# sikang/motion_primitive_library

Hardware: AMD Instinct MI355X
Metric: node-expansions/s (frontier x |U| pair evaluations per second) (higher is better)
Workload: dtype f64; 1 GPU; C4: 3D VoxelMapUtil 512^3, Control::ACC |U|=729 (9^3), 64k-node synthetic frontier; frontier=random, frontier_nodes=65536, frontier_nodes_per_gpu=65536, controls=729, dim=3, map_cells=134217728, device=AMD Radeon Graphics (gfx950:sramecc+:xnack-), compute_units=256, kernel=expand_lex_kernel

## Files before the change

### include/mplx.h

```cpp
#ifndef MPLX_H
#define MPLX_H

#include <stddef.h>
#include <stdint.h>

#ifdef __cplusplus
extern "C" {
#endif

#define MPLX_ABI_VERSION 9

typedef struct mplx_ctx mplx_ctx;

typedef enum {
  MPLX_OK = 0,
  MPLX_ERR_ARG = -1,
  MPLX_ERR_HIP = -2,
  MPLX_ERR_NO_DEVICE = -3,
  MPLX_ERR_STATE = -4,
  MPLX_ERR_NOMEM = -5
} mplx_status;

enum {
  MPLX_VEL = 0x01, MPLX_ACC = 0x03, MPLX_JRK = 0x07, MPLX_SNP = 0x0f,
  MPLX_VELxYAW = 0x11, MPLX_ACCxYAW = 0x13, MPLX_JRKxYAW = 0x17, MPLX_SNPxYAW = 0x1f
};

enum {
  MPLX_SLOT_SKIP_SAME = 0,
  MPLX_SLOT_FINITE = 1,
  MPLX_SLOT_BLOCKED = 2,
  MPLX_SLOT_SKIP_DYN = 3
};

typedef struct {
  int32_t control;
  int32_t reserved;
  double dt;
  double w;
  double wyaw;
  double v_max, a_max, j_max, yaw_max;
  double potential_weight;
  double gradient_weight;
} mplx_params;

typedef struct {
  uint8_t *status;
  double *cost;
  uint64_t *hash;
  double *state;
  int64_t state_stride;
  int32_t *iters;
} mplx_succ;

int mplx_create(int dim, int device, mplx_ctx **out);
void mplx_destroy(mplx_ctx *ctx);
const char *mplx_last_error(const mplx_ctx *ctx);
int mplx_abi_version(void);

int mplx_set_map(mplx_ctx *ctx, const int8_t *cells, const int32_t *dim, const double *origin,
                 double res);
int mplx_edit_map(mplx_ctx *ctx, const int64_t *cell_index, const int8_t *values, int64_t n);
int mplx_map_upload_bytes(mplx_ctx *ctx, uint64_t *bytes);
int mplx_read_cells(mplx_ctx *ctx, int which, const int64_t *cell_index, int64_t n, int8_t *out);

int mplx_set_potential(mplx_ctx *ctx, const int8_t *cells_or_null);
int mplx_set_region(mplx_ctx *ctx, const uint8_t *cells_or_null);
int mplx_set_params(mplx_ctx *ctx, const mplx_params *p);
int mplx_set_controls(mplx_ctx *ctx, const double *U, int32_t nU, int32_t udim);

int mplx_update_potential_map(mplx_ctx *ctx, const double *pos, const double *radius,
                              const double *range_or_null, double pow, int8_t *h_map_out_or_null);
int mplx_set_search_region_path(mplx_ctx *ctx, const double *path, int32_t n_points, int32_t dense,
                                const double *search_radius, uint8_t *h_region_out_or_null);

int mplx_expand_device(mplx_ctx *ctx, const double *d_nodes, int64_t n_nodes, int64_t node_stride,
                       const mplx_succ *d_out);
int mplx_expand(mplx_ctx *ctx, const double *h_nodes, int64_t n_nodes, int64_t node_stride,
                const mplx_succ *h_out);
int mplx_get_succ(mplx_ctx *ctx, const double *node, double *succ, double *cost, int32_t *action,
                  int32_t *n_succ);

typedef struct {
  int32_t *count;
  int32_t *action;
  double *cost;
  uint64_t *hash;
  double *state;
  int64_t state_stride;
  int32_t *iters;
  int64_t node_stride;
  double *heur;
  uint8_t *flags;
} mplx_succ_lists;

int mplx_expand_lists_device(mplx_ctx *ctx, const double *d_nodes, int64_t n_nodes, int64_t node_stride,
                             const mplx_succ_lists *d_out);
int mplx_expand_lists(mplx_ctx *ctx, const double *h_nodes, int64_t n_nodes, int64_t node_stride,
                      const mplx_succ_lists *h_out);

int mplx_lists_zero_fill(mplx_ctx *ctx, const mplx_succ_lists *d_lists, uint32_t *zero_rows);
int mplx_expand_lists_device_z(mplx_ctx *ctx, const double *d_nodes, int64_t n_nodes, int64_t node_stride,
                               const mplx_succ_lists *d_out, uint32_t *zero_rows);

typedef struct {
  const double *goal;
  int32_t control;
  int32_t goal_control;
  double w, v_max;
  double tol_pos, tol_vel, tol_acc, tol_yaw;
} mplx_goal_spec;

int mplx_set_goal(mplx_ctx *ctx, const mplx_goal_spec *goal);

typedef struct {
  double *heur;
  uint8_t *flags;
  int32_t *canon;
} mplx_post;

int mplx_post_lists_device(mplx_ctx *ctx, const mplx_succ_lists *d_lists, int64_t n_nodes,
                           const mplx_goal_spec *goal, const mplx_post *d_out);

typedef struct {
  int32_t *count;
  int64_t *offs;
  int32_t *action;
  double *cost;
  uint64_t *hash;
  double *state;
  int64_t state_stride;
  int64_t capacity;
} mplx_packed_lists;

int mplx_pack_lists_device(mplx_ctx *ctx, const mplx_succ_lists *d_lists, int64_t n_nodes,
                           const mplx_packed_lists *d_out, int64_t *h_total_or_null);

int mplx_post_packed_device(mplx_ctx *ctx, const mplx_packed_lists *d_packed, int64_t n_nodes,
                            const mplx_goal_spec *goal, const mplx_post *d_out);

#define MPLX_COMM_ID_BYTES 128
int mplx_comm_unique_id(uint8_t *id_out );
int mplx_comm_init(mplx_ctx *ctx, const uint8_t *id, int32_t rank, int32_t world);
int mplx_comm_destroy(mplx_ctx *ctx);
int mplx_comm_broadcast_map(mplx_ctx *ctx, int32_t root);
int mplx_comm_allgather_lists(mplx_ctx *ctx, const mplx_packed_lists *d_local, int64_t n_local,
                              const mplx_packed_lists *d_all, int64_t *h_node_offs, int64_t *h_entry_offs);

#define MPLX_COMM_META 8
enum { MPLX_ROWBIT_ACTION = 1, MPLX_ROWBIT_COST = 2, MPLX_ROWBIT_HASH = 4, MPLX_ROWBIT_STATE = 8 };
enum { MPLX_COMM_COPY = 0, MPLX_COMM_SEND = 1, MPLX_COMM_RECV = 2 };
enum { MPLX_ROW_COUNT = 0, MPLX_ROW_ACTION = 1, MPLX_ROW_COST = 2, MPLX_ROW_HASH = 3, MPLX_ROW_STATE0 = 4  };
typedef struct {
  int32_t kind;
  int32_t peer;
  int32_t row;
  int32_t elem;
  int64_t src_off;
  int64_t dst_off;
  int64_t bytes;
} mplx_comm_op;
int64_t mplx_comm_schedule(int32_t world, int32_t rank, const int64_t *meta, int32_t n_fields,
                           mplx_comm_op *ops, int64_t cap, int64_t *node_offs, int64_t *entry_offs);

typedef struct {
  uint8_t *free_flag;
  double *cost;
  int32_t *cells;
  int32_t *cell_count;
  int32_t cell_cap;
  uint8_t *outside;
} mplx_edges_out;
int mplx_check_edges(mplx_ctx *ctx, const double *h_parents, const int32_t *h_actions, int64_t n_edges,
                     int64_t stride, const mplx_edges_out *h_out);

int mplx_device_alloc(mplx_ctx *ctx, size_t bytes, void **dptr);
int mplx_device_free(mplx_ctx *ctx, void *dptr);
int mplx_memcpy_h2d(mplx_ctx *ctx, void *dst, const void *src, size_t bytes);
int mplx_memcpy_d2h(mplx_ctx *ctx, void *dst, const void *src, size_t bytes);
int mplx_memset(mplx_ctx *ctx, void *dst, int value, size_t bytes);
int mplx_synchronize(mplx_ctx *ctx);
int mplx_timer_begin(mplx_ctx *ctx);
int mplx_timer_end(mplx_ctx *ctx, float *ms);


typedef struct mplx_planner mplx_planner;

typedef int (*mplx_succ_fn)(void *user, const double *node, double *succ, double *cost,
                            int32_t *action, int32_t *n_succ);
typedef int (*mplx_batch_fn)(void *user, const double *nodes, int64_t n, uint8_t *status,
                             double *cost, double *state);

typedef struct {
  int32_t control;
  int32_t max_expand;
  int32_t batch;
  int32_t goal_control;
  double dt, w, v_max;
  double epsilon;
  double tol_pos, tol_vel, tol_acc, tol_yaw;
} mplx_planner_config;

typedef struct {
  int32_t ok;
  int32_t expansions;
  int32_t closed, opened, nodes;
  int32_t device_launches;
  int64_t pairs;
  double cost;
  double total_time;
  double J[4];
  int32_t segments;
  int32_t state_mismatches;
} mplx_plan_summary;

int mplx_planner_create(int dim, mplx_planner **out);
void mplx_planner_destroy(mplx_planner *p);
int mplx_planner_attach_ctx(mplx_planner *p, mplx_ctx *ctx);
int mplx_planner_set_provider(mplx_planner *p, mplx_succ_fn single, mplx_batch_fn batched, void *user);
int mplx_planner_set_map(mplx_planner *p, const int8_t *cells, const int32_t *dim,
                         const double *origin, double res);
int mplx_planner_edit_map(mplx_planner *p, const int64_t *cell_index, const int8_t *values, int64_t n);
int mplx_planner_set_controls(mplx_planner *p, const double *U, int32_t nU, int32_t udim);
int mplx_planner_configure(mplx_planner *p, const mplx_planner_config *cfg);
int mplx_planner_plan(mplx_planner *p, const double *start, const double *goal, mplx_plan_summary *out);
int mplx_planner_trajectory(mplx_planner *p, double *nodes, int32_t *actions, int32_t cap_segments);
int mplx_planner_trajectory_end(mplx_planner *p, double *node);
int mplx_planner_closed_set(mplx_planner *p, double *pos, int32_t cap, int32_t *n);
int mplx_planner_open_set(mplx_planner *p, double *states, int32_t cap, int32_t *n);
const char *mplx_planner_last_error(const mplx_planner *p);
typedef struct {
  double total_ms;
  double provider_ms;
  double fill_ms;
  double pick_ms;
  double relax_ms;
  double recover_ms;
  int64_t relaxed;
  int64_t improved;
  int64_t pushes;
  int64_t materialised;
  int64_t heur_from_device;
} mplx_plan_timing;
int mplx_planner_timing(const mplx_planner *p, mplx_plan_timing *out);
int mplx_planner_set_prior_trajectory(mplx_planner *p, const mplx_planner *from);
int mplx_planner_set_prior_trajectory_potential(mplx_planner *p, const mplx_planner *from, const int8_t *potential,
                                                double potential_weight, double gradient_weight);

int mplx_planner_set_lpastar(mplx_planner *p, int on);
int mplx_planner_reset(mplx_planner *p);
int mplx_planner_linked_nodes(mplx_planner *p, double *points, int64_t cap_points, int64_t *n_points, int64_t *n_cells,
                              int64_t *n_entries);
int mplx_planner_update_blocked_nodes(mplx_planner *p, const int32_t *cells, int64_t n);
int mplx_planner_update_cleared_nodes(mplx_planner *p, const int32_t *cells, int64_t n);
int mplx_planner_sub_state_space(mplx_planner *p, int32_t time_step);
typedef int (*mplx_edges_fn)(void *user, const double *parents, const int32_t *actions, int64_t n_edges, uint8_t *free_flag,
                             double *cost, int32_t *cells, int32_t *cell_count, int32_t cell_cap);
int mplx_planner_set_edge_provider(mplx_planner *p, mplx_edges_fn fn, void *user);
int mplx_planner_use_device_heuristic(mplx_planner *p, int on);

enum { MPLX_ROUTE_AUTO = 0, MPLX_ROUTE_DENSE = 1, MPLX_ROUTE_TILE = 2, MPLX_ROUTE_GRID = 3 };
int mplx_set_lists_route(mplx_ctx *ctx, int route);
int mplx_last_lists_route(const mplx_ctx *ctx);
int mplx_last_lists_zero_rows(const mplx_ctx *ctx);
enum { MPLX_KERNEL_NONE = 0, MPLX_KERNEL_GRID = 1, MPLX_KERNEL_LEX = 2,
       MPLX_KERNEL_PAIR = 3 };
int mplx_last_grid_kernel(const mplx_ctx *ctx);
enum { MPLX_IDENTITY_TABLE = 0, MPLX_IDENTITY_CLAIMED = 1, MPLX_IDENTITY_EXACT = 2, MPLX_IDENTITY_CLAIMED_THEN_EXACT = 3 };
int mplx_last_identity_form(const mplx_ctx *ctx);
int mplx_service(mplx_ctx *ctx, int mode, int64_t stats[4]);
int mplx_device_info(mplx_ctx *ctx, char *name, size_t cap, int32_t *compute_units);

#ifdef __cplusplus
}
#endif
#endif
```

### motion_primitive_library_amd/_abi.py

```python
import ctypes as C
import os

HERE = os.path.dirname(os.path.abspath(__file__))
LIB_PATH = os.environ.get("MPLX_LIB") or os.path.join(HERE, "csrc", "libmplx.so")

OK = 0
ERR_ARG, ERR_HIP, ERR_NO_DEVICE, ERR_STATE = -1, -2, -3, -4

SYMBOLS = [
    "mplx_create", "mplx_destroy", "mplx_last_error", "mplx_abi_version",
    "mplx_set_map", "mplx_edit_map", "mplx_map_upload_bytes", "mplx_read_cells", "mplx_set_potential", "mplx_set_region", "mplx_set_params", "mplx_set_controls",
    "mplx_update_potential_map", "mplx_set_search_region_path",
    "mplx_expand_device", "mplx_expand", "mplx_expand_lists_device", "mplx_expand_lists", "mplx_lists_zero_fill", "mplx_expand_lists_device_z", "mplx_get_succ",
    "mplx_set_goal", "mplx_post_lists_device", "mplx_post_packed_device",
    "mplx_pack_lists_device", "mplx_comm_unique_id", "mplx_comm_init", "mplx_comm_destroy", "mplx_comm_broadcast_map",
    "mplx_comm_allgather_lists", "mplx_comm_schedule",
    "mplx_check_edges",
    "mplx_device_alloc", "mplx_device_free", "mplx_memcpy_h2d", "mplx_memcpy_d2h", "mplx_memset",
    "mplx_synchronize", "mplx_timer_begin", "mplx_timer_end",
    "mplx_planner_create", "mplx_planner_destroy", "mplx_planner_attach_ctx", "mplx_planner_set_provider",
    "mplx_planner_set_map", "mplx_planner_edit_map", "mplx_planner_set_controls", "mplx_planner_configure", "mplx_planner_plan",
    "mplx_planner_trajectory", "mplx_planner_trajectory_end", "mplx_planner_closed_set", "mplx_planner_open_set", "mplx_planner_last_error", "mplx_planner_timing", "mplx_planner_set_prior_trajectory", "mplx_planner_set_prior_trajectory_potential", "mplx_planner_use_device_heuristic", "mplx_planner_set_lpastar", "mplx_planner_reset", "mplx_planner_linked_nodes", "mplx_planner_update_blocked_nodes", "mplx_planner_update_cleared_nodes", "mplx_planner_sub_state_space", "mplx_planner_set_edge_provider",
    "mplx_selftest_math", "mplx_selftest_forward_state", "mplx_set_lists_route", "mplx_last_lists_route", "mplx_last_lists_zero_rows", "mplx_last_grid_kernel", "mplx_last_identity_form", "mplx_debug_store_model", "mplx_yaw_pin_stats", "mplx_service", "mplx_device_info",
]

MAP_UTIL_SYMBOLS = ["mplx_map_dilate", "mplx_map_free", "mplx_map_cloud"]
CELL_OCCUPIED, CELL_FREE, CELL_UNKNOWN = 0, 1, 2
ROLLOUT_SYMBOLS = ["mplx_rollout_device", "mplx_rollout"]
ROLLOUT_BAD_ACTION, ROLLOUT_HEADING_BAND = 4, 0x80
RAY_SYMBOLS = ["mplx_ray_trace_device", "mplx_ray_trace", "mplx_goal_sight_device"]
RAY_LEFT_MAP, RAY_HIT, RAY_BAD, RAY_TRUNCATED = 1, 2, 4, 8
FLAG_GOAL_BLOCKED = 8
TRAJ_SYMBOLS = ["mplx_traj_info_device", "mplx_traj_info", "mplx_traj_sample_device", "mplx_traj_sample",
                "mplx_traj_traverse_device", "mplx_traj_traverse"]
TRAJ_EMPTY, TRAJ_BAD_ACTION, TRAJ_BAD = 1, 2, 4
TRAJ_COMMAND, TRAJ_WAYPOINT = 0, 1
TABLE_SYMBOLS = ["mplx_table_create", "mplx_table_destroy", "mplx_table_clear", "mplx_table_view_of", "mplx_table_stats",
                 "mplx_table_seed", "mplx_table_relax_device", "mplx_table_find_device", "mplx_table_find", "mplx_table_path",
                 "mplx_table_set_time_keys", "mplx_time_key"]
TABLE_NODES_FULL, TABLE_PROBE_FULL, TABLE_FRONTIER_FULL = 1, 2, 4
OPEN_SYMBOLS = ["mplx_open_create", "mplx_open_destroy", "mplx_open_clear", "mplx_open_view_of", "mplx_open_push_device",
                "mplx_open_select_device"]
OPEN_IS_OPEN, OPEN_IS_GOAL, OPEN_SEEN = 1, 2, 4
OPEN_SELECTED, OPEN_FOUND, OPEN_EMPTY = 0, 1, 2
MULTI_SYMBOLS = ["mplx_table_create_multi", "mplx_table_query_of", "mplx_table_seed_multi", "mplx_table_find_multi_device",
                 "mplx_table_find_multi", "mplx_open_set_goals", "mplx_open_select_multi_device"]
REPLAN_SYMBOLS = ["mplx_table_rebase_device", "mplx_table_rebase_multi_device", "mplx_open_push_closed_device"]
PRIOR_SYMBOLS = ["mplx_open_set_priors_device", "mplx_open_clear_priors", "mplx_open_prior_view_of", "mplx_planner_prior_table"]
SOLVE_SYMBOLS = ["mplx_poly_create", "mplx_poly_destroy", "mplx_solve_device", "mplx_solve", "mplx_poly_info_device",
                 "mplx_poly_info", "mplx_poly_sample_device", "mplx_poly_sample", "mplx_poly_traverse_device",
                 "mplx_poly_traverse"]
SOLVE_EMPTY, SOLVE_BAD_TIME, SOLVE_SINGULAR = 1, 2, 8
USE_POS, USE_VEL, USE_ACC = 1, 2, 4
LIMITS_SYMBOLS = ["mplx_poly_load_device", "mplx_poly_load", "mplx_poly_limits_device", "mplx_poly_limits",
                  "mplx_shortcut_device", "mplx_shortcut"]
SHORTCUT_BAD_CHAIN = 16
LIMITS_REFERENCE, LIMITS_ALL_ROOTS = 0, 1
EXCEED_VEL, EXCEED_ACC, EXCEED_JRK = 1, 2, 4
SCALE_SYMBOLS = ["mplx_poly_set_lambda_device", "mplx_poly_set_lambda", "mplx_poly_scale_device", "mplx_poly_scale",
                 "mplx_poly_scale_down_device", "mplx_poly_scale_down", "mplx_poly_tau_device", "mplx_poly_tau",
                 "mplx_poly_clear_lambda"]
SCALE_REFERENCE, SCALE_ROBUST = 0, 1
LAMBDA_BAD_POINTS, LAMBDA_NOT_POSITIVE = 32, 64
LAMBDA_MAX_SEGS, LAMBDA_NEWTON = 8, 3
CONFLICT_SYMBOLS = ["mplx_poly_conflicts_device", "mplx_poly_conflicts", "mplx_traj_conflicts_device", "mplx_traj_conflicts"]
CONFLICT_PARK, CONFLICT_GONE = 0, 1
CONFLICT_BAD_INPUT = 128
RESERVE_SYMBOLS = ["mplx_reserve_create", "mplx_reserve_destroy", "mplx_reserve_fill_poly_device", "mplx_reserve_fill_poly",
                   "mplx_reserve_fill_traj_device", "mplx_reserve_fill_traj", "mplx_reserve_shape", "mplx_reserve_positions",
                   "mplx_reserve_set_queries", "mplx_reserve_check_device", "mplx_reserve_park_device"]
RESERVE_MAX_BYTES = 1 << 30
WAIT_SYMBOLS = ["mplx_lists_add_wait_device"]
REPLAN_TIMED_SYMBOLS = ["mplx_table_rebase_timed_device"]
FIELD_SYMBOLS = ["mplx_field_create", "mplx_field_destroy", "mplx_field_build", "mplx_field_shape", "mplx_field_view_of",
                 "mplx_field_download", "mplx_field_is_stale", "mplx_field_passes", "mplx_open_set_field", "mplx_open_clear_field"]
FIELD_MAX_BYTES = 1 << 30
HEUR_SYMBOLS = ["mplx_heur_eval", "mplx_heur_eval_device", "mplx_open_set_heur", "mplx_planner_set_heur_dynamics"]
HEUR_DEFAULT, HEUR_REFERENCE, HEUR_ROBUST = 0, 1, 2
HEUR_BISECT = 56


def heur_mode(mode):
    names = {None: HEUR_DEFAULT, False: HEUR_DEFAULT, "default": HEUR_DEFAULT, "reference": HEUR_REFERENCE, "robust": HEUR_ROBUST}
    if isinstance(mode, str) or mode is None:
        if mode not in names:
            raise ValueError("heuristic mode %r: None, 'default', 'reference' or 'robust'" % (mode,))
        return names[mode]
    return int(mode)

ROUTE_AUTO, ROUTE_DENSE, ROUTE_TILE, ROUTE_GRID = 0, 1, 2, 3


class Params(C.Structure):
    _fields_ = [
        ("control", C.c_int32), ("reserved", C.c_int32),
        ("dt", C.c_double), ("w", C.c_double), ("wyaw", C.c_double),
        ("v_max", C.c_double), ("a_max", C.c_double), ("j_max", C.c_double), ("yaw_max", C.c_double),
        ("potential_weight", C.c_double), ("gradient_weight", C.c_double),
    ]


class Succ(C.Structure):
    _fields_ = [
        ("status", C.c_void_p), ("cost", C.c_void_p), ("hash", C.c_void_p),
        ("state", C.c_void_p), ("state_stride", C.c_int64), ("iters", C.c_void_p),
    ]


class SuccLists(C.Structure):
    _fields_ = [
        ("count", C.c_void_p), ("action", C.c_void_p), ("cost", C.c_void_p), ("hash", C.c_void_p),
        ("state", C.c_void_p), ("state_stride", C.c_int64), ("iters", C.c_void_p), ("node_stride", C.c_int64),
        ("heur", C.c_void_p), ("flags", C.c_void_p),
    ]


class RolloutOut(C.Structure):
    _fields_ = [
        ("status", C.c_void_p), ("steps", C.c_void_p), ("cost", C.c_void_p), ("prefix_cost", C.c_void_p),
        ("end_state", C.c_void_p), ("end_stride", C.c_int64),
        ("end_hash", C.c_void_p), ("end_heur", C.c_void_p), ("end_flags", C.c_void_p),
    ]


class RayOut(C.Structure):
    _fields_ = [("status", C.c_void_p), ("n_cells", C.c_void_p), ("first_hit", C.c_void_p), ("cells", C.c_void_p),
                ("cell_cap", C.c_int32)]


class TrajSet(C.Structure):
    _fields_ = [("starts", C.c_void_p), ("n_starts", C.c_int64), ("start_stride", C.c_int64), ("actions", C.c_void_p),
                ("n_traj", C.c_int64), ("horizon", C.c_int32), ("action_stride", C.c_int64)]


class TrajInfoOut(C.Structure):
    _fields_ = [("status", C.c_void_p), ("n_segs", C.c_void_p), ("total_time", C.c_void_p), ("effort", C.c_void_p),
                ("effort_stride", C.c_int64), ("seg_state", C.c_void_p), ("seg_stride", C.c_int64)]


class TrajTimes(C.Structure):
    _fields_ = [("form", C.c_int32), ("n_uniform", C.c_int32), ("times", C.c_void_p), ("n_times", C.c_int64),
                ("time_stride", C.c_int64)]


class TrajSampleOut(C.Structure):
    _fields_ = [("out", C.c_void_p), ("row_stride", C.c_int64), ("sample_stride", C.c_int64), ("status", C.c_void_p)]


class TrajTraverseOut(C.Structure):
    _fields_ = [("status", C.c_void_p), ("cost", C.c_void_p), ("n_samples", C.c_void_p), ("n_cells", C.c_void_p),
                ("stop_sample", C.c_void_p)]


class SolveIn(C.Structure):
    _fields_ = [("waypoints", C.c_void_p), ("n_prob", C.c_int64), ("w_max", C.c_int32), ("wp_stride", C.c_int64),
                ("n_wp", C.c_void_p), ("dts", C.c_void_p), ("dt_stride", C.c_int64), ("v", C.c_double),
                ("v_arr", C.c_void_p), ("control", C.c_int32), ("yaw_control", C.c_int32), ("wp_flags", C.c_void_p),
                ("flag_stride", C.c_int64)]


class SolveOut(C.Structure):
    _fields_ = [("status", C.c_void_p), ("n_segs", C.c_void_p), ("total_time", C.c_void_p), ("coeff", C.c_void_p),
                ("coeff_stride", C.c_int64), ("dts_out", C.c_void_p), ("dts_out_stride", C.c_int64),
                ("yaw_coeff", C.c_void_p), ("yaw_stride", C.c_int64), ("taus", C.c_void_p), ("taus_stride", C.c_int64)]


class PolyLoadIn(C.Structure):
    _fields_ = [("n_prob", C.c_int64), ("w_max", C.c_int32), ("control", C.c_int32), ("n_segs", C.c_void_p),
                ("dts", C.c_void_p), ("dt_stride", C.c_int64), ("coeff", C.c_void_p), ("coeff_stride", C.c_int64),
                ("src", C.c_void_p), ("src_index", C.c_void_p), ("index_stride", C.c_int64)]


class PolyLoadOut(C.Structure):
    _fields_ = [("status", C.c_void_p), ("n_segs", C.c_void_p), ("total_time", C.c_void_p), ("taus", C.c_void_p),
                ("taus_stride", C.c_int64)]


class ShortcutIn(C.Structure):
    _fields_ = [("states", C.c_void_p), ("n_query", C.c_int64), ("w_max", C.c_int32), ("control", C.c_int32),
                ("stride", C.c_int64), ("n_wp", C.c_void_p), ("max_hop", C.c_int32)]


class ShortcutOut(C.Structure):
    _fields_ = [("status", C.c_void_p), ("n_keep", C.c_void_p), ("keep", C.c_void_p), ("keep_stride", C.c_int64),
                ("cost", C.c_void_p), ("chain_cost", C.c_void_p), ("edge_cost", C.c_void_p), ("pair_out", C.POINTER(SolveOut))]


class LimitsIn(C.Structure):
    _fields_ = [("mv", C.c_double), ("ma", C.c_double), ("mj", C.c_double), ("mode", C.c_int32)]


class LimitsOut(C.Structure):
    _fields_ = [("max_vel", C.c_void_p), ("max_acc", C.c_void_p), ("max_jrk", C.c_void_p), ("max_stride", C.c_int64),
                ("exceed", C.c_void_p), ("valid", C.c_void_p), ("first_bad", C.c_void_p)]


class LambdaOut(C.Structure):
    _fields_ = [("status", C.c_void_p), ("n_lseg", C.c_void_p), ("total", C.c_void_p), ("Ts", C.c_void_p),
                ("ts_stride", C.c_int64), ("segs", C.c_void_p), ("seg_stride", C.c_int64)]


class LambdaIn(C.Structure):
    _fields_ = [("pts", C.c_void_p), ("stride", C.c_int64), ("n_pts", C.c_void_p), ("mode", C.c_int32)]


class ScaleIn(C.Structure):
    _fields_ = [("ri", C.c_double), ("rf", C.c_double), ("ri_arr", C.c_void_p), ("rf_arr", C.c_void_p), ("mode", C.c_int32)]


class ScaleDownIn(C.Structure):
    _fields_ = [("mv", C.c_double), ("ma", C.c_double), ("ri", C.c_double), ("rf", C.c_double), ("mode", C.c_int32)]


class ScaleDownOut(C.Structure):
    _fields_ = [("scaled", C.c_void_p), ("max_l", C.c_void_p), ("t_lo", C.c_void_p), ("t_hi", C.c_void_p), ("lam", LambdaOut)]


class TauOut(C.Structure):
    _fields_ = [("tau", C.c_void_p), ("lam", C.c_void_p), ("lam_dot", C.c_void_p), ("found", C.c_void_p), ("stride", C.c_int64)]


class ConflictIn(C.Structure):
    _fields_ = [("step", C.c_double), ("n_steps", C.c_int32), ("mode", C.c_int32), ("t0", C.c_void_p), ("radius", C.c_void_p),
                ("radius_all", C.c_double), ("group", C.c_void_p), ("rank", C.c_void_p), ("chunk_steps", C.c_int32)]


class ConflictOut(C.Structure):
    _fields_ = [("first_step", C.c_void_p), ("first_partner", C.c_void_p), ("min_d2", C.c_void_p), ("status", C.c_void_p),
                ("pair_first", C.c_void_p), ("pair_stride", C.c_int64)]


class TableView(C.Structure):
    _fields_ = [("hash", C.c_void_p), ("g", C.c_void_p), ("pred", C.c_void_p), ("pred_action", C.c_void_p),
                ("state", C.c_void_p), ("state_stride", C.c_int64)]


class TableFrontier(C.Structure):
    _fields_ = [("id", C.c_void_p), ("g", C.c_void_p), ("state", C.c_void_p), ("state_stride", C.c_int64),
                ("capacity", C.c_int64), ("count", C.c_void_p)]


class OpenView(C.Structure):
    _fields_ = [("f", C.c_void_p), ("flags", C.c_void_p)]


class OpenResult(C.Structure):
    _fields_ = [("status", C.c_int32), ("goal_id", C.c_int32), ("count", C.c_int64), ("n_open", C.c_int64),
                ("f_min", C.c_double), ("goal_f", C.c_double), ("goal_g", C.c_double)]


class PriorSource(C.Structure):
    _fields_ = [("control", C.c_int32), ("nU", C.c_int32), ("udim", C.c_int32), ("U", C.c_void_p), ("dt", C.c_double)]


class PriorInfo(C.Structure):
    _fields_ = [("status", C.c_void_p), ("n_steps", C.c_void_p)]


class PriorView(C.Structure):
    _fields_ = [("n_steps", C.c_void_p), ("pos", C.c_void_p), ("togo", C.c_void_p), ("goal_row", C.c_void_p),
                ("goal_hash", C.c_void_p), ("step_capacity", C.c_int64)]


class FieldView(C.Structure):
    _fields_ = [("dist", C.c_void_p), ("F", C.c_int32), ("n_cells", C.c_int64)]


class RebaseResult(C.Structure):
    _fields_ = [("n_kept", C.c_int64), ("n_bad_edges", C.c_int64), ("n_roots", C.c_int64)]


class PackedLists(C.Structure):
    _fields_ = [
        ("count", C.c_void_p), ("offs", C.c_void_p), ("action", C.c_void_p), ("cost", C.c_void_p), ("hash", C.c_void_p),
        ("state", C.c_void_p), ("state_stride", C.c_int64), ("capacity", C.c_int64),
    ]


COMM_ID_BYTES = 128
COMM_META = 8
ROWBIT_ACTION, ROWBIT_COST, ROWBIT_HASH, ROWBIT_STATE = 1, 2, 4, 8
COMM_COPY, COMM_SEND, COMM_RECV = 0, 1, 2
ROW_COUNT, ROW_ACTION, ROW_COST, ROW_HASH, ROW_STATE0 = 0, 1, 2, 3, 4


class CommOp(C.Structure):
    _fields_ = [("kind", C.c_int32), ("peer", C.c_int32), ("row", C.c_int32), ("elem", C.c_int32),
                ("src_off", C.c_int64), ("dst_off", C.c_int64), ("bytes", C.c_int64)]


class GoalSpec(C.Structure):
    _fields_ = [("goal", C.c_void_p), ("control", C.c_int32), ("goal_control", C.c_int32), ("w", C.c_double),
                ("v_max", C.c_double), ("tol_pos", C.c_double), ("tol_vel", C.c_double), ("tol_acc", C.c_double),
                ("tol_yaw", C.c_double)]


class EdgesOut(C.Structure):
    _fields_ = [("free_flag", C.c_void_p), ("cost", C.c_void_p), ("cells", C.c_void_p), ("cell_count", C.c_void_p),
                ("cell_cap", C.c_int32), ("outside", C.c_void_p)]


class Post(C.Structure):
    _fields_ = [("heur", C.c_void_p), ("flags", C.c_void_p), ("canon", C.c_void_p)]


class PlannerConfig(C.Structure):
    _fields_ = [
        ("control", C.c_int32), ("max_expand", C.c_int32), ("batch", C.c_int32), ("goal_control", C.c_int32),
        ("dt", C.c_double), ("w", C.c_double), ("v_max", C.c_double), ("epsilon", C.c_double),
        ("tol_pos", C.c_double), ("tol_vel", C.c_double), ("tol_acc", C.c_double), ("tol_yaw", C.c_double),
    ]


class PlanSummary(C.Structure):
    _fields_ = [
        ("ok", C.c_int32), ("expansions", C.c_int32), ("closed", C.c_int32), ("opened", C.c_int32),
        ("nodes", C.c_int32), ("device_launches", C.c_int32), ("pairs", C.c_int64),
        ("cost", C.c_double), ("total_time", C.c_double), ("J", C.c_double * 4),
        ("segments", C.c_int32), ("state_mismatches", C.c_int32),
    ]


class PlanTiming(C.Structure):
    _fields_ = [(k, C.c_double) for k in ("total_ms", "provider_ms", "fill_ms", "pick_ms", "relax_ms", "recover_ms")] + \
               [(k, C.c_int64) for k in ("relaxed", "improved", "pushes", "materialised", "heur_from_device")]


class MplxError(RuntimeError):
    def __init__(self, code, text):
        super().__init__("mplx error %d: %s" % (code, text))
        self.code = code


_lib = None


def lib():
    global _lib
    if _lib is not None:
        return _lib
    if not os.path.exists(LIB_PATH):
        raise ImportError(
            "motion_primitive_library_amd: %s is missing. Build it with "
            "`python -m motion_primitive_library_amd.build` (needs hipcc); there is no CPU fallback."
            % LIB_PATH)
    try:
        L = C.CDLL(LIB_PATH)
    except OSError as e:
        raise ImportError("motion_primitive_library_amd: cannot load %s: %s" % (LIB_PATH, e))
    vp, i32, i64, dbl = C.c_void_p, C.c_int32, C.c_int64, C.c_double
    sig = {
        "mplx_create": (C.c_int, [C.c_int, C.c_int, C.POINTER(vp)]),
        "mplx_destroy": (None, [vp]),
        "mplx_last_error": (C.c_char_p, [vp]),
        "mplx_abi_version": (C.c_int, []),
        "mplx_set_map": (C.c_int, [vp, vp, vp, vp, dbl]),
        "mplx_set_potential": (C.c_int, [vp, vp]),
        "mplx_set_region": (C.c_int, [vp, vp]),
        "mplx_set_params": (C.c_int, [vp, C.POINTER(Params)]),
        "mplx_set_controls": (C.c_int, [vp, vp, i32, i32]),
        "mplx_edit_map": (C.c_int, [vp, vp, vp, i64]),
        "mplx_map_upload_bytes": (C.c_int, [vp, C.POINTER(C.c_uint64)]),
        "mplx_read_cells": (C.c_int, [vp, C.c_int, vp, i64, vp]),
        "mplx_set_goal": (C.c_int, [vp, C.POINTER(GoalSpec)]),
        "mplx_update_potential_map": (C.c_int, [vp, vp, vp, vp, dbl, vp]),
        "mplx_set_search_region_path": (C.c_int, [vp, vp, i32, i32, vp, vp]),
        "mplx_expand_device": (C.c_int, [vp, vp, i64, i64, C.POINTER(Succ)]),
        "mplx_expand": (C.c_int, [vp, vp, i64, i64, C.POINTER(Succ)]),
        "mplx_expand_lists_device": (C.c_int, [vp, vp, i64, i64, C.POINTER(SuccLists)]),
        "mplx_expand_lists": (C.c_int, [vp, vp, i64, i64, C.POINTER(SuccLists)]),
        "mplx_lists_zero_fill": (C.c_int, [vp, C.POINTER(SuccLists), C.POINTER(C.c_uint32)]),
        "mplx_expand_lists_device_z": (C.c_int, [vp, vp, i64, i64, C.POINTER(SuccLists), C.POINTER(C.c_uint32)]),
        "mplx_get_succ": (C.c_int, [vp, vp, vp, vp, vp, C.POINTER(i32)]),
        "mplx_post_lists_device": (C.c_int, [vp, C.POINTER(SuccLists), i64, C.POINTER(GoalSpec), C.POINTER(Post)]),
        "mplx_check_edges": (C.c_int, [vp, vp, vp, i64, i64, C.POINTER(EdgesOut)]),
        "mplx_pack_lists_device": (C.c_int, [vp, C.POINTER(SuccLists), i64, C.POINTER(PackedLists), C.POINTER(i64)]),
        "mplx_post_packed_device": (C.c_int, [vp, C.POINTER(PackedLists), i64, C.POINTER(GoalSpec), C.POINTER(Post)]),
        "mplx_comm_unique_id": (C.c_int, [vp]),
        "mplx_comm_init": (C.c_int, [vp, vp, i32, i32]),
        "mplx_comm_destroy": (C.c_int, [vp]),
        "mplx_comm_broadcast_map": (C.c_int, [vp, i32]),
        "mplx_comm_allgather_lists": (C.c_int, [vp, C.POINTER(PackedLists), i64, C.POINTER(PackedLists), vp, vp]),
        "mplx_comm_schedule": (i64, [i32, i32, vp, i32, C.POINTER(CommOp), i64, vp, vp]),
        "mplx_device_alloc": (C.c_int, [vp, C.c_size_t, C.POINTER(vp)]),
        "mplx_device_free": (C.c_int, [vp, vp]),
        "mplx_memcpy_h2d": (C.c_int, [vp, vp, vp, C.c_size_t]),
        "mplx_memcpy_d2h": (C.c_int, [vp, vp, vp, C.c_size_t]),
        "mplx_memset": (C.c_int, [vp, vp, C.c_int, C.c_size_t]),
        "mplx_synchronize": (C.c_int, [vp]),
        "mplx_timer_begin": (C.c_int, [vp]),
        "mplx_timer_end": (C.c_int, [vp, C.POINTER(C.c_float)]),
        "mplx_planner_create": (C.c_int, [C.c_int, C.POINTER(vp)]),
        "mplx_planner_destroy": (None, [vp]),
        "mplx_planner_attach_ctx": (C.c_int, [vp, vp]),
        "mplx_planner_set_provider": (C.c_int, [vp, vp, vp, vp]),
        "mplx_planner_set_map": (C.c_int, [vp, vp, vp, vp, dbl]),
        "mplx_planner_edit_map": (C.c_int, [vp, vp, vp, i64]),
        "mplx_planner_set_controls": (C.c_int, [vp, vp, i32, i32]),
        "mplx_planner_configure": (C.c_int, [vp, C.POINTER(PlannerConfig)]),
        "mplx_planner_plan": (C.c_int, [vp, vp, vp, C.POINTER(PlanSummary)]),
        "mplx_planner_trajectory": (C.c_int, [vp, vp, vp, i32]),
        "mplx_planner_trajectory_end": (C.c_int, [vp, vp]),
        "mplx_planner_closed_set": (C.c_int, [vp, vp, i32, C.POINTER(i32)]),
        "mplx_planner_open_set": (C.c_int, [vp, vp, i32, C.POINTER(i32)]),
        "mplx_planner_last_error": (C.c_char_p, [vp]),
        "mplx_planner_timing": (C.c_int, [vp, C.POINTER(PlanTiming)]),
        "mplx_planner_use_device_heuristic": (C.c_int, [vp, C.c_int]),
        "mplx_planner_set_prior_trajectory": (C.c_int, [vp, vp]),
        "mplx_planner_set_prior_trajectory_potential": (C.c_int, [vp, vp, vp, dbl, dbl]),
        "mplx_planner_set_lpastar": (C.c_int, [vp, C.c_int]),
        "mplx_planner_reset": (C.c_int, [vp]),
        "mplx_planner_linked_nodes": (C.c_int, [vp, vp, i64, C.POINTER(i64), C.POINTER(i64), C.POINTER(i64)]),
        "mplx_planner_update_blocked_nodes": (C.c_int, [vp, vp, i64]),
        "mplx_planner_update_cleared_nodes": (C.c_int, [vp, vp, i64]),
        "mplx_planner_sub_state_space": (C.c_int, [vp, i32]),
        "mplx_planner_set_edge_provider": (C.c_int, [vp, vp, vp]),
        "mplx_selftest_math": (C.c_int, [vp, C.c_int, vp, vp, vp, i64]),
        "mplx_selftest_forward_state": (C.c_int, [i32, i32, vp, vp, C.c_double, vp]),
        "mplx_set_lists_route": (C.c_int, [vp, C.c_int]),
        "mplx_last_lists_route": (C.c_int, [vp]),
        "mplx_last_lists_zero_rows": (C.c_int, [vp]),
        "mplx_last_grid_kernel": (C.c_int, [vp]),
        "mplx_last_identity_form": (C.c_int, [vp]),
        "mplx_debug_store_model": (C.c_int, [vp, C.POINTER(SuccLists), i64]),
        "mplx_yaw_pin_stats": (C.c_int, [vp, C.POINTER(i64), C.POINTER(i64)]),
        "mplx_service": (C.c_int, [vp, C.c_int, C.POINTER(i64)]),
        "mplx_device_info": (C.c_int, [vp, C.c_char_p, C.c_size_t, C.POINTER(i32)]),
        "mplx_map_dilate": (C.c_int, [vp, vp, i32, vp]),
        "mplx_map_free": (C.c_int, [vp, C.c_int, vp]),
        "mplx_map_cloud": (C.c_int, [vp, C.c_int, vp, i64, C.POINTER(i64)]),
        "mplx_rollout_device": (C.c_int, [vp, vp, i64, i64, vp, i64, i32, i64, C.POINTER(RolloutOut)]),
        "mplx_rollout": (C.c_int, [vp, vp, i64, i64, vp, i64, i32, i64, C.POINTER(RolloutOut)]),
        "mplx_ray_trace_device": (C.c_int, [vp, vp, vp, i64, i64, i64, i32, C.POINTER(RayOut)]),
        "mplx_ray_trace": (C.c_int, [vp, vp, vp, i64, i64, i64, i32, C.POINTER(RayOut)]),
        "mplx_goal_sight_device": (C.c_int, [vp, C.POINTER(SuccLists), i64, C.POINTER(GoalSpec), vp]),
        "mplx_traj_info_device": (C.c_int, [vp, C.POINTER(TrajSet), C.POINTER(TrajInfoOut)]),
        "mplx_traj_info": (C.c_int, [vp, C.POINTER(TrajSet), C.POINTER(TrajInfoOut)]),
        "mplx_traj_sample_device": (C.c_int, [vp, C.POINTER(TrajSet), C.POINTER(TrajTimes), C.POINTER(TrajSampleOut)]),
        "mplx_traj_sample": (C.c_int, [vp, C.POINTER(TrajSet), C.POINTER(TrajTimes), C.POINTER(TrajSampleOut)]),
        "mplx_traj_traverse_device": (C.c_int, [vp, C.POINTER(TrajSet), i32, C.POINTER(TrajTraverseOut)]),
        "mplx_traj_traverse": (C.c_int, [vp, C.POINTER(TrajSet), i32, C.POINTER(TrajTraverseOut)]),
        "mplx_poly_create": (C.c_int, [vp, i64, i32, C.POINTER(vp)]),
        "mplx_poly_destroy": (None, [vp]),
        "mplx_solve_device": (C.c_int, [vp, C.POINTER(SolveIn), C.POINTER(SolveOut)]),
        "mplx_solve": (C.c_int, [vp, C.POINTER(SolveIn), C.POINTER(SolveOut)]),
        "mplx_poly_info_device": (C.c_int, [vp, C.POINTER(TrajInfoOut)]),
        "mplx_poly_info": (C.c_int, [vp, C.POINTER(TrajInfoOut)]),
        "mplx_poly_sample_device": (C.c_int, [vp, C.POINTER(TrajTimes), C.POINTER(TrajSampleOut)]),
        "mplx_poly_sample": (C.c_int, [vp, C.POINTER(TrajTimes), C.POINTER(TrajSampleOut)]),
        "mplx_poly_traverse_device": (C.c_int, [vp, i32, C.POINTER(TrajTraverseOut)]),
        "mplx_poly_traverse": (C.c_int, [vp, i32, C.POINTER(TrajTraverseOut)]),
        "mplx_poly_load_device": (C.c_int, [vp, C.POINTER(PolyLoadIn), C.POINTER(PolyLoadOut)]),
        "mplx_poly_load": (C.c_int, [vp, C.POINTER(PolyLoadIn), C.POINTER(PolyLoadOut)]),
        "mplx_poly_limits_device": (C.c_int, [vp, C.POINTER(LimitsIn), C.POINTER(LimitsOut)]),
        "mplx_poly_limits": (C.c_int, [vp, C.POINTER(LimitsIn), C.POINTER(LimitsOut)]),
        "mplx_shortcut_device": (C.c_int, [vp, vp, C.POINTER(ShortcutIn), C.POINTER(ShortcutOut)]),
        "mplx_shortcut": (C.c_int, [vp, vp, C.POINTER(ShortcutIn), C.POINTER(ShortcutOut)]),
        "mplx_poly_set_lambda_device": (C.c_int, [vp, C.POINTER(LambdaIn), C.POINTER(LambdaOut)]),
        "mplx_poly_set_lambda": (C.c_int, [vp, C.POINTER(LambdaIn), C.POINTER(LambdaOut)]),
        "mplx_poly_scale_device": (C.c_int, [vp, C.POINTER(ScaleIn), C.POINTER(LambdaOut)]),
        "mplx_poly_scale": (C.c_int, [vp, C.POINTER(ScaleIn), C.POINTER(LambdaOut)]),
        "mplx_poly_scale_down_device": (C.c_int, [vp, C.POINTER(ScaleDownIn), C.POINTER(ScaleDownOut)]),
        "mplx_poly_scale_down": (C.c_int, [vp, C.POINTER(ScaleDownIn), C.POINTER(ScaleDownOut)]),
        "mplx_poly_tau_device": (C.c_int, [vp, C.POINTER(TrajTimes), C.POINTER(TauOut)]),
        "mplx_poly_tau": (C.c_int, [vp, C.POINTER(TrajTimes), C.POINTER(TauOut)]),
        "mplx_poly_clear_lambda": (C.c_int, [vp]),
        "mplx_poly_conflicts_device": (C.c_int, [vp, C.POINTER(ConflictIn), C.POINTER(ConflictOut)]),
        "mplx_poly_conflicts": (C.c_int, [vp, C.POINTER(ConflictIn), C.POINTER(ConflictOut)]),
        "mplx_traj_conflicts_device": (C.c_int, [vp, C.POINTER(TrajSet), C.POINTER(ConflictIn), C.POINTER(ConflictOut)]),
        "mplx_traj_conflicts": (C.c_int, [vp, C.POINTER(TrajSet), C.POINTER(ConflictIn), C.POINTER(ConflictOut)]),
        "mplx_table_create": (C.c_int, [vp, i64, i32, C.POINTER(vp)]),
        "mplx_table_destroy": (None, [vp]),
        "mplx_table_clear": (C.c_int, [vp]),
        "mplx_table_view_of": (C.c_int, [vp, C.POINTER(TableView)]),
        "mplx_table_stats": (C.c_int, [vp, C.POINTER(i64), C.POINTER(C.c_uint32)]),
        "mplx_table_seed": (C.c_int, [vp, vp, i64, i64, vp, C.POINTER(TableFrontier), C.POINTER(i64)]),
        "mplx_table_relax_device": (C.c_int, [vp, C.POINTER(SuccLists), i64, vp, vp, dbl, C.POINTER(TableFrontier), vp,
                                              C.POINTER(i64)]),
        "mplx_table_find_device": (C.c_int, [vp, vp, i64, vp]),
        "mplx_table_find": (C.c_int, [vp, vp, i64, vp]),
        "mplx_table_path": (C.c_int, [vp, i32, vp, vp, i64, C.POINTER(i64)]),
        "mplx_open_create": (C.c_int, [vp, C.POINTER(vp)]),
        "mplx_open_destroy": (None, [vp]),
        "mplx_open_clear": (C.c_int, [vp]),
        "mplx_open_view_of": (C.c_int, [vp, C.POINTER(OpenView)]),
        "mplx_open_push_device": (C.c_int, [vp, C.POINTER(TableFrontier), i64, dbl, i32]),
        "mplx_open_select_device": (C.c_int, [vp, dbl, C.POINTER(TableFrontier), vp, C.POINTER(OpenResult)]),
        "mplx_table_create_multi": (C.c_int, [vp, i64, i32, i32, C.POINTER(vp)]),
        "mplx_table_query_of": (C.c_int, [vp, C.POINTER(vp), C.POINTER(i32)]),
        "mplx_table_seed_multi": (C.c_int, [vp, vp, i64, i64, vp, vp, C.POINTER(TableFrontier), C.POINTER(i64)]),
        "mplx_table_find_multi_device": (C.c_int, [vp, vp, vp, i64, vp]),
        "mplx_table_find_multi": (C.c_int, [vp, vp, vp, i64, vp]),
        "mplx_open_set_goals": (C.c_int, [vp, C.POINTER(GoalSpec), i32]),
        "mplx_open_select_multi_device": (C.c_int, [vp, dbl, C.POINTER(TableFrontier), vp, C.POINTER(OpenResult)]),
        "mplx_table_rebase_device": (C.c_int, [vp, i32, i32, C.POINTER(TableFrontier), vp, C.POINTER(RebaseResult)]),
        "mplx_table_rebase_multi_device": (C.c_int, [vp, vp, i32, C.POINTER(TableFrontier), vp, C.POINTER(RebaseResult)]),
        "mplx_open_push_closed_device": (C.c_int, [vp, C.POINTER(TableFrontier), i64, dbl, i32]),
        "mplx_open_set_priors_device": (C.c_int, [vp, C.POINTER(PriorSource), C.POINTER(TrajSet), C.POINTER(PriorInfo)]),
        "mplx_open_clear_priors": (C.c_int, [vp]),
        "mplx_open_prior_view_of": (C.c_int, [vp, C.POINTER(PriorView)]),
        "mplx_planner_prior_table": (C.c_int, [vp, vp, vp, i32, C.POINTER(i32), vp, C.POINTER(i32)]),
        "mplx_reserve_create": (C.c_int, [vp, C.POINTER(vp)]),
        "mplx_reserve_destroy": (None, [vp]),
        "mplx_reserve_fill_poly_device": (C.c_int, [vp, vp, C.POINTER(ConflictIn)]),
        "mplx_reserve_fill_poly": (C.c_int, [vp, vp, C.POINTER(ConflictIn)]),
        "mplx_reserve_fill_traj_device": (C.c_int, [vp, vp, C.POINTER(TrajSet), C.POINTER(ConflictIn)]),
        "mplx_reserve_fill_traj": (C.c_int, [vp, vp, C.POINTER(TrajSet), C.POINTER(ConflictIn)]),
        "mplx_reserve_shape": (C.c_int, [vp, C.POINTER(i64), C.POINTER(i32), C.POINTER(dbl)]),
        "mplx_reserve_positions": (C.c_int, [vp, vp, vp, vp, vp, vp, vp]),
        "mplx_reserve_set_queries": (C.c_int, [vp, i32, vp, vp, vp]),
        "mplx_reserve_check_device": (C.c_int, [vp, vp, C.POINTER(SuccLists), i64, vp, vp, i64, vp, vp]),
        "mplx_reserve_park_device": (C.c_int, [vp, vp, C.POINTER(TableFrontier), i64, vp, vp]),
        "mplx_lists_add_wait_device": (C.c_int, [vp, C.POINTER(SuccLists), i64, vp, i64, vp, vp]),
        "mplx_table_rebase_timed_device": (C.c_int, [vp, vp, i32, i32, vp, C.POINTER(TableFrontier), vp, vp, vp,
                                                    C.POINTER(RebaseResult)]),
        "mplx_field_create": (C.c_int, [vp, C.POINTER(vp)]),
        "mplx_field_destroy": (None, [vp]),
        "mplx_field_build": (C.c_int, [vp, i32, vp, vp]),
        "mplx_field_shape": (C.c_int, [vp, C.POINTER(i32), C.POINTER(i64)]),
        "mplx_field_view_of": (C.c_int, [vp, C.POINTER(FieldView)]),
        "mplx_field_download": (C.c_int, [vp, vp]),
        "mplx_field_is_stale": (C.c_int, [vp]),
        "mplx_field_passes": (C.c_int, [vp, C.POINTER(i64)]),
        "mplx_open_set_field": (C.c_int, [vp, vp, vp]),
        "mplx_open_clear_field": (C.c_int, [vp]),
        "mplx_heur_eval": (C.c_int, [vp, C.POINTER(GoalSpec), i32, vp, i64, i64, vp]),
        "mplx_heur_eval_device": (C.c_int, [vp, C.POINTER(GoalSpec), i32, vp, i64, i64, vp]),
        "mplx_open_set_heur": (C.c_int, [vp, i32]),
        "mplx_planner_set_heur_dynamics": (C.c_int, [vp, i32]),
        "mplx_table_set_time_keys": (C.c_int, [vp, i32]),
        "mplx_time_key": (C.c_uint64, [C.c_uint64, dbl]),
    }
    for name in SYMBOLS + MAP_UTIL_SYMBOLS + ROLLOUT_SYMBOLS + RAY_SYMBOLS + TRAJ_SYMBOLS + TABLE_SYMBOLS + OPEN_SYMBOLS + MULTI_SYMBOLS + REPLAN_SYMBOLS + PRIOR_SYMBOLS + SOLVE_SYMBOLS + LIMITS_SYMBOLS + SCALE_SYMBOLS + CONFLICT_SYMBOLS + RESERVE_SYMBOLS + WAIT_SYMBOLS + REPLAN_TIMED_SYMBOLS + FIELD_SYMBOLS + HEUR_SYMBOLS:
        fn = getattr(L, name)
        fn.restype, fn.argtypes = sig[name]
    _lib = L
    return L


def check(ctx, rc):
    if rc != OK:
        msg = lib().mplx_last_error(ctx)
        raise MplxError(rc, msg.decode() if msg else "?")
```

### motion_primitive_library_amd/build.py

```python
import os
import shutil
import subprocess
import sys

HERE = os.path.dirname(os.path.abspath(__file__))
CSRC = os.path.join(HERE, "csrc")
LIB = os.path.join(CSRC, "libmplx.so")
SOURCES = ["expand_kernel.hip", "expand_tile_kernel.hip", "expand_grid_kernel.hip", "expand_lex_kernel.hip", "expand_pair_kernel.hip", "map_prep_kernel.hip", "map_prep_api.cpp", "map_util_kernel.hip", "map_util_api.cpp", "rollout_kernel.hip", "rollout_api.cpp", "ray_kernel.hip", "ray_api.cpp", "traj_kernel.hip", "traj_api.cpp", "solve_kernel.hip", "solve_api.cpp", "limits_kernel.hip", "limits_api.cpp", "scale_kernel.hip", "scale_api.cpp", "conflict_kernel.hip", "conflict_api.cpp", "reserve_kernel.hip", "reserve_api.cpp", "wait_kernel.hip", "wait_api.cpp", "table_kernel.hip", "table_api.cpp", "open_kernel.hip", "open_api.cpp", "field_kernel.hip", "field_api.cpp", "heur_kernel.hip", "heur_api.cpp", "replan_kernel.hip", "replan_api.cpp", "post_kernel.hip", "identity_kernel.hip", "post_api.cpp", "edge_kernel.hip", "edge_api.cpp", "mplx_api.cpp", "lists_route.cpp", "yaw_pin.cpp", "lists_host.cpp", "planner_capi.cpp", "pack_kernel.hip", "store_model_kernel.hip", "lists_copy_api.cpp", "pack_api.cpp", "comm_api.cpp"]
HEADERS = ["mplx_internal.h", "mplx_ctx.h", "mplx_device_common.h", "mplx_pair_device.h", "mplx_grid_common.h", "mplx_poly.h", "mplx_traj_device.h", "mplx_limits_math.h", "mplx_scale_math.h", "mplx_heur_math.h", "host_planner.hpp", "host_lpastar.hpp", os.path.join("..", "..", "include", "mplx.h"), os.path.join("..", "..", "include", "mplx_debug.h"), os.path.join("..", "..", "include", "mplx_map_util.h"), os.path.join("..", "..", "include", "mplx_rollout.h"), os.path.join("..", "..", "include", "mplx_ray.h"), os.path.join("..", "..", "include", "mplx_traj.h"), os.path.join("..", "..", "include", "mplx_table.h"), os.path.join("..", "..", "include", "mplx_open.h"), os.path.join("..", "..", "include", "mplx_multi.h"), os.path.join("..", "..", "include", "mplx_replan.h"), os.path.join("..", "..", "include", "mplx_replan_timed.h"), os.path.join("..", "..", "include", "mplx_prior.h"), os.path.join("..", "..", "include", "mplx_solve.h"), os.path.join("..", "..", "include", "mplx_limits.h"), os.path.join("..", "..", "include", "mplx_scale.h"), os.path.join("..", "..", "include", "mplx_conflict.h"), os.path.join("..", "..", "include", "mplx_reserve.h"), os.path.join("..", "..", "include", "mplx_wait.h"), os.path.join("..", "..", "include", "mplx_field.h"), os.path.join("..", "..", "include", "mplx_heur.h")]
ARCH = "gfx950"


def hipcc_path():
    for cand in (os.environ.get("HIPCC"), shutil.which("hipcc"), "/opt/rocm/bin/hipcc"):
        if cand and os.path.exists(cand):
            return cand
    raise RuntimeError("hipcc not found (set HIPCC or install ROCm under /opt/rocm)")


def _obj_dir():
    d = os.path.join(CSRC, "build")
    os.makedirs(d, exist_ok=True)
    return d


def is_stale():
    if not os.path.exists(LIB):
        return True
    t = os.path.getmtime(LIB)
    deps = [os.path.join(CSRC, s) for s in SOURCES + HEADERS]
    return any(os.path.getmtime(d) > t for d in deps)


FLAGS = ["--offload-arch=" + ARCH, "-O3", "-std=c++17", "-ffp-contract=off", "-fPIC", "-Wall"]
EXTRA_FLAGS = {}


def build_variant(out_path, defines, verbose=False):
    cmd = [hipcc_path()] + FLAGS + ["-D" + d for d in defines] + ["-shared", "-o", out_path] + SOURCES
    if verbose:
        print(" ".join(cmd), file=sys.stderr)
    proc = subprocess.run(cmd, cwd=CSRC, capture_output=True, text=True)
    if proc.returncode != 0:
        raise RuntimeError("hipcc failed:\n%s\n%s" % (proc.stdout, proc.stderr))
    return out_path


def build(force=False, verbose=False, jobs=None):
    if not force and not is_stale():
        return LIB
    from concurrent.futures import ThreadPoolExecutor

    hipcc = hipcc_path()
    odir = _obj_dir()
    hdr_t = max(os.path.getmtime(os.path.join(CSRC, h)) for h in HEADERS)
    todo, objs = [], []
    for src in SOURCES:
        obj = os.path.join(odir, src + ".o")
        objs.append(obj)
        st = max(os.path.getmtime(os.path.join(CSRC, src)), hdr_t)
        if force or not os.path.exists(obj) or os.path.getmtime(obj) < st:
            todo.append((src, obj))

    def cc(job):
        src, obj = job
        cmd = [hipcc] + FLAGS + EXTRA_FLAGS.get(src, []) + ["-x", "hip", "-c", src, "-o", obj]
        if verbose:
            print(" ".join(cmd), file=sys.stderr)
        return src, subprocess.run(cmd, cwd=CSRC, capture_output=True, text=True)

    with ThreadPoolExecutor(max_workers=jobs or min(8, os.cpu_count() or 1)) as ex:
        for src, proc in ex.map(cc, todo):
            if proc.returncode != 0:
                raise RuntimeError("hipcc failed on %s:\n%s\n%s" % (src, proc.stdout, proc.stderr))
            if verbose and proc.stderr.strip():
                print(proc.stderr, file=sys.stderr)
    cmd = [hipcc, "--offload-arch=" + ARCH, "-fPIC", "-shared", "-o", LIB] + objs
    if verbose:
        print(" ".join(cmd), file=sys.stderr)
    proc = subprocess.run(cmd, cwd=CSRC, capture_output=True, text=True)
    if proc.returncode != 0:
        raise RuntimeError("hipcc link failed:\n%s\n%s" % (proc.stdout, proc.stderr))
    return LIB


if __name__ == "__main__":
    if "--define" in sys.argv:
        defs = [d for i, a in enumerate(sys.argv[:-1]) if a == "--define" for d in sys.argv[i + 1].split(",")]
        out = sys.argv[sys.argv.index("--out") + 1]
        print(build_variant(os.path.abspath(out), defs, verbose=True))
    else:
        print(build(force="--force" in sys.argv, verbose=True))
```

### motion_primitive_library_amd/csrc/lists_copy_api.cpp

```cpp
#include "mplx_ctx.h"

#include <atomic>
#include <cstring>
#include <thread>

namespace mplx_detail {

namespace {

struct Row {
  const void *dev;
  char *host;
  int es;
  int64_t host_node_stride;
};

constexpr size_t kChunkBytes = 32u << 20;

int ensure_pinned(mplx_ctx *c, size_t bytes) {
  if (bytes <= c->pk_pin_cap) return MPLX_OK;
  for (int i = 0; i < 2; i++) {
    if (c->pk_pin[i]) HIP_TRY(c, hipHostFree(c->pk_pin[i]));
    c->pk_pin[i] = nullptr;
  }
  c->pk_pin_cap = 0;
  for (int i = 0; i < 2; i++) HIP_TRY(c, hipHostMalloc(&c->pk_pin[i], bytes, hipHostMallocDefault));
  c->pk_pin_cap = bytes;
  return MPLX_OK;
}

struct Chunk {
  int64_t node0, node1, off0, entries;
};

void scatter(const Row *rows, int n_rows, const int64_t *row_off, const char *pin, const int32_t *count,
             const int64_t *offs, const Chunk &ch, int64_t a, int64_t b) {
  for (int r = 0; r < n_rows; r++) {
    const int es = rows[r].es;
    const char *src = pin + row_off[r];
    for (int64_t k = a; k < b; k++) {
      const int cnt = count[k];
      if (cnt > 0)
        std::memcpy(rows[r].host + (size_t)k * rows[r].host_node_stride * es, src + (size_t)(offs[k] - ch.off0) * es,
                    (size_t)cnt * es);
    }
  }
}

}

void release_copy_buffers(mplx_ctx *c) {
  for (int i = 0; i < 2; i++) {
    if (c->pk_pin[i]) (void)hipHostFree(c->pk_pin[i]);
    c->pk_pin[i] = nullptr;
    if (c->pk_ev[i]) (void)hipEventDestroy(c->pk_ev[i]);
    c->pk_ev[i] = nullptr;
    release(c->pk_dev[i]);
  }
  c->pk_pin_cap = 0;
  release(c->pk_offs);
  if (c->pk_hb) (void)hipHostFree(c->pk_hb);
  c->pk_hb = nullptr;
  c->pk_hb_cap = 0;
}

int copy_lists_to_host(mplx_ctx *c, const mplx_succ_lists &d, const mplx_succ_lists *h, int64_t n_nodes) {
  const int F = 4 * c->dim + 2;
  const int64_t S = list_stride(c, &d);
  HIP_TRY(c, hipMemcpyAsync(h->count, d.count, (size_t)n_nodes * 4, hipMemcpyDeviceToHost, c->stream));
  HIP_TRY(c, hipStreamSynchronize(c->stream));
  Row rows[mplx::kPackRows];
  int n_rows = 0;
  if (h->cost) rows[n_rows++] = {d.cost, (char *)h->cost, 8, S};
  if (h->hash) rows[n_rows++] = {d.hash, (char *)h->hash, 8, S};
  if (h->state)
    for (int f = 0; f < F; f++)
      rows[n_rows++] = {d.state + (size_t)f * d.state_stride, (char *)(h->state + (size_t)f * h->state_stride), 8, S};
  if (h->action) rows[n_rows++] = {d.action, (char *)h->action, 4, S};
  if (h->iters) rows[n_rows++] = {d.iters, (char *)h->iters, 4, S};
  if (n_rows == 0) return MPLX_OK;
  int bpe = 0;
  for (int r = 0; r < n_rows; r++) bpe += rows[r].es;

  std::vector<int64_t> &offs = c->pk_hoffs;
  offs.resize((size_t)n_nodes + 1);
  int64_t total = 0;
  int max_cnt = 0;
  for (int64_t k = 0; k < n_nodes; k++) {
    offs[(size_t)k] = total;
    const int cnt = h->count[k];
    total += cnt;
    max_cnt = cnt > max_cnt ? cnt : max_cnt;
  }
  offs[(size_t)n_nodes] = total;
  if (total == 0) return MPLX_OK;
  size_t cap = kChunkBytes;
  if ((size_t)max_cnt * bpe > cap) cap = (size_t)max_cnt * bpe;
  if ((size_t)total * bpe < cap) cap = (size_t)total * bpe;
  cap = align256(cap);
  const int64_t cap_entries = (int64_t)(cap / bpe);
  if (int rc = ensure_pinned(c, cap)) return rc;
  for (int i = 0; i < 2; i++) {
    if (int rc = ensure(c, c->pk_dev[i], cap)) return rc;
    if (!c->pk_ev[i]) HIP_TRY(c, hipEventCreateWithFlags(&c->pk_ev[i], hipEventDisableTiming));
  }
  if (int rc = ensure(c, c->pk_offs, (size_t)n_nodes * 8)) return rc;
  HIP_TRY(c, hipMemcpyAsync(c->pk_offs.p, offs.data(), (size_t)n_nodes * 8, hipMemcpyHostToDevice, c->stream));

  std::vector<Chunk> chunks;
  for (int64_t a = 0; a < n_nodes;) {
    int64_t b = a + 1;
    while (b < n_nodes && offs[(size_t)b + 1] - offs[(size_t)a] <= cap_entries) b++;
    chunks.push_back({a, b, offs[(size_t)a], offs[(size_t)b] - offs[(size_t)a]});
    a = b;
  }
  const int n_chunks = (int)chunks.size();
  std::vector<int64_t> row_off((size_t)n_chunks * n_rows);
  for (int i = 0; i < n_chunks; i++) {
    int64_t o = 0;
    for (int r = 0; r < n_rows; r++) {
      row_off[(size_t)i * n_rows + r] = o;
      o += chunks[(size_t)i].entries * rows[r].es;
    }
  }

  int n_thr = (int)(((size_t)total * bpe) >> 23);
  const int hw = (int)std::thread::hardware_concurrency();
  if (n_thr > 15) n_thr = 15;
  if (hw > 0 && n_thr > hw - 1) n_thr = hw - 1;
  if (n_thr < 0) n_thr = 0;
  int parts = n_thr + 1;
  std::atomic<int> ready{0};
  std::atomic<int> done{0};
  std::atomic<bool> cancel{false};
  const int32_t *count = h->count;
  auto share = [&](int i, int part) {
    const Chunk &ch = chunks[(size_t)i];
    const int64_t n = ch.node1 - ch.node0;
    const int64_t a = ch.node0 + n * part / parts, b = ch.node0 + n * (part + 1) / parts;
    scatter(rows, n_rows, &row_off[(size_t)i * n_rows], (const char *)c->pk_pin[i & 1], count, offs.data(), ch, a, b);
  };
  std::vector<std::thread> helpers;
  try {
    for (int t = 0; t < n_thr; t++)
      helpers.emplace_back([&, t] {
        for (int i = 0; i < n_chunks; i++) {
          while (ready.load(std::memory_order_acquire) <= i) std::this_thread::yield();
          if (cancel.load(std::memory_order_acquire)) return;
          share(i, t + 1);
          done.fetch_add(1, std::memory_order_release);
        }
      });
  } catch (...) {
    cancel.store(true, std::memory_order_release);
    ready.store(n_chunks + 1, std::memory_order_release);
    for (auto &th : helpers) th.join();
    helpers.clear();
    ready.store(0, std::memory_order_release);
    n_thr = 0;
    parts = 1;
  }
  auto join_all = [&] {
    ready.store(n_chunks + 1, std::memory_order_release);
    for (auto &th : helpers) th.join();
  };

  int rc = MPLX_OK;
  auto issue = [&](int i) -> hipError_t {
    const Chunk &ch = chunks[(size_t)i];
    mplx::PackArgs a{};
    for (int r = 0; r < n_rows; r++) {
      a.src[r] = rows[r].dev;
      a.dst_off[r] = row_off[(size_t)i * n_rows + r];
      a.es[r] = rows[r].es;
    }
    a.n_rows = n_rows;
    a.node_stride = S;
    a.count = d.count;
    a.offs = (const int64_t *)c->pk_offs.p;
    a.node0 = ch.node0;
    a.off0 = ch.off0;
    a.dst = (char *)c->pk_dev[i & 1].p;
    hipError_t e = mplx::launch_pack_rows(a, ch.node1 - ch.node0, c->stream);
    if (e != hipSuccess) return e;
    if (ch.entries > 0) {
      e = hipMemcpyAsync(c->pk_pin[i & 1], c->pk_dev[i & 1].p, (size_t)ch.entries * bpe, hipMemcpyDeviceToHost, c->stream);
      if (e != hipSuccess) return e;
    }
    return hipEventRecord(c->pk_ev[i & 1], c->stream);
  };
  for (int i = 0; i <= n_chunks && rc == MPLX_OK; i++) {
    hipError_t e = hipSuccess;
    if (i < n_chunks) e = issue(i);
    if (e == hipSuccess && i >= 1) e = hipEventSynchronize(c->pk_ev[(i - 1) & 1]);
    if (e != hipSuccess) {
      rc = fail(c, MPLX_ERR_HIP, "copy of the successor lists failed: %s", hipGetErrorString(e));
      break;
    }
    if (i >= 1) {
      ready.store(i, std::memory_order_release);
      share(i - 1, 0);
      while (done.load(std::memory_order_acquire) < i * n_thr) std::this_thread::yield();
    }
  }
  if (rc != MPLX_OK) {
    join_all();
    (void)hipStreamSynchronize(c->stream);
    return rc;
  }
  join_all();
  return MPLX_OK;
}

int expand_lists_packed(mplx_ctx *c, const double *h_nodes, int64_t n_nodes, int64_t node_stride, bool want_state,
                        PackedLists *out, bool want_heur) {
  if (!c || !out || !h_nodes || n_nodes <= 0 || node_stride < n_nodes) return fail(c, MPLX_ERR_ARG, "expand_lists_packed: bad arguments");
  if (int rc = ctx_ready(c)) return rc;
  const int F = 4 * c->dim + 2;
  const int64_t S = (c->nU + 31) & ~31;
  const int64_t n_slots = n_nodes * S;
  {
    mplx_succ_lists want{}, v{};
    int32_t dummy_i = 0;
    double dummy_d = 0;
    uint64_t dummy_h = 0;
    want.count = &dummy_i; want.action = &dummy_i; want.cost = &dummy_d; want.hash = &dummy_h;
    if (want_state) want.state = &dummy_d;
    if (want_heur) want.heur = &dummy_d;
    want.node_stride = S;
    bool handled = false;
    if (int rc = svc_request(c, h_nodes, n_nodes, node_stride, &want, &handled, &v)) return rc;
    if (handled) {
      c->pk_hoffs.resize((size_t)n_nodes + 1);
      for (int64_t k = 0; k <= n_nodes; k++) c->pk_hoffs[(size_t)k] = k * S;
      *out = PackedLists{};
      out->total = want_state ? v.state_stride : n_slots;
      out->count = v.count;
      out->offs = c->pk_hoffs.data();
      out->cost = v.cost;
      out->hash = v.hash;
      out->action = v.action;
      out->state = want_state ? v.state : nullptr;
      out->heur = want_heur ? v.heur : nullptr;
      return MPLX_OK;
    }
    const int counted = c->svc.streak;
    if (int rc = bind_device(c)) return rc;
    c->svc.streak = counted;
  }
  if (c->tune.zero_copy && (size_t)n_slots * (size_t)((want_state ? F * 8 : 0) + 24 + (want_heur ? 8 : 0)) <= ((size_t)32 << 20)) {
    const size_t o_cnt = align256((size_t)F * n_nodes * 8);
    const size_t o_off = o_cnt + align256((size_t)n_nodes * 4);
    const size_t o_act = o_off + align256((size_t)(n_nodes + 1) * 8);
    const size_t o_cost = o_act + align256((size_t)n_slots * 4);
    const size_t o_hash = o_cost + align256((size_t)n_slots * 8);
    const size_t o_heur = o_hash + align256((size_t)n_slots * 8);
    const size_t o_state = o_heur + (want_heur ? align256((size_t)n_slots * 8) : 0);
    const size_t bytes = o_state + (want_state ? align256((size_t)F * n_slots * 8) : 0);
    if (bytes > c->pk_hb_cap) {
      if (c->pk_hb) HIP_TRY(c, hipHostFree(c->pk_hb));
      c->pk_hb = nullptr;
      c->pk_hb_cap = 0;
      HIP_TRY(c, hipHostMalloc(&c->pk_hb, bytes + bytes / 2, hipHostMallocCoherent));
      c->pk_hb_cap = bytes + bytes / 2;
    }
    char *hb = (char *)c->pk_hb;
    for (int f = 0; f < F; f++)
      std::memcpy(hb + (size_t)f * n_nodes * 8, h_nodes + (size_t)f * node_stride, (size_t)n_nodes * 8);
    mplx_succ_lists d{};
    d.count = (int32_t *)(hb + o_cnt);
    d.action = (int32_t *)(hb + o_act);
    d.cost = (double *)(hb + o_cost);
    d.hash = (uint64_t *)(hb + o_hash);
    if (want_state) { d.state = (double *)(hb + o_state); d.state_stride = n_slots; }
    if (want_heur) d.heur = (double *)(hb + o_heur);
    d.node_stride = S;
    c->want_done = true;
    const int rc_launch = lists_device(c, (const double *)hb, n_nodes, n_nodes, &d);
    c->want_done = false;
    if (rc_launch) return rc_launch;
    if (int rc = wait_small_launch(c)) return rc;
    if (int rc = resolve_pending(c, true)) return rc;
    int64_t *offs = (int64_t *)(hb + o_off);
    for (int64_t k = 0; k <= n_nodes; k++) offs[k] = k * S;
    *out = PackedLists{};
    out->total = n_slots;
    out->count = d.count;
    out->offs = offs;
    out->cost = d.cost;
    out->hash = d.hash;
    out->action = d.action;
    out->state = d.state;
    out->heur = d.heur;
    return MPLX_OK;
  }
  const size_t o_cnt = align256((size_t)F * n_nodes * 8);
  const size_t o_off = o_cnt + align256((size_t)n_nodes * 4);
  const size_t hb_bytes = o_off + (size_t)(n_nodes + 1) * 8;
  if (hb_bytes > c->pk_hb_cap) {
    if (c->pk_hb) HIP_TRY(c, hipHostFree(c->pk_hb));
    c->pk_hb = nullptr;
    c->pk_hb_cap = 0;
    HIP_TRY(c, hipHostMalloc(&c->pk_hb, hb_bytes * 2, hipHostMallocCoherent));
    c->pk_hb_cap = hb_bytes * 2;
  }
  char *hb = (char *)c->pk_hb;
  for (int f = 0; f < F; f++)
    std::memcpy(hb + (size_t)f * n_nodes * 8, h_nodes + (size_t)f * node_stride, (size_t)n_nodes * 8);
  const size_t slots = (size_t)n_slots;
  StageLayout l;
  const size_t o_nodes = l.add((size_t)F * n_nodes * 8), o_count = l.add((size_t)n_nodes * 4), o_action = l.add(slots * 4),
               o_cost = l.add(slots * 8), o_hash = l.add(slots * 8), o_state = l.add(want_state ? F * slots * 8 : 0);
  if (int rc = stage_commit(c, &l)) return rc;
  if (int rc = ensure(c, c->pk_offs, (size_t)n_nodes * 8)) return rc;
  HIP_TRY(c, stage_in(c, l.base + o_nodes, hb, (size_t)F * n_nodes * 8));
  mplx_succ_lists d{};
  d.count = (int32_t *)(l.base + o_count);
  d.action = (int32_t *)(l.base + o_action);
  d.cost = (double *)(l.base + o_cost);
  d.hash = (uint64_t *)(l.base + o_hash);
  if (want_state) { d.state = (double *)(l.base + o_state); d.state_stride = n_slots; }
  d.node_stride = S;
  if (int rc = lists_device(c, (const double *)(l.base + o_nodes), n_nodes, n_nodes, &d)) return rc;
  if (int rc = resolve_pending(c)) return rc;
  int32_t *cnt = (int32_t *)(hb + o_cnt);
  int64_t *offs = (int64_t *)(hb + o_off);
  HIP_TRY(c, hipMemcpyAsync(cnt, d.count, (size_t)n_nodes * 4, hipMemcpyDeviceToHost, c->stream));
  HIP_TRY(c, hipStreamSynchronize(c->stream));
  int64_t total = 0;
  for (int64_t k = 0; k < n_nodes; k++) { offs[k] = total; total += cnt[k]; }
  offs[n_nodes] = total;
  *out = PackedLists{};
  out->total = total;
  out->count = cnt;
  out->offs = offs;
  if (total == 0) return MPLX_OK;
  const int bpe = 8 + 8 + (want_state ? 8 * F : 0) + 4;
  const size_t bytes = align256((size_t)total * bpe);
  if (int rc = ensure_pinned(c, bytes)) return rc;
  if (int rc = ensure(c, c->pk_dev[0], bytes)) return rc;
  HIP_TRY(c, hipMemcpyAsync(c->pk_offs.p, offs, (size_t)n_nodes * 8, hipMemcpyHostToDevice, c->stream));
  mplx::PackArgs a{};
  int r = 0;
  int64_t o = 0;
  auto row = [&](const void *src, int es) { a.src[r] = src; a.dst_off[r] = o; a.es[r] = es; o += total * es; r++; };
  row(d.cost, 8);
  row(d.hash, 8);
  if (want_state)
    for (int f = 0; f < F; f++) row(d.state + (size_t)f * n_slots, 8);
  row(d.action, 4);
  a.n_rows = r;
  a.node_stride = S;
  a.count = d.count;
  a.offs = (const int64_t *)c->pk_offs.p;
  a.node0 = 0;
  a.off0 = 0;
  a.dst = (char *)c->pk_dev[0].p;
  HIP_TRY(c, mplx::launch_pack_rows(a, n_nodes, c->stream));
  HIP_TRY(c, hipMemcpyAsync(c->pk_pin[0], c->pk_dev[0].p, (size_t)total * bpe, hipMemcpyDeviceToHost, c->stream));
  HIP_TRY(c, hipStreamSynchronize(c->stream));
  const char *pin = (const char *)c->pk_pin[0];
  out->cost = (const double *)(pin + a.dst_off[0]);
  out->hash = (const uint64_t *)(pin + a.dst_off[1]);
  out->state = want_state ? (const double *)(pin + a.dst_off[2]) : nullptr;
  out->action = (const int32_t *)(pin + a.dst_off[want_state ? 2 + F : 2]);
  return MPLX_OK;
}

}
```

### motion_primitive_library_amd/csrc/lists_host.cpp

```cpp
#include "mplx_ctx.h"

#include <atomic>
#include <chrono>
#include <cstring>

using namespace mplx_detail;

namespace {

double mono_us() {
  return std::chrono::duration<double, std::micro>(std::chrono::steady_clock::now().time_since_epoch()).count();
}

struct ArenaLayout {
  size_t o_count = 0, o_action = 0, o_cost = 0, o_hash = 0, o_iters = 0, o_heur = 0, o_flags = 0, o_state = 0, total = 0;
  int64_t n_alloc = 0, n_slots = 0;
};
enum : unsigned { kRowAction = 1, kRowCost = 2, kRowHash = 4, kRowIters = 8, kRowState = 16, kRowHeur = 32, kRowFlags = 64 };

unsigned rows_of(const mplx_succ_lists *o) {
  return (o->action ? kRowAction : 0u) | (o->cost ? kRowCost : 0u) | (o->hash ? kRowHash : 0u) |
         (o->iters ? kRowIters : 0u) | (o->state ? kRowState : 0u) | (o->heur ? kRowHeur : 0u) | (o->flags ? kRowFlags : 0u);
}

ArenaLayout arena_layout(int F, int64_t n_alloc, int64_t S, unsigned rows) {
  ArenaLayout L;
  L.n_alloc = n_alloc;
  L.n_slots = n_alloc * S;
  L.o_count = align256((size_t)F * n_alloc * 8);
  L.o_action = L.o_count + align256((size_t)n_alloc * 4);
  L.o_cost = L.o_action + ((rows & kRowAction) ? align256((size_t)L.n_slots * 4) : 0);
  L.o_hash = L.o_cost + ((rows & kRowCost) ? align256((size_t)L.n_slots * 8) : 0);
  L.o_iters = L.o_hash + ((rows & kRowHash) ? align256((size_t)L.n_slots * 8) : 0);
  L.o_heur = L.o_iters + ((rows & kRowIters) ? align256((size_t)L.n_slots * 4) : 0);
  L.o_flags = L.o_heur + ((rows & kRowHeur) ? align256((size_t)L.n_slots * 8) : 0);
  L.o_state = L.o_flags + ((rows & kRowFlags) ? align256((size_t)L.n_slots) : 0);
  L.total = L.o_state + ((rows & kRowState) ? align256((size_t)F * L.n_slots * 8) : 0);
  return L;
}

void arena_put_nodes(char *hb, const ArenaLayout &L, int F, const double *h_nodes, int64_t n_nodes, int64_t node_stride) {
  for (int f = 0; f < F; f++)
    std::memcpy(hb + (size_t)f * L.n_alloc * 8, h_nodes + (size_t)f * node_stride, (size_t)n_nodes * 8);
}

mplx_succ_lists arena_lists(char *b, const ArenaLayout &L, int64_t S, unsigned rows) {
  mplx_succ_lists d{};
  d.count = (int32_t *)(b + L.o_count);
  if (rows & kRowAction) d.action = (int32_t *)(b + L.o_action);
  if (rows & kRowCost) d.cost = (double *)(b + L.o_cost);
  if (rows & kRowHash) d.hash = (uint64_t *)(b + L.o_hash);
  if (rows & kRowIters) d.iters = (int32_t *)(b + L.o_iters);
  if (rows & kRowHeur) d.heur = (double *)(b + L.o_heur);
  if (rows & kRowFlags) d.flags = (uint8_t *)(b + L.o_flags);
  if (rows & kRowState) { d.state = (double *)(b + L.o_state); d.state_stride = L.n_slots; }
  d.node_stride = S;
  return d;
}

void arena_get_lists(const char *hb, const ArenaLayout &L, int F, int64_t S, int64_t n_nodes, const mplx_succ_lists *h_out) {
  const int32_t *cnt = (const int32_t *)(hb + L.o_count);
  std::memcpy(h_out->count, cnt, (size_t)n_nodes * 4);
  for (int64_t k = 0; k < n_nodes; k++) {
    const size_t m = (size_t)cnt[k], at = (size_t)k * (size_t)S;
    if (!m) continue;
    if (h_out->action) std::memcpy(h_out->action + at, hb + L.o_action + at * 4, m * 4);
    if (h_out->cost) std::memcpy(h_out->cost + at, hb + L.o_cost + at * 8, m * 8);
    if (h_out->hash) std::memcpy(h_out->hash + at, hb + L.o_hash + at * 8, m * 8);
    if (h_out->iters) std::memcpy(h_out->iters + at, hb + L.o_iters + at * 4, m * 4);
    if (h_out->heur) std::memcpy(h_out->heur + at, hb + L.o_heur + at * 8, m * 8);
    if (h_out->flags) std::memcpy(h_out->flags + at, hb + L.o_flags + at, m);
    if (h_out->state)
      for (int f = 0; f < F; f++)
        std::memcpy(h_out->state + (size_t)f * h_out->state_stride + at,
                    hb + L.o_state + ((size_t)f * L.n_slots + at) * 8, m * 8);
  }
}

int svc_launch(mplx_ctx *c, const TilePlan &tp, uint32_t seq_served) {
  mplx_ctx::Service &sv = c->svc;
  const int F = 4 * c->dim + 2;
  HIP_TRY(c, hipSetDevice(c->device));
  if (!sv.stream) HIP_TRY(c, hipStreamCreateWithFlags(&sv.stream, hipStreamNonBlocking));
  if (!sv.mb) {
    HIP_TRY(c, hipHostMalloc((void **)&sv.mb, sizeof(mplx::SvcMailbox), hipHostMallocCoherent));
    std::memset(sv.mb, 0, sizeof(mplx::SvcMailbox));
  }
  if (int rc = ensure_tables(c)) return rc;
  HIP_TRY(c, hipStreamSynchronize(c->stream));
  const ArenaLayout L = arena_layout(F, sv.cap, sv.S, sv.rows);
  if (L.total > sv.block_cap) {
    if (sv.block) HIP_TRY(c, hipHostFree(sv.block));
    sv.block = nullptr;
    sv.block_cap = 0;
    HIP_TRY(c, hipHostMalloc((void **)&sv.block, L.total, hipHostMallocCoherent));
    sv.block_cap = L.total;
  }
  int64_t g = (sv.cap + tp.npb - 1) / tp.npb;
  if (g > tp.grid) g = tp.grid;
  if (g > 1024) g = 1024;
  sv.workgroups = (int)g;
  if (int rc = ensure(c, sv.dev, (size_t)(1 + g) * 8)) return rc;
  HIP_TRY(c, hipMemsetAsync(sv.dev.p, 0, (size_t)(1 + g) * 8, sv.stream));
  const mplx_succ_lists d = arena_lists(sv.block, L, sv.S, sv.rows);
  mplx::TileArgs a = tile_args(c, tp, (const double *)sv.block, sv.cap, sv.cap, &d);
  a.grid_limit = (int32_t)g;
  a.svc_mb = sv.mb;
  a.svc_dev = (uint64_t *)sv.dev.p;
  a.svc_seq0 = seq_served;
  a.svc_idle = (uint64_t)c->tune.service_idle_us * 100ull;
  const int resident = mplx::tile_service_resident_workgroups(c->dim, c->prm.control, a);
  if (resident > 0 && resident < (int)g) {
    sv.disabled = true;
    return MPLX_OK;
  }
  *(volatile uint32_t *)&sv.mb->quit = 0;
  *(volatile uint32_t *)&sv.mb->alive = 1;
  std::atomic_thread_fence(std::memory_order_seq_cst);
  HIP_TRY(c, mplx::launch_expand_tile(c->dim, c->prm.control, a, sv.stream));
  sv.running = true;
  sv.launches++;
  return MPLX_OK;
}
}

int mplx_detail::svc_stop(mplx_ctx *c) {
  mplx_ctx::Service &sv = c->svc;
  if (!sv.running) return MPLX_OK;
  sv.running = false;
  *(volatile uint32_t *)&sv.mb->quit = 1;
  std::atomic_thread_fence(std::memory_order_seq_cst);
  const hipError_t e = hipStreamSynchronize(sv.stream);
  *(volatile uint32_t *)&sv.mb->quit = 0;
  if (e != hipSuccess) {
    sv.disabled = true;
    return fail(c, MPLX_ERR_HIP, "the resident expansion kernel did not leave: %s", hipGetErrorString(e));
  }
  return MPLX_OK;
}

int mplx_detail::wait_small_launch(mplx_ctx *c) {
  if (!c->done_armed) {
    HIP_TRY(c, hipStreamSynchronize(c->stream));
    return MPLX_OK;
  }
  c->done_armed = false;
  volatile uint64_t *f = c->done_host;
  const uint64_t want = c->done_seq;
  double t0 = 0;
  c->done_waits++;
  for (uint32_t spins = 1; *f != want; spins++) {
    __builtin_ia32_pause();
    if ((spins & 0xfffu) != 0) continue;
    const double now = mono_us();
    if (t0 == 0) t0 = now;
    if (now - t0 > 2e5) {
      c->done_timeouts++;
      c->tune.done_flag = 0;
      HIP_TRY(c, hipStreamSynchronize(c->stream));
      (void)hipMemsetAsync(c->done_count.p, 0, 64, c->stream);
      return MPLX_OK;
    }
  }
  std::atomic_thread_fence(std::memory_order_acquire);
  return MPLX_OK;
}

int mplx_detail::svc_request(mplx_ctx *c, const double *h_nodes, int64_t n_nodes, int64_t node_stride, const mplx_succ_lists *h_out,
                bool *handled, mplx_succ_lists *view) {
  *handled = false;
  mplx_ctx::Service &sv = c->svc;
  if (!c->tune.service || sv.disabled) return MPLX_OK;
  const TilePlan tp = (c->lists_route == MPLX_ROUTE_AUTO || c->lists_route == MPLX_ROUTE_TILE) ? plan_tile(c) : TilePlan();
  constexpr int64_t kMaxWorkgroups = 64;
  if (!tp.ok || n_nodes > c->tune.service_max_nodes || (n_nodes + tp.npb - 1) / tp.npb > kMaxWorkgroups) {
    sv.streak = 0;
    return MPLX_OK;
  }
  const int F = 4 * c->dim + 2;
  const int64_t S = list_stride(c, h_out);
  const unsigned rows = rows_of(h_out);
  if (!sv.running || S != sv.S || (rows & ~sv.rows) != 0 || n_nodes > sv.cap) {
    if (!sv.running && ++sv.streak < 2) return MPLX_OK;
    if (int rc = svc_stop(c)) return rc;
    int64_t cap = 64;
    while (cap < n_nodes) cap <<= 1;
    const size_t arena_max = c->tune.arena_kb > 0 ? (size_t)c->tune.arena_kb << 10 : (size_t)8 << 20;
    const unsigned want_rows = (S == sv.S) ? (rows | sv.rows) : rows;
    while (cap > n_nodes && (arena_layout(F, cap, S, want_rows).total > arena_max || (cap + tp.npb - 1) / tp.npb > kMaxWorkgroups)) cap >>= 1;
    if (cap < n_nodes) cap = n_nodes;
    if (arena_layout(F, cap, S, want_rows).total > arena_max) return MPLX_OK;
    sv.cap = cap;
    sv.rows = (S == sv.S) ? (rows | sv.rows) : rows;
    sv.S = S;
    if (sv.seq > 0xfffffff0u) {
      sv.seq = 0;
      if (sv.mb) *(volatile uint64_t *)&sv.mb->doorbell = 0;
    }
    if (int rc = svc_launch(c, tp, sv.seq)) return rc;
    if (!sv.running) return MPLX_OK;
  }
  const ArenaLayout L = arena_layout(F, sv.cap, sv.S, sv.rows);
  arena_put_nodes(sv.block, L, F, h_nodes, n_nodes, node_stride);
  const uint32_t seq = ++sv.seq;
  std::atomic_thread_fence(std::memory_order_release);
  *(volatile uint64_t *)&sv.mb->doorbell = ((uint64_t)seq << 32) | (uint64_t)(uint32_t)n_nodes;
  volatile uint64_t *done = &sv.mb->done;
  volatile uint32_t *alive = &sv.mb->alive;
  double t0 = 0;
  int relaunches = 0;
  for (uint32_t spins = 1; *done != (uint64_t)seq; spins++) {
    __builtin_ia32_pause();
    if ((spins & 0x3ffu) != 0) continue;
    const double now = mono_us();
    if (t0 == 0) t0 = now;
    if (*alive == 0 && *done != (uint64_t)seq && relaunches < 2) {
      sv.running = false;
      relaunches++;
      if (int rc = svc_launch(c, tp, seq - 1)) return rc;
      if (!sv.running) return MPLX_OK;
    } else if (now - t0 > 2e6) {
      sv.failures++;
      (void)svc_stop(c);
      sv.disabled = true;
      return MPLX_OK;
    }
  }
  std::atomic_thread_fence(std::memory_order_acquire);
  if (view) *view = arena_lists(sv.block, L, sv.S, sv.rows);
  else arena_get_lists(sv.block, L, F, sv.S, n_nodes, h_out);
  sv.requests++;
  c->last_route = MPLX_ROUTE_TILE;
  *handled = true;
  return MPLX_OK;
}

extern "C" {

int mplx_expand_lists(mplx_ctx *c, const double *h_nodes, int64_t n_nodes, int64_t node_stride,
                      const mplx_succ_lists *h_out) {
  if (!c) return MPLX_ERR_ARG;
  if (!h_out || !h_out->count || n_nodes < 0 || node_stride < n_nodes || (!h_nodes && n_nodes > 0))
    return fail(c, MPLX_ERR_ARG, "mplx_expand_lists: bad arguments");
  if (int rc = ctx_ready(c)) return rc;
  if (n_nodes == 0) return MPLX_OK;
  const int F = 4 * c->dim + 2;
  if (h_out->node_stride != 0 && h_out->node_stride < c->nU)
    return fail(c, MPLX_ERR_ARG, "mplx_expand_lists: node_stride %lld < nU %d", (long long)h_out->node_stride, c->nU);
  const int64_t S = list_stride(c, h_out), n_slots = n_nodes * S;
  if (h_out->state && h_out->state_stride < n_slots)
    return fail(c, MPLX_ERR_ARG, "mplx_expand_lists: state_stride < n_nodes*node_stride");
  {
    bool handled = false;
    if (int rc = svc_request(c, h_nodes, n_nodes, node_stride, h_out, &handled, nullptr)) return rc;
    if (handled) return MPLX_OK;
    const int counted = c->svc.streak;
    if (int rc = bind_device(c)) return rc;
    c->svc.streak = counted;
  }
  {
    const unsigned rows = rows_of(h_out);
    const ArenaLayout L = arena_layout(F, n_nodes, S, rows);
    const size_t total = L.total, o_count = L.o_count;
    const size_t arena_max = c->tune.arena_kb > 0 ? (size_t)c->tune.arena_kb << 10 : (size_t)8 << 20;
    if (total <= arena_max) {
      if (int rc = ensure(c, c->s_arena, total)) return rc;
      if (total > c->h_arena_cap) {
        if (c->h_arena) HIP_TRY(c, hipHostFree(c->h_arena));
        c->h_arena = nullptr;
        c->h_arena_cap = 0;
        HIP_TRY(c, hipHostMalloc(&c->h_arena, arena_max, hipHostMallocCoherent));
        c->h_arena_cap = arena_max;
      }
      char *hb = (char *)c->h_arena, *db = (char *)c->s_arena.p;
      arena_put_nodes(hb, L, F, h_nodes, n_nodes, node_stride);
      const bool zero_copy = c->tune.zero_copy != 0;
      if (zero_copy) db = hb;
      else HIP_TRY(c, hipMemcpyAsync(db, hb, (size_t)F * n_nodes * 8, hipMemcpyHostToDevice, c->stream));
      const mplx_succ_lists d = arena_lists(db, L, h_out->node_stride, rows);
      c->want_done = zero_copy;
      const int rc_launch = lists_device(c, (const double *)db, n_nodes, n_nodes, &d);
      c->want_done = false;
      if (rc_launch) return rc_launch;
      if (!zero_copy)
        HIP_TRY(c, hipMemcpyAsync(hb + o_count, db + o_count, total - o_count, hipMemcpyDeviceToHost, c->stream));
      if (int rc = wait_small_launch(c)) return rc;
      if (!c->yaw_pending.empty()) {
        if (int rc = resolve_pending(c, true)) return rc;
        if (!zero_copy) {
          HIP_TRY(c, hipMemcpyAsync(hb + o_count, db + o_count, total - o_count, hipMemcpyDeviceToHost, c->stream));
          HIP_TRY(c, hipStreamSynchronize(c->stream));
        }
      }
      arena_get_lists(hb, L, F, S, n_nodes, h_out);
      return MPLX_OK;
    }
  }
  if (h_out->heur || h_out->flags)
    return fail(c, MPLX_ERR_ARG, "mplx_expand_lists: the heur / flags rows come back through host pointers for batches of up to "
                                 "8 MiB of lists only (a search's); larger ones: mplx_expand_lists_device and a copy of the rows");
  const size_t slots = (size_t)n_slots;
  StageLayout l;
  const size_t o_nodes = l.add((size_t)F * n_nodes * 8), o_count = l.add((size_t)n_nodes * 4), o_action = l.add(h_out->action ? slots * 4 : 0),
               o_cost = l.add(h_out->cost ? slots * 8 : 0), o_hash = l.add(h_out->hash ? slots * 8 : 0),
               o_iters = l.add(h_out->iters ? slots * 4 : 0), o_state = l.add(h_out->state ? F * slots * 8 : 0);
  if (int rc = stage_commit(c, &l)) return rc;
  HIP_TRY(c, stage_in_rows(c, l.base + o_nodes, h_nodes, (size_t)node_stride * 8, (size_t)n_nodes * 8, F));
  mplx_succ_lists d{};
  d.count = (int32_t *)(l.base + o_count);
  if (h_out->action) d.action = (int32_t *)(l.base + o_action);
  if (h_out->cost) d.cost = (double *)(l.base + o_cost);
  if (h_out->hash) d.hash = (uint64_t *)(l.base + o_hash);
  if (h_out->iters) d.iters = (int32_t *)(l.base + o_iters);
  if (h_out->state) { d.state = (double *)(l.base + o_state); d.state_stride = n_slots; }
  d.node_stride = h_out->node_stride;
  if (int rc = lists_device(c, (const double *)(l.base + o_nodes), n_nodes, n_nodes, &d)) return rc;
  MPLX_GUARD_BEGIN
  if (int rc = resolve_pending(c)) return rc;
  return copy_lists_to_host(c, d, h_out, n_nodes);
  MPLX_GUARD_END(c)
}

int mplx_get_succ(mplx_ctx *c, const double *node, double *succ, double *cost, int32_t *action,
                  int32_t *n_succ) {
  if (!c) return MPLX_ERR_ARG;
  if (!node || !succ || !cost || !action || !n_succ) return fail(c, MPLX_ERR_ARG, "mplx_get_succ: NULL argument");
  if (int rc = ctx_ready(c)) return rc;
  MPLX_GUARD_BEGIN
  const int F = 4 * c->dim + 2;
  const int nU = c->nU;
  c->h_state.resize((size_t)F * nU);
  int32_t count = 0;
  mplx_succ_lists o{};
  o.count = &count;
  o.action = action;
  o.cost = cost;
  o.state = c->h_state.data();
  o.state_stride = nU;
  if (int rc = mplx_expand_lists(c, node, 1, 1, &o)) return rc;
  for (int m = 0; m < count; m++)
    for (int f = 0; f < F; f++) succ[(size_t)m * F + f] = c->h_state[(size_t)f * nU + m];
  *n_succ = count;
  return MPLX_OK;
  MPLX_GUARD_END(c)
}

int mplx_service(mplx_ctx *c, int mode, int64_t stats[4]) {
  if (!c) return MPLX_ERR_ARG;
  if (mode < -1 || mode > 1) return fail(c, MPLX_ERR_ARG, "mplx_service: mode must be -1, 0 or 1");
  if (mode >= 0) {
    c->tune.service = mode;
    c->svc.streak = 0;
    if (mode == 0) {
      if (int rc = svc_stop(c)) return rc;
    }
  }
  if (stats) {
    stats[0] = c->svc.requests;
    stats[1] = c->svc.launches;
    stats[2] = c->svc.failures;
    stats[3] = c->svc.running ? 1 : 0;
  }
  return MPLX_OK;
}

}
```

### motion_primitive_library_amd/csrc/lists_route.cpp

```cpp
#include "mplx_ctx.h"

#include <cmath>
#include <cstdio>
#include <cstdlib>

namespace mplx_detail {


template <class Args>
static void set_env(const mplx_ctx *c, Args *a) {
  a->region = c->has_region ? (const uint32_t *)c->region_bits.p : nullptr;
  a->dim0 = c->mdim[0]; a->dim1 = c->mdim[1]; a->dim2 = c->mdim[2];
  a->org0 = c->origin[0]; a->org1 = c->origin[1]; a->org2 = c->origin[2];
  a->res = c->res;
  a->dt = c->prm.dt; a->w = c->prm.w;
  a->v_max = c->prm.v_max; a->a_max = c->prm.a_max; a->j_max = c->prm.j_max;
}

template <class Args>
static void set_tables(const mplx_ctx *c, Args *a) {
  a->ttab = (const double *)c->tables.p;
  a->tcnt = (const unsigned char *)c->tables.p + kTcntOffset;
  a->Rres = c->recips[0]; a->R001 = c->recips[1]; a->R01 = c->recips[2];
}
// ... 49 lines not shown
static void arm_done(mplx_ctx *c, mplx::DoneSignal *done) {
  c->done_armed = false;
  if (c->want_done && c->tune.done_flag && c->done_host) {
    done->flag = c->done_host;
    done->count = (uint32_t *)c->done_count.p;
    done->seq = ++c->done_seq;
  }
}

static int sample_bound(const mplx_ctx *c, double limit) {
  const mplx_params &p = c->prm;
  double vbound;
  if ((p.control & 0x0f) == MPLX_VEL) vbound = c->u_absmax;
  else if (p.v_max > 0) vbound = p.v_max;
  else return 0;
  const double nf = std::ceil(vbound * p.dt / c->res) + 1.0;
  if (!(nf <= limit)) return 0;
  const int n_max = (int)nf;
  return n_max < 5 ? 5 : n_max;
}

TilePlan plan_tile(const mplx_ctx *c) {
  TilePlan t;
  const mplx_params &p = c->prm;
  if (p.control & 0x10) return t;
  if (c->has_pot) return t;
  if (c->nU > 1024 || c->nU < 1) return t;
  const int n_max = sample_bound(c, 63.0);
  if (!n_max) return t;
  const int cnt_max = n_max + 1;
  int npb = 1024 / c->nU;
  if (npb < 1) npb = 1;
  if (npb > 32) npb = 32;
  for (; npb >= 1; npb--) {
    const int tp = npb * c->nU;
    int uoff = 0;
    const size_t lds = mplx::tile_lds_bytes(tp, npb, tp * cnt_max, n_max, 4 * c->dim + 2, c->nU * c->udim, &uoff);
    if (lds <= 80 * 1024 || npb == 1) {
      if (lds > kLdsBudget - 64) return t;
      t.ok = true;
      t.npb = npb;
      t.tile_pairs = tp;
      t.wl_cap = tp * cnt_max;
      t.n_max = n_max;
      t.u_offset = uoff;
      t.grid = c->n_cus * (lds <= 53 * 1024 ? 3 : lds <= 80 * 1024 ? 2 : 1);
      return t;
    }
  }
  return t;
}

namespace {
struct GridPlan {
  bool ok = false;
  int ndp = 1, n_max = 0, rmax = 0, boxcap = 0, grid = 0, order = 0;
  int ulex = 0;
  bool gather = false, use_sat = true;
  bool lex = false;
};
struct PairPlan {
  bool ok = false;
  int rmax = 0, grid = 0;
};
enum OccKernel { kOccGrid = 0, kOccLex = 0x100, kOccPair = 0x200 };
}

static int resident_per_cu(const mplx_ctx *c, OccKernel kernel, int inst, int rows_per_pass, size_t lds) {
  if (lds > kLdsBudget) return 0;
  const int control = c->prm.control, key = control | kernel | (inst << 12);
  int nb = -1;
  for (const auto &e : c->grid_occ)
    if (e.control == key && e.pot == c->has_pot && e.lds == lds) nb = e.nb;
  if (nb < 0) {
    nb = kernel == kOccLex    ? mplx::lex_resident_blocks(c->dim, control, inst, lds)
         : kernel == kOccPair ? mplx::pair_resident_blocks(c->dim, control, inst, lds)
                              : mplx::grid_resident_blocks(c->dim, control, c->has_pot, lds);
    if (c->grid_occ.size() >= 8) c->grid_occ.clear();
    c->grid_occ.push_back({key, c->has_pot, lds, nb});
    if (getenv("MPLX_GRID_VERBOSE"))
      fprintf(stderr, "mplx: %s kernel control 0x%x pot %d rows/pass %d: LDS %zu B per workgroup, %d workgroups resident per CU\n",
              kernel == kOccLex ? "lex" : kernel == kOccPair ? "pair" : "grid", control, (int)c->has_pot, rows_per_pass, lds, nb);
  }
  const int by_lds = (int)(kLdsBudget / lds);
  return (nb > 0 && nb < by_lds) ? nb : by_lds;
}

static GridPlan plan_grid(const mplx_ctx *c) {
  GridPlan g;
  const mplx_params &p = c->prm;
  const bool yaw = (p.control & 0x10) != 0;
  if (yaw && (c->udim != c->dim + 1 || c->u_nd[3] < 1)) return g;
  if (!c->u_factored || c->nU < 1) return g;
  const bool lex_only = c->u_wide || c->nU > 1024;
  if (lex_only && (c->nU > 8192 || !c->u_lex || c->tune.no_lex || !c->tune.grid_lex || yaw || c->has_pot ||
                   !mplx::lex_covers(c->dim, p.control)))
    return g;
  const int n_max = sample_bound(c, 61.0);
  if (!n_max) return g;
  int ndp = 1;
  for (int i = 0; i < c->dim; i++) ndp = c->u_nd[i] > ndp ? c->u_nd[i] : ndp;
  const int order = control_order(p.control);
  const int ym = (yaw ? (p.wyaw > 0 ? 2 : 1) : 0) | ((c->has_pot && p.gradient_weight != 0) ? 4 : 0), ndy = yaw ? c->u_nd[3] : 0;
  int rmax = 4, boxcap = (c->dim == 3) ? (n_max + 3) * (n_max + 3) : 4 * (n_max + 3);
  if (boxcap < 64) boxcap = 64;
  if (boxcap > 1024) boxcap = 1024;
  if (c->has_pot) boxcap = 64;
  g.gather = false;
  if (c->tune.grid_gather >= 0) g.gather = c->tune.grid_gather != 0;
  g.use_sat = (!g.gather || c->has_pot) && order <= 2;
  if (c->tune.grid_sat >= 0) g.use_sat = c->tune.grid_sat != 0;
  if (g.gather) boxcap = 64;
  if (c->tune.grid_rmax > 0) rmax = c->tune.grid_rmax;
  if (c->tune.grid_boxcap > 0) boxcap = c->tune.grid_boxcap;
  if (rmax < 1) rmax = 1;
  const int ulex = (c->u_lex && !c->tune.no_lex && (yaw || c->udim == c->dim)) ? 1 : 0;
  g.lex = ulex && !yaw && !c->has_pot && !g.gather && c->tune.grid_lex && mplx::lex_covers(c->dim, p.control);
  if (lex_only && !g.lex) return GridPlan();
  auto lds_of = [&](int rm) -> size_t {
    return g.lex ? mplx::lex_lds_bytes(c->dim, order, ndp, c->nU, n_max, rm, boxcap)
                 : mplx::grid_lds_bytes(c->dim, order, c->nU, ndp, n_max, rm, boxcap, ym, ndy, ulex);
  };
  while (rmax > 1 && lds_of(rmax) > 80 * 1024) rmax--;
  const int wpb = g.lex ? mplx::lex_waves_per_block() : mplx::grid_waves_per_block();
  if (mplx::lex_waves_per_block() != mplx::grid_waves_per_block()) return GridPlan();
  auto resident = [&](int rm, size_t *lds_out) -> int {
    *lds_out = lds_of(rm);
    return g.lex ? resident_per_cu(c, kOccLex, ndp, rm, *lds_out) : resident_per_cu(c, kOccGrid, 0, rm, *lds_out);
  };
  const int cap = c->tune.grid_waves_per_cu > 0 ? c->tune.grid_waves_per_cu : (g.lex ? 24 : 16);
  size_t lds = 0;
  int per_cu = resident(rmax, &lds);
  if (per_cu < 1) return g;
  if (g.lex && c->dim == 3 && c->tune.grid_boxcap <= 0 && per_cu * wpb < cap) {
    const int keep = boxcap;
    boxcap = (boxcap * 25 / 32) & ~31;
    size_t lds_b = 0;
    const int per_cu_b = boxcap >= 256 ? resident(rmax, &lds_b) : 0;
    if (per_cu_b > per_cu) { per_cu = per_cu_b; lds = lds_b; }
    else boxcap = keep;
  }
  if (c->tune.grid_rmax <= 0 && rmax == 4 && per_cu * wpb < cap) {
    size_t lds3 = 0;
    const int per_cu3 = resident(3, &lds3);
    if (per_cu3 > per_cu) { rmax = 3; per_cu = per_cu3; lds = lds3; }
  }
  if (per_cu * wpb > cap) per_cu = cap / wpb;
  if (per_cu < 1) per_cu = 1;
  g.ok = true;
  g.ndp = ndp;
  g.n_max = n_max;
  g.rmax = rmax;
  g.boxcap = boxcap;
  g.order = order;
  g.ulex = ulex;
  g.grid = c->n_cus * per_cu;
  if (c->tune.grid_blocks > 0) g.grid = c->tune.grid_blocks;
  return g;
}

static PairPlan plan_pair(const mplx_ctx *c, const GridPlan &gp, const mplx::GridArgs &a) {
  PairPlan pp;
  if (!(a.live != nullptr && c->has_pot && a.ulex && !gp.lex && !c->tune.no_pair && a.yaw.tab == nullptr &&
        mplx::pair_covers(c->dim, c->prm.control) && c->dim * gp.ndp <= 16 && a.ndy <= mplx::pair_max_yaw_rates()))
    return pp;
  int per_cu = 0;
  for (int rm = c->tune.pair_rmax > 0 ? c->tune.pair_rmax : 3; rm >= 1 && per_cu < 1; rm--) {
    const size_t lds = mplx::pair_lds_bytes(c->dim, gp.order, c->nU, gp.ndp, gp.n_max, rm, c->prm.wyaw > 0, a.ndy);
    per_cu = resident_per_cu(c, kOccPair, a.ndy, rm, lds);
    pp.rmax = rm;
  }
  if (per_cu < 1) return pp;
  const int cap = c->tune.pair_wg_per_cu > 0 ? c->tune.pair_wg_per_cu : 3;
  if (per_cu > cap) per_cu = cap;
  pp.grid = c->n_cus * per_cu;
  pp.ok = true;
  return pp;
}

static int grid_work(mplx_ctx *c, mplx::GridArgs *a) {
  a->work = nullptr;
  a->work_zero = nullptr;
  a->work_chunk = 1;
  const int64_t wpb = mplx::grid_waves_per_block();
  const int64_t n_wg = (a->n_nodes + wpb - 1) / wpb;
  const int64_t W = (n_wg < (int64_t)a->grid_limit ? n_wg : (int64_t)a->grid_limit) * wpb;
  if (c->tune.grid_static || a->n_nodes <= W) return MPLX_OK;
  const size_t set_bytes = (size_t)mplx::kWorkCounters * 128;
  if (!c->work_counter.p) {
    if (int rc = ensure(c, c->work_counter, 2 * set_bytes)) return rc;
    HIP_TRY(c, hipMemsetAsync(c->work_counter.p, 0, 2 * set_bytes, c->stream));
    c->work_parity = 0;
  }
  a->work = (unsigned int *)((char *)c->work_counter.p + (c->work_parity ? set_bytes : 0));
  a->work_zero = (unsigned int *)((char *)c->work_counter.p + (c->work_parity ? 0 : set_bytes));
  int64_t per_wave = a->n_nodes / W, ck = per_wave / 16;
  if (ck < 1) ck = 1;
  if (ck > 8) ck = 8;
  if (c->tune.grid_chunk > 0) ck = c->tune.grid_chunk;
  a->work_chunk = (int32_t)ck;
  a->work_blocked = c->tune.grid_blocked ? 1 : 0;
  return MPLX_OK;
}

int launch_grid(mplx_ctx *c, mplx::GridArgs *a) {
  if (int rc = grid_work(c, a)) return rc;
  const hipError_t e = a->lex ? mplx::launch_expand_lex(c->dim, c->prm.control, *a, c->stream)
                              : mplx::launch_expand_grid(c->dim, c->prm.control, *a, c->stream);
  c->last_grid_lex = a->lex != 0;
  c->last_grid_pair = false;
  if (e != hipSuccess) {
    if (a->work) {
      (void)hipStreamSynchronize(c->stream);
      release(c->work_counter);
    }
    return fail(c, MPLX_ERR_HIP, "expand_grid_kernel launch failed: %s", hipGetErrorString(e));
  }
  if (a->work) c->work_parity ^= 1;
  return MPLX_OK;
}

static int launch_pair(mplx_ctx *c, const PairPlan &pp, const mplx::GridArgs &a) {
  mplx::GridArgs b = a;
  b.rmax = pp.rmax;
  b.grid_limit = pp.grid;
  b.work = nullptr;
  b.work_zero = nullptr;
  const hipError_t e = mplx::launch_expand_pair(c->dim, c->prm.control, b, c->stream);
  if (e != hipSuccess) return fail(c, MPLX_ERR_HIP, "expand_pair_kernel launch failed: %s", hipGetErrorString(e));
  c->last_grid_lex = false;
  c->last_grid_pair = true;
  return MPLX_OK;
}

static int prescreen(mplx_ctx *c, const GridPlan &gp, mplx::GridArgs *a) {
  const bool yaw = (c->prm.control & 0x10) != 0;
  const int64_t n_nodes = a->n_nodes;
  const int64_t ps_min = c->tune.prescreen_min > 0 ? c->tune.prescreen_min : (int64_t)4 * gp.grid * mplx::grid_waves_per_block();
  if (!(yaw && gp.order >= 2 && c->prm.yaw_max > 0 && c->tune.prescreen_min >= 0 && n_nodes >= ps_min && n_nodes < 0x7fffffffLL))
    return MPLX_OK;
  if (int rc = ensure(c, c->live_list, (size_t)n_nodes * 4)) return rc;
  if (!c->live_ctr.p) {
    if (int rc = ensure(c, c->live_ctr, 256)) return rc;
    HIP_TRY(c, hipMemsetAsync(c->live_ctr.p, 0, 256, c->stream));
    c->live_parity = 0;
  }
  int32_t *live = (int32_t *)c->live_list.p;
  uint32_t *live_n = (uint32_t *)c->live_ctr.p + (c->live_parity ? 32 : 0);
  uint32_t *live_zero = (uint32_t *)c->live_ctr.p + (c->live_parity ? 0 : 32);
  const hipError_t pe = mplx::launch_grid_prescreen(c->dim, c->prm.control, *a, live, live_n, live_zero, c->stream);
  if (pe != hipSuccess) {
    (void)hipStreamSynchronize(c->stream);
    release(c->live_ctr);
    return fail(c, MPLX_ERR_HIP, "grid_prescreen_kernel launch failed: %s", hipGetErrorString(pe));
  }
  c->live_parity ^= 1;
  a->live = live;
  a->live_n = live_n;
  return MPLX_OK;
}

static int rebuild_sat(mplx_ctx *c) {
  c->sat_stale = false;
  const int d2p = c->dim == 3 ? c->mdim[2] + 1 : 2;
  const int64_t sat_n = (int64_t)(c->mdim[0] + 1) * (c->mdim[1] + 1) * d2p;
  if (c->tune.no_sat || sat_n * 4 > (16LL << 30)) return MPLX_OK;
  if (int rc = ensure(c, c->sat, (size_t)sat_n * 4)) return rc;
  HIP_TRY(c, mplx::launch_build_sat(c->dim, (const uint32_t *)c->blk.p, c->mdim, (uint32_t *)c->sat.p, c->stream));
  c->sat_ok = true;
  return MPLX_OK;
}

int ensure_blocked_bits(mplx_ctx *c) {
  if (c->blk_ok) return MPLX_OK;
  c->sat_stale = false;
  const int64_t words = (c->n_cells + 31) >> 5;
  if (int rc = ensure(c, c->blk, (size_t)words * 4)) return rc;
  HIP_TRY(c, mplx::launch_build_blocked_bits((const int8_t *)(c->has_pot ? c->pot.p : c->map.p),
                                             c->has_region ? (const uint32_t *)c->region_bits.p : nullptr, c->n_cells,
                                             c->has_pot ? 1 : 0, (uint32_t *)c->blk.p, c->stream));
  c->sat_ok = false;
  if (int rc = rebuild_sat(c)) return rc;
  c->blk_ok = true;
  return MPLX_OK;
}

int ensure_tables(mplx_ctx *c) {
  if (c->tables_ok && c->tab_dt == c->prm.dt && c->tab_res == c->res) return MPLX_OK;
  const size_t bytes = kTcntOffset + 64 + 64;
  if (int rc = ensure(c, c->tables, bytes)) return rc;
  double *ttab = (double *)c->tables.p;
  unsigned char *tcnt = (unsigned char *)c->tables.p + kTcntOffset;
  double *rec = (double *)((unsigned char *)c->tables.p + kTcntOffset + 64);
  HIP_TRY(c, hipMemsetAsync(c->tables.p, 0, bytes, c->stream));
  HIP_TRY(c, mplx::launch_make_tables(c->prm.dt, c->res, ttab, tcnt, rec, c->stream));
  HIP_TRY(c, hipMemcpyAsync(c->recips, rec, 3 * sizeof(double), hipMemcpyDeviceToHost, c->stream));
  HIP_TRY(c, hipStreamSynchronize(c->stream));
  c->tab_dt = c->prm.dt;
  c->tab_res = c->res;
  c->tables_ok = true;
  return MPLX_OK;
}

static uint32_t const_zero_rows(int dim, int control) {
  const int order = control_order(control);
  uint32_t m = 0;
  for (int b = order + 1; b <= 3; b++)
    for (int i = 0; i < dim; i++) m |= 1u << (b * dim + i);
  if (!(control & 0x10)) m |= 1u << (4 * dim);
  return m;
}

static mplx::GridArgs grid_args(mplx_ctx *c, const GridPlan &gp, const double *d_nodes, int64_t n_nodes, int64_t node_stride,
                                const mplx_succ_lists *o, uint32_t skip) {
  mplx::GridArgs a{};
  set_env(c, &a);
  set_tables(c, &a);
  set_lists(c, o, &a);
  a.blk = (const uint32_t *)c->blk.p;
  a.blk_words = (c->n_cells + 31) >> 5;
  a.pot = c->has_pot ? (const int8_t *)c->pot.p : nullptr;
  a.pot_w = c->prm.potential_weight;
  a.grad_w = c->has_pot ? c->prm.gradient_weight : 0.0;
  const bool yaw = (c->prm.control & 0x10) != 0;
  a.sat = (c->sat_ok && gp.order <= 3 && !(yaw && c->prm.wyaw > 0) && !c->tune.no_sat && gp.use_sat)
              ? (const uint32_t *)c->sat.p : nullptr;
  a.gather = gp.gather ? 1 : 0;
  a.yaw_max = c->prm.yaw_max; a.wyaw = c->prm.wyaw; a.ndy = yaw ? c->u_nd[3] : 0;
  a.uvals = (const double *)c->uvals.p + (c->u_wide ? 4 * 16 : 0);
  a.uval_stride = c->u_wide ? 32 : 16;
  a.uidx = (const uint32_t *)c->uidx.p;
  a.nd0 = c->u_nd[0]; a.nd1 = c->u_nd[1]; a.nd2 = c->u_nd[2];
  a.ndp = gp.ndp;
  a.ulex = gp.ulex;
  a.nU = c->nU;
  a.nodes = d_nodes; a.n_nodes = n_nodes; a.node_stride = node_stride;
  a.n_max = gp.n_max; a.rmax = gp.rmax; a.boxcap = gp.boxcap; a.grid_limit = gp.grid;
  a.lex = gp.lex ? 1 : 0;
  a.dbg = c->tune.dbg;
  a.l_pad = line_pad(c, a.l_nstride);
  a.l_zrows = skip;
  a.post = post_of(c, o);
  return a;
}

static int lists_grid(mplx_ctx *c, const GridPlan &gp, const double *d_nodes, int64_t n_nodes, int64_t node_stride,
                      const mplx_succ_lists *o, uint32_t skip) {
  if (int rc = ensure_tables(c)) return rc;
  if (int rc = ensure_blocked_bits(c)) return rc;
  if (c->sat_stale && n_nodes >= 4096)
    if (int rc = rebuild_sat(c)) return rc;
  mplx::GridArgs a = grid_args(c, gp, d_nodes, n_nodes, node_stride, o, skip);
  if (int rc = yaw_slot(c, &a.yaw)) return rc;
  if (int rc = prescreen(c, gp, &a)) return rc;
  arm_done(c, &a.done);
  const PairPlan pp = plan_pair(c, gp, a);
  if (int rc = pp.ok ? launch_pair(c, pp, a) : launch_grid(c, &a)) return rc;
  c->done_armed = a.done.flag != nullptr;
  if (a.yaw.amb) {
    mplx_ctx::YawPending p;
    p.kind = 0;
    p.g = a;
    p.g.live = nullptr;
    p.g.live_n = nullptr;
    p.g.done = {};
    c->yaw_pending.push_back(p);
  }
  c->last_route = MPLX_ROUTE_GRID;
  return MPLX_OK;
}

static int lists_tile(mplx_ctx *c, const TilePlan &tp, const double *d_nodes, int64_t n_nodes, int64_t node_stride,
                      const mplx_succ_lists *o) {
  if (int rc = ensure_tables(c)) return rc;
  mplx::TileArgs a = tile_args(c, tp, d_nodes, n_nodes, node_stride, o);
  arm_done(c, &a.done);
  HIP_TRY(c, mplx::launch_expand_tile(c->dim, c->prm.control, a, c->stream));
  c->done_armed = a.done.flag != nullptr;
  c->last_route = MPLX_ROUTE_TILE;
  return MPLX_OK;
}

static int lists_dense(mplx_ctx *c, const double *d_nodes, int64_t n_nodes, int64_t node_stride, const mplx_succ_lists *o) {
  const int F = 4 * c->dim + 2;
  c->done_armed = false;
  const int64_t max_chunk_slots = (int64_t)(256u << 20) / (F * 8 + 21);
  int64_t chunk_nodes = max_chunk_slots / c->nU;
  if (chunk_nodes < 1) chunk_nodes = 1;
  if (chunk_nodes > n_nodes) chunk_nodes = n_nodes;
  const int64_t cs = chunk_nodes * c->nU;
  if (int rc = ensure(c, c->d_status, (size_t)cs)) return rc;
  if (int rc = ensure(c, c->d_cost, (size_t)cs * 8)) return rc;
  if (int rc = ensure(c, c->d_hash, (size_t)cs * 8)) return rc;
  if (int rc = ensure(c, c->d_state, (size_t)cs * 8 * F)) return rc;
  if (int rc = ensure(c, c->d_iters, (size_t)cs * 4)) return rc;
  for (int64_t k0 = 0; k0 < n_nodes; k0 += chunk_nodes) {
    const int64_t nk = (n_nodes - k0) < chunk_nodes ? (n_nodes - k0) : chunk_nodes;
    mplx_succ d{};
    d.status = (uint8_t *)c->d_status.p;
    d.cost = (double *)c->d_cost.p;
    d.hash = (uint64_t *)c->d_hash.p;
    d.state = o->state ? (double *)c->d_state.p : nullptr;
    d.state_stride = cs;
    d.iters = o->iters ? (int32_t *)c->d_iters.p : nullptr;
    mplx::ExpandArgs a = expand_args(c, d_nodes + k0, nk, node_stride, &d);
    if (int rc = yaw_slot(c, &a.yaw)) return rc;
    HIP_TRY(c, mplx::launch_expand(c->dim, c->prm.control, a, c->stream));
    if (a.yaw.amb) {
      mplx_ctx::YawPending p;
      p.kind = 1;
      p.e = a;
      c->yaw_pending.push_back(p);
      if (int rc = resolve_pending(c)) return rc;
    }
    mplx::CompactArgs ca{};
    ca.status = d.status; ca.cost = d.cost; ca.hash = d.hash; ca.state = d.state; ca.iters = d.iters;
    ca.chunk_slots = cs; ca.nU = c->nU; ca.n_fields = F;
    ca.node_offset = k0; ca.n_nodes_chunk = nk;
    set_lists(c, o, &ca);
    HIP_TRY(c, mplx::launch_compact_lists(ca, c->stream));
  }
  if (o->heur || o->flags) {
    if (!o->hash || !o->state)
      return fail(c, MPLX_ERR_STATE, "heur / flags rows on the DENSE lists route need the hash and state rows as well");
    mplx::PostArgs pa{};
    pa.count = o->count;
    pa.hash = o->hash;
    pa.state = o->state;
    pa.sstride = o->state_stride;
    pa.n_nodes = n_nodes;
    pa.nstride = list_stride(c, o);
    for (int i = 0; i < F; i++) pa.goal[i] = c->goal_fuse.goal[i];
    pa.goal_hash = c->goal_fuse.goal_hash;
    pa.w = c->goal_fuse.w; pa.v_max = c->goal_fuse.v_max;
    pa.tol_pos = c->goal_fuse.tol_pos; pa.tol_vel = c->goal_fuse.tol_vel; pa.tol_acc = c->goal_fuse.tol_acc; pa.tol_yaw = c->goal_fuse.tol_yaw;
    pa.heur = o->heur;
    pa.flags = o->flags;
    HIP_TRY(c, mplx::launch_post_lists(c->dim, pa, c->stream));
  }
  c->last_route = MPLX_ROUTE_DENSE;
  return MPLX_OK;
}

int lists_device(mplx_ctx *c, const double *d_nodes, int64_t n_nodes, int64_t node_stride,
                 const mplx_succ_lists *o, uint32_t *zero_rows) {
  const int F = 4 * c->dim + 2;
  const int route = c->lists_route;
  const uint32_t const_rows = const_zero_rows(c->dim, c->prm.control);
  const uint32_t in_rows = zero_rows ? (*zero_rows & ((1u << F) - 1u)) : 0u;
  const uint32_t skip = o->state ? (in_rows & const_rows) : 0u;
  c->last_zero_rows = 0;
  if (zero_rows) *zero_rows = o->state ? 0u : (in_rows & const_rows);
  if ((o->heur || o->flags) && !c->has_goal)
    return fail(c, MPLX_ERR_STATE, "the heur / flags rows of the lists need a goal: call mplx_set_goal first");
  const GridPlan gp = (route == MPLX_ROUTE_AUTO || route == MPLX_ROUTE_GRID) ? plan_grid(c) : GridPlan();
  if (route == MPLX_ROUTE_GRID && !gp.ok)
    return fail(c, MPLX_ERR_STATE, "lists route GRID does not cover this configuration");
  bool grid = gp.ok;
  if (route == MPLX_ROUTE_AUTO && grid && n_nodes <= 512 && c->nU >= 512 && plan_tile(c).ok) grid = false;
  if (grid && n_nodes >= 0x7fffffffLL - 4096) grid = false;
  if (grid) {
    if (int rc = lists_grid(c, gp, d_nodes, n_nodes, node_stride, o, skip)) return rc;
    c->last_zero_rows = skip;
    if (zero_rows && o->state) *zero_rows = skip;
    return MPLX_OK;
  }
  const TilePlan tp = (route == MPLX_ROUTE_AUTO || route == MPLX_ROUTE_TILE) ? plan_tile(c) : TilePlan();
  if (route == MPLX_ROUTE_TILE && !tp.ok)
    return fail(c, MPLX_ERR_STATE, "lists route TILE does not cover this configuration");
  if (tp.ok) return lists_tile(c, tp, d_nodes, n_nodes, node_stride, o);
  return lists_dense(c, d_nodes, n_nodes, node_stride, o);
}

static int lists_entry(mplx_ctx *c, const char *fn, const double *d_nodes, int64_t n_nodes, int64_t node_stride,
                       const mplx_succ_lists *d_out, uint32_t *zero_rows) {
  if (!c) return MPLX_ERR_ARG;
  if (!d_out || !d_out->count || n_nodes < 0 || node_stride < n_nodes || (!d_nodes && n_nodes > 0))
    return fail(c, MPLX_ERR_ARG, "%s: bad arguments", fn);
  if (int rc = ctx_ready(c)) return rc;
  if (n_nodes == 0) return MPLX_OK;
  if (d_out->node_stride != 0 && d_out->node_stride < c->nU)
    return fail(c, MPLX_ERR_ARG, "%s: node_stride %lld < nU %d", fn, (long long)d_out->node_stride, c->nU);
  if (d_out->state && d_out->state_stride < n_nodes * list_stride(c, d_out))
    return fail(c, MPLX_ERR_ARG, "%s: state_stride < n_nodes*node_stride", fn);
  if (int rc = bind_device(c)) return rc;
  return lists_device(c, d_nodes, n_nodes, node_stride, d_out, zero_rows);
}

}

using namespace mplx_detail;

extern "C" {

int mplx_expand_lists_device(mplx_ctx *c, const double *d_nodes, int64_t n_nodes, int64_t node_stride,
                             const mplx_succ_lists *d_out) {
  return lists_entry(c, "mplx_expand_lists_device", d_nodes, n_nodes, node_stride, d_out, nullptr);
}

int mplx_expand_lists_device_z(mplx_ctx *c, const double *d_nodes, int64_t n_nodes, int64_t node_stride,
                               const mplx_succ_lists *d_out, uint32_t *zero_rows) {
  if (!zero_rows || *zero_rows == 0) return mplx_expand_lists_device(c, d_nodes, n_nodes, node_stride, d_out);
  return lists_entry(c, "mplx_expand_lists_device_z", d_nodes, n_nodes, node_stride, d_out, zero_rows);
}

int mplx_lists_zero_fill(mplx_ctx *c, const mplx_succ_lists *d_lists, uint32_t *zero_rows) {
  if (!c) return MPLX_ERR_ARG;
  if (!d_lists || !zero_rows) return fail(c, MPLX_ERR_ARG, "mplx_lists_zero_fill: NULL argument");
  *zero_rows = 0;
  if (!d_lists->state) return MPLX_OK;
  if (d_lists->state_stride <= 0) return fail(c, MPLX_ERR_ARG, "mplx_lists_zero_fill: state_stride <= 0");
  if (int rc = bind_device(c)) return rc;
  if (int rc = resolve_pending(c)) return rc;
  const int F = 4 * c->dim + 2;
  HIP_TRY(c, hipMemsetAsync(d_lists->state, 0, (size_t)F * (size_t)d_lists->state_stride * 8, c->stream));
  *zero_rows = (1u << F) - 1u;
  return MPLX_OK;
}

}
```

### motion_primitive_library_amd/csrc/mplx_api.cpp

```cpp
#include "mplx_ctx.h"
#include "host_planner.hpp"

#include <cmath>
#include <cstdio>
#include <cstdlib>
#include <cstring>
#include <new>
#include <string>
#include <vector>

using namespace mplx_detail;

namespace mplx_detail {
std::string &create_error() {
  thread_local std::string e;
  return e;
}

int ctx_ready(mplx_ctx *c) {
  if (!c->has_map) return fail(c, MPLX_ERR_STATE, "mplx_set_map has not been called");
  if (!c->has_params) return fail(c, MPLX_ERR_STATE, "mplx_set_params has not been called");
  if (!c->has_U) return fail(c, MPLX_ERR_STATE, "mplx_set_controls has not been called");
  const int need = c->dim + ((c->prm.control & 0x10) ? 1 : 0);
  if (c->udim < need)
// ... 228 lines not shown
  if (!cells) {
    c->svc.streak = 0;
    if (int rc = mplx_detail::svc_stop(c)) return rc;
    c->blk_ok = c->blk_ok && !c->has_region;
    c->blk_epoch++;
    c->has_region = false;
    return MPLX_OK;
  }
  if (!c->has_map) return fail(c, MPLX_ERR_STATE, "mplx_set_region: set the map first");
  if (int rc = bind_device(c)) return rc;
  const size_t words = (size_t)((c->n_cells + 31) >> 5);
  if (int rc = ensure(c, c->region_bytes, (size_t)c->n_cells)) return rc;
  if (int rc = ensure(c, c->region_bits, words * 4)) return rc;
  HIP_TRY(c, hipMemcpyAsync(c->region_bytes.p, cells, (size_t)c->n_cells, hipMemcpyHostToDevice, c->stream));
  c->map_upload_bytes += (uint64_t)c->n_cells;
  HIP_TRY(c, mplx::launch_pack_region((const uint8_t *)c->region_bytes.p, (uint32_t *)c->region_bits.p,
                                      c->n_cells, c->stream));
  HIP_TRY(c, hipStreamSynchronize(c->stream));
  c->has_region = true;
  c->blk_ok = false;
  c->blk_epoch++;
  return MPLX_OK;
}

int mplx_set_params(mplx_ctx *c, const mplx_params *p) {
  if (!c) return MPLX_ERR_ARG;
  if (!p) return fail(c, MPLX_ERR_ARG, "mplx_set_params: NULL");
  if (!control_ok(p->control)) return fail(c, MPLX_ERR_ARG, "mplx_set_params: unknown control flag 0x%x", p->control);
  if (!(p->dt > 0)) return fail(c, MPLX_ERR_ARG, "mplx_set_params: dt must be > 0");
  if (int rc = resolve_pending(c)) return rc;
  if (int rc = mplx_detail::svc_stop(c)) return rc;
  c->prm = *p;
  c->has_params = true;
  return MPLX_OK;
}

int mplx_set_goal(mplx_ctx *c, const mplx_goal_spec *g) {
  if (!c) return MPLX_ERR_ARG;
  if (int rc = resolve_pending(c)) return rc;
  mplx::PostFuse f{};
  bool has = false;
  if (g) {
    if (int rc = mplx_detail::goal_fuse_of(c, "mplx_set_goal", g, &f)) return rc;
    has = true;
  }
  if (has != c->has_goal || std::memcmp(&f, &c->goal_fuse, sizeof(f)) != 0) {
    if (int rc = mplx_detail::svc_stop(c)) return rc;
    c->goal_fuse = f;
    c->has_goal = has;
  }
  c->goal_ctl[0] = g ? g->control : 0;
  c->goal_ctl[1] = g ? g->goal_control : 0;
  return MPLX_OK;
}

int mplx_set_controls(mplx_ctx *c, const double *U, int32_t nU, int32_t udim) {
  if (!c) return MPLX_ERR_ARG;
  if (!U || nU <= 0 || udim < c->dim || udim > c->dim + 1)
    return fail(c, MPLX_ERR_ARG, "mplx_set_controls: need U != NULL, nU > 0, udim in {%d,%d}", c->dim, c->dim + 1);
  MPLX_GUARD_BEGIN
  if (int rc = bind_device(c)) return rc;
  if (int rc = resolve_pending(c)) return rc;
  const size_t bytes = (size_t)nU * udim * sizeof(double);
  if (int rc = ensure(c, c->U, bytes)) return rc;
  HIP_TRY(c, hipMemcpyAsync(c->U.p, U, bytes, hipMemcpyHostToDevice, c->stream));
  HIP_TRY(c, hipStreamSynchronize(c->stream));
  c->nU = nU;
  c->udim = udim;
  c->h_U.assign(U, U + (size_t)nU * udim);
  c->u_absmax = 0;
  for (int32_t i = 0; i < nU; i++)
    for (int k = 0; k < c->dim; k++) {
      const double a = std::fabs(U[(size_t)i * udim + k]);
      if (a > c->u_absmax) c->u_absmax = a;
    }
  c->u_factored = true;
  c->u_wide = false;
  double vals32[4][32] = {};
  std::vector<uint32_t> packed((size_t)nU, 0u);
  c->u_nd[3] = 0;
  for (int k = 0; k < udim && c->u_factored; k++) {
    const int slot = k < c->dim ? k : 3;
    int n = 0;
    for (int32_t i = 0; i < nU; i++) {
      const double x = U[(size_t)i * udim + k];
      int j = 0;
      for (; j < n; j++)
        if (std::memcmp(&vals32[slot][j], &x, sizeof x) == 0) break;
      if (j == n) {
        if (n == 32) { c->u_factored = false; break; }
        vals32[slot][n++] = x;
      }
      packed[(size_t)i] |= (uint32_t)j << (8 * slot);
    }
    c->u_nd[slot] = n;
    if (n > 16) c->u_wide = true;
  }
  double vals[4][16] = {};
  for (int a4 = 0; a4 < 4; a4++) std::memcpy(vals[a4], vals32[a4], sizeof vals[a4]);
  c->u_lex = false;
  if (c->u_factored) {
    for (int k = c->dim; k < 3; k++) c->u_nd[k] = 0;
    int64_t prod = 1;
    for (int k = 0; k < c->dim; k++) prod *= c->u_nd[k];
    const int ny = udim > c->dim ? c->u_nd[3] : 1;
    prod *= ny;
    if (prod == nU) {
      c->u_lex = true;
      for (int32_t i = 0; i < nU && c->u_lex; i++) {
        int32_t r = i;
        uint32_t want = 0;
        if (udim > c->dim) { want |= (uint32_t)(r % ny) << 24; r /= ny; }
        for (int k = c->dim - 1; k >= 0; k--) { want |= (uint32_t)(r % c->u_nd[k]) << (8 * k); r /= c->u_nd[k]; }
        c->u_lex = want == packed[(size_t)i];
      }
    }
    if (c->u_wide && (!c->u_lex || udim != c->dim)) c->u_factored = false;
  }
  if (c->u_factored) {
    std::memcpy(c->h_uyaw, vals[3], sizeof c->h_uyaw);
    if (int rc = ensure(c, c->uvals, sizeof vals + sizeof vals32)) return rc;
    if (int rc = ensure(c, c->uidx, (size_t)nU * 4)) return rc;
    HIP_TRY(c, hipMemcpyAsync(c->uvals.p, vals, sizeof vals, hipMemcpyHostToDevice, c->stream));
    HIP_TRY(c, hipMemcpyAsync((char *)c->uvals.p + sizeof vals, vals32, sizeof vals32, hipMemcpyHostToDevice, c->stream));
    HIP_TRY(c, hipMemcpyAsync(c->uidx.p, packed.data(), (size_t)nU * 4, hipMemcpyHostToDevice, c->stream));
    HIP_TRY(c, hipStreamSynchronize(c->stream));
  }
  c->has_U = true;
  return MPLX_OK;
  MPLX_GUARD_END(c)
}

int mplx_expand_device(mplx_ctx *c, const double *d_nodes, int64_t n_nodes, int64_t node_stride,
                       const mplx_succ *d_out) {
  if (!c) return MPLX_ERR_ARG;
  if (!d_out || n_nodes < 0 || node_stride < n_nodes || (!d_nodes && n_nodes > 0))
    return fail(c, MPLX_ERR_ARG, "mplx_expand_device: bad arguments");
  if (int rc = ctx_ready(c)) return rc;
  if (n_nodes == 0) return MPLX_OK;
  const int64_t n_slots = n_nodes * c->nU;
  if (d_out->state && d_out->state_stride < n_slots)
    return fail(c, MPLX_ERR_ARG, "mplx_expand_device: state_stride %lld < n_slots %lld",
                (long long)d_out->state_stride, (long long)n_slots);
  if (int rc = bind_device(c)) return rc;
  mplx::ExpandArgs a = expand_args(c, d_nodes, n_nodes, node_stride, d_out);
  a.stream_out = 1;
  if (int rc = yaw_slot(c, &a.yaw)) return rc;
  HIP_TRY(c, mplx::launch_expand(c->dim, c->prm.control, a, c->stream));
  if (a.yaw.amb) {
    mplx_ctx::YawPending p;
    p.kind = 1;
    p.e = a;
    c->yaw_pending.push_back(p);
  }
  return MPLX_OK;
}

int mplx_expand(mplx_ctx *c, const double *h_nodes, int64_t n_nodes, int64_t node_stride,
                const mplx_succ *h_out) {
  if (!c) return MPLX_ERR_ARG;
  if (!h_out || n_nodes < 0 || node_stride < n_nodes || (!h_nodes && n_nodes > 0))
    return fail(c, MPLX_ERR_ARG, "mplx_expand: bad arguments");
  if (int rc = ctx_ready(c)) return rc;
  if (n_nodes == 0) return MPLX_OK;
  if (int rc = bind_device(c)) return rc;
  const int F = 4 * c->dim + 2;
  const int64_t n_slots = n_nodes * c->nU;
  if (h_out->state && h_out->state_stride < n_slots)
    return fail(c, MPLX_ERR_ARG, "mplx_expand: state_stride < n_slots");
  const size_t slots = (size_t)n_slots;
  StageLayout l;
  const size_t o_nodes = l.add((size_t)F * n_nodes * 8), o_status = l.add(h_out->status ? slots : 0),
               o_cost = l.add(h_out->cost ? slots * 8 : 0), o_hash = l.add(h_out->hash ? slots * 8 : 0),
               o_iters = l.add(h_out->iters ? slots * 4 : 0), o_state = l.add(h_out->state ? F * slots * 8 : 0);
  if (int rc = stage_commit(c, &l)) return rc;
  HIP_TRY(c, stage_in_rows(c, l.base + o_nodes, h_nodes, (size_t)node_stride * 8, (size_t)n_nodes * 8, F));
  mplx_succ d{};
  if (h_out->status) d.status = (uint8_t *)(l.base + o_status);
  if (h_out->cost) d.cost = (double *)(l.base + o_cost);
  if (h_out->hash) d.hash = (uint64_t *)(l.base + o_hash);
  if (h_out->iters) d.iters = (int32_t *)(l.base + o_iters);
  if (h_out->state) { d.state = (double *)(l.base + o_state); d.state_stride = n_slots; }
  mplx::ExpandArgs a = expand_args(c, (const double *)(l.base + o_nodes), n_nodes, n_nodes, &d);
  a.stream_out = 1;
  if (int rc = yaw_slot(c, &a.yaw)) return rc;
  HIP_TRY(c, mplx::launch_expand(c->dim, c->prm.control, a, c->stream));
  if (a.yaw.amb) {
    mplx_ctx::YawPending p;
    p.kind = 1;
    p.e = a;
    c->yaw_pending.push_back(p);
    if (int rc = mplx_detail::resolve_pending(c)) return rc;
  }
  HIP_TRY(c, stage_out(c, h_out->status, d.status, slots));
  HIP_TRY(c, stage_out(c, h_out->cost, d.cost, slots * 8));
  HIP_TRY(c, stage_out(c, h_out->hash, d.hash, slots * 8));
  HIP_TRY(c, stage_out(c, h_out->iters, d.iters, slots * 4));
  HIP_TRY(c, stage_out_rows(c, h_out->state, (size_t)h_out->state_stride * 8, d.state, slots * 8, F));
  HIP_TRY(c, hipStreamSynchronize(c->stream));
  return MPLX_OK;
}

int mplx_device_alloc(mplx_ctx *c, size_t bytes, void **dptr) {
  if (!c) return MPLX_ERR_ARG;
  if (!dptr) return fail(c, MPLX_ERR_ARG, "mplx_device_alloc: NULL");
  *dptr = nullptr;
  if (int rc = bind_device(c)) return rc;
  HIP_TRY(c, hipMalloc(dptr, bytes ? bytes : 1));
  return MPLX_OK;
}

int mplx_device_free(mplx_ctx *c, void *dptr) {
  if (!c) return MPLX_ERR_ARG;
  if (!dptr) return MPLX_OK;
  if (int rc = bind_device(c)) return rc;
  if (int rc = resolve_pending(c)) return rc;
  HIP_TRY(c, hipStreamSynchronize(c->stream));
  HIP_TRY(c, hipFree(dptr));
  return MPLX_OK;
}

int mplx_memcpy_h2d(mplx_ctx *c, void *dst, const void *src, size_t bytes) {
  if (!c) return MPLX_ERR_ARG;
  if (int rc = bind_device(c)) return rc;
  if (int rc = resolve_pending(c)) return rc;
  HIP_TRY(c, hipMemcpyAsync(dst, src, bytes, hipMemcpyHostToDevice, c->stream));
  HIP_TRY(c, hipStreamSynchronize(c->stream));
  return MPLX_OK;
}

int mplx_memcpy_d2h(mplx_ctx *c, void *dst, const void *src, size_t bytes) {
  if (!c) return MPLX_ERR_ARG;
  if (int rc = bind_device(c)) return rc;
  if (int rc = resolve_pending(c)) return rc;
  HIP_TRY(c, hipMemcpyAsync(dst, src, bytes, hipMemcpyDeviceToHost, c->stream));
  HIP_TRY(c, hipStreamSynchronize(c->stream));
  return MPLX_OK;
}

int mplx_memset(mplx_ctx *c, void *dst, int value, size_t bytes) {
  if (!c) return MPLX_ERR_ARG;
  if (int rc = bind_device(c)) return rc;
  if (int rc = resolve_pending(c)) return rc;
  HIP_TRY(c, hipMemsetAsync(dst, value, bytes, c->stream));
  return MPLX_OK;
}

int mplx_synchronize(mplx_ctx *c) {
  if (!c) return MPLX_ERR_ARG;
  if (int rc = bind_device(c)) return rc;
  HIP_TRY(c, hipStreamSynchronize(c->stream));
  return resolve_pending(c);
}

int mplx_timer_begin(mplx_ctx *c) {
  if (!c) return MPLX_ERR_ARG;
  if (int rc = bind_device(c)) return rc;
  HIP_TRY(c, hipEventRecord(c->ev0, c->stream));
  return MPLX_OK;
}

int mplx_timer_end(mplx_ctx *c, float *ms) {
  if (!c) return MPLX_ERR_ARG;
  if (!ms) return fail(c, MPLX_ERR_ARG, "mplx_timer_end: NULL");
  if (int rc = bind_device(c)) return rc;
  HIP_TRY(c, hipEventRecord(c->ev1, c->stream));
  HIP_TRY(c, hipEventSynchronize(c->ev1));
  HIP_TRY(c, hipEventElapsedTime(ms, c->ev0, c->ev1));
  return resolve_pending(c);
}

int mplx_selftest_math(mplx_ctx *c, int op, const double *a, const double *b, double *out, int64_t n) {
  if (!c) return MPLX_ERR_ARG;
  if (!a || !out || n < 0 || (op == 0 && !b) || op < 0 || op > 5)
    return fail(c, MPLX_ERR_ARG, "mplx_selftest_math: bad arguments");
  if (n == 0) return MPLX_OK;
  if (int rc = bind_device(c)) return rc;
  void *da = nullptr, *db = nullptr, *dout = nullptr;
  const size_t bytes = (size_t)n * sizeof(double);
  HIP_TRY(c, hipMalloc(&da, bytes));
  HIP_TRY(c, hipMalloc(&db, bytes));
  HIP_TRY(c, hipMalloc(&dout, bytes));
  HIP_TRY(c, hipMemcpyAsync(da, a, bytes, hipMemcpyHostToDevice, c->stream));
  HIP_TRY(c, hipMemcpyAsync(db, b ? b : a, bytes, hipMemcpyHostToDevice, c->stream));
  HIP_TRY(c, mplx::launch_math_probe(op, (const double *)da, (const double *)db, (double *)dout, n, c->stream));
  HIP_TRY(c, hipMemcpyAsync(out, dout, bytes, hipMemcpyDeviceToHost, c->stream));
  HIP_TRY(c, hipStreamSynchronize(c->stream));
  (void)hipFree(da);
  (void)hipFree(db);
  (void)hipFree(dout);
  return MPLX_OK;
}

int mplx_set_lists_route(mplx_ctx *c, int route) {
  if (!c) return MPLX_ERR_ARG;
  if (route < MPLX_ROUTE_AUTO || route > MPLX_ROUTE_GRID) return fail(c, MPLX_ERR_ARG, "mplx_set_lists_route: unknown route %d", route);
  c->lists_route = route;
  c->svc.streak = 0;
  return MPLX_OK;
}

int mplx_last_lists_route(const mplx_ctx *c) { return c ? c->last_route : MPLX_ERR_ARG; }
int mplx_last_lists_zero_rows(const mplx_ctx *c) { return c ? (int)c->last_zero_rows : MPLX_ERR_ARG; }
int mplx_last_grid_kernel(const mplx_ctx *c) {
  if (!c) return MPLX_ERR_ARG;
  if (c->last_route != MPLX_ROUTE_GRID) return MPLX_KERNEL_NONE;
  return c->last_grid_pair ? MPLX_KERNEL_PAIR : (c->last_grid_lex ? MPLX_KERNEL_LEX : MPLX_KERNEL_GRID);
}

int mplx_last_identity_form(const mplx_ctx *c) { return c ? c->last_identity_form : MPLX_ERR_ARG; }

int mplx_yaw_pin_stats(const mplx_ctx *c, int64_t *flagged_nodes, int64_t *fix_passes) {
  if (!c) return MPLX_ERR_ARG;
  if (flagged_nodes) *flagged_nodes = c->yaw_flagged;
  if (fix_passes) *fix_passes = c->yaw_fix_passes;
  return MPLX_OK;
}

int mplx_device_info(mplx_ctx *c, char *name, size_t cap, int32_t *compute_units) {
  if (!c) return MPLX_ERR_ARG;
  hipDeviceProp_t prop;
  HIP_TRY(c, hipGetDeviceProperties(&prop, c->device));
  if (name && cap) snprintf(name, cap, "%s (%s)", prop.name, prop.gcnArchName);
  if (compute_units) *compute_units = prop.multiProcessorCount;
  return MPLX_OK;
}

}
```

### motion_primitive_library_amd/csrc/mplx_ctx.h

```cpp
#ifndef MPLX_CTX_H
#define MPLX_CTX_H

#include "../../include/mplx.h"
#include "../../include/mplx_debug.h"
#include "../../include/mplx_open.h"
#include "../../include/mplx_traj.h"
#include "mplx_internal.h"

#include <cstdarg>
#include <cstdio>
#include <exception>
#include <new>
#include <string>
#include <vector>

struct mplx_table;
struct mplx_reserve;

namespace mplx_detail {

struct DevBuf {
  void *p = nullptr;
  size_t cap = 0;
};

std::string &create_error();

}

struct mplx_ctx {
  int dim = 0;
  int device = 0;
  hipStream_t stream = nullptr;
  hipEvent_t ev0 = nullptr, ev1 = nullptr;
  std::string err;

  mplx_detail::DevBuf map, pot, region_bits, region_bytes, U;
  bool has_map = false, has_pot = false, has_region = false, has_params = false, has_U = false;
  bool has_goal = false;
  mplx::PostFuse goal_fuse{};
  int32_t goal_ctl[2] = {0, 0};
  int32_t mdim[3] = {1, 1, 1};
  double origin[3] = {0, 0, 0};
  double res = 0;
  int64_t n_cells = 0;
  uint64_t map_upload_bytes = 0;
  mplx_params prm{};
  int32_t nU = 0, udim = 0;
  double u_absmax = 0;
  mplx_detail::DevBuf uvals, uidx, blk, sat;
  bool sat_ok = false;
  mplx_detail::DevBuf post_keys;
  mplx_detail::DevBuf post_ws;
  mplx_detail::DevBuf ray_work;
  mplx_detail::DevBuf heur_ws;
  mplx_detail::DevBuf traj_tab;
  mplx_detail::DevBuf conflict_ws;
  mplx_detail::DevBuf prep_lut, prep_a, prep_b;
  bool blk_ok = false;
  uint64_t blk_epoch = 0;
  bool u_factored = false;
  bool u_wide = false;
  bool u_lex = false;
  int32_t u_nd[4] = {0, 0, 0, 0};
  struct Tuning {
    int grid_rmax = 0, grid_boxcap = 0, grid_blocks = 0;
    int grid_waves_per_cu = 0;
    int grid_gather = -1, grid_sat = -1;
    bool grid_lex = true;
    bool grid_static = false;
    int grid_chunk = 0;
    int grid_blocked = 0;
    int dbg = 0;
    bool no_pair = false;
    int pair_rmax = 0, pair_wg_per_cu = 0;
    int zero_copy = 1;
    int arena_kb = 0;
    bool no_sat = false, no_lex = false, no_line_pad = false;
    int prescreen_min = 0;
    bool yaw_pin = true;
    double yaw_margin = 0;
    int done_flag = 1;
    int service = 1;
    int service_idle_us = 500;
    int service_max_nodes = 256;
    int reserve_lanes = 0;
  } tune;
  int lists_route = MPLX_ROUTE_AUTO;
  int last_route = MPLX_ROUTE_AUTO;
  uint32_t last_zero_rows = 0;
  bool last_grid_pair = false;
  bool last_grid_lex = false;
  int n_cus = 256;

  mplx_detail::DevBuf tables;
  bool tables_ok = false;
  double tab_dt = 0, tab_res = 0;
  double recips[3] = {0, 0, 0};
  mplx_detail::DevBuf d_status, d_cost, d_hash, d_state, d_iters;
  mplx_detail::DevBuf s_arena;
  void *h_arena = nullptr;
  size_t h_arena_cap = 0;
  uint64_t *done_host = nullptr;
  mplx_detail::DevBuf done_count;
  uint64_t done_seq = 0;
  bool want_done = false;
  bool done_armed = false;
  int64_t done_waits = 0, done_timeouts = 0;
  struct Service {
    bool running = false;
    bool disabled = false;
    int streak = 0;
    hipStream_t stream = nullptr;
    mplx::SvcMailbox *mb = nullptr;
    char *block = nullptr;
    size_t block_cap = 0;
    mplx_detail::DevBuf dev;
    uint32_t seq = 0;
    int64_t cap = 0, S = 0;
    unsigned rows = 0;
    int workgroups = 0;
    int64_t requests = 0, launches = 0, failures = 0;
  } svc;
  mplx_detail::DevBuf pk_dev[2], pk_offs;
  void *pk_pin[2] = {nullptr, nullptr};
  size_t pk_pin_cap = 0;
  hipEvent_t pk_ev[2] = {nullptr, nullptr};
  std::vector<int64_t> pk_hoffs;
  void *pk_hb = nullptr;
  size_t pk_hb_cap = 0;
  struct YawPending {
    int kind = 0;
    mplx::GridArgs g{};
    mplx::ExpandArgs e{};
  };
  std::vector<YawPending> yaw_pending;
  int32_t *yaw_any_host = nullptr;
  int32_t *id_ovf_host = nullptr;
  bool sat_stale = false;
  int id_backoff = 0;
  int last_identity_form = 0;
  mplx_detail::DevBuf yaw_ring, yaw_ids, yaw_tab;
  std::vector<double> h_U;
  double h_uyaw[16] = {0};
  int64_t yaw_flagged = 0, yaw_fix_passes = 0;
  mplx_detail::DevBuf live_list;
  mplx_detail::DevBuf live_ctr;
  int live_parity = 0;
  mplx_detail::DevBuf work_counter;
  int work_parity = 0;
  struct GridOcc { int control; bool pot; size_t lds; int nb; };
  mutable std::vector<GridOcc> grid_occ;
  void *comm = nullptr;
  int comm_rank = 0, comm_world = 1;
  mplx_detail::DevBuf comm_meta;
  std::vector<double> h_state;
};

struct mplx_field {
  mplx_ctx *c = nullptr;
  mplx_detail::DevBuf dist, active, counter;
  mplx_detail::DevBuf bits;
  std::vector<mplx_open *> users;
  int32_t F = 0;
  int64_t n_cells = 0;
  uint64_t epoch = 0;
  int64_t passes = 0;
};

namespace mplx_detail {

inline int fail(mplx_ctx *c, int code, const char *fmt, ...) {
  char buf[512];
  va_list ap;
  va_start(ap, fmt);
  vsnprintf(buf, sizeof buf, fmt, ap);
  va_end(ap);
  if (c) c->err = buf; else create_error() = buf;
  return code;
}

#define HIP_TRY(c, expr)                                                                   \
  do {                                                                                     \
    hipError_t e__ = (expr);                                                               \
    if (e__ != hipSuccess)                                                                 \
      return mplx_detail::fail((c), MPLX_ERR_HIP, "%s failed: %s (%s:%d)", #expr, hipGetErrorString(e__), \
                  __FILE__, __LINE__);                                                     \
  } while (0)

#define MPLX_GUARD_BEGIN try {
#define MPLX_GUARD_END(c)                                                                            \
  }                                                                                                  \
  catch (const std::bad_alloc &) { return mplx_detail::fail((c), MPLX_ERR_NOMEM, "out of host memory"); } \
  catch (const std::exception &e) { return mplx_detail::fail((c), MPLX_ERR_NOMEM, "unexpected exception: %s", e.what()); } \
  catch (...) { return mplx_detail::fail((c), MPLX_ERR_NOMEM, "unexpected exception"); }

int svc_stop(mplx_ctx *c);

inline int bind_device(mplx_ctx *c) {
  HIP_TRY(c, hipSetDevice(c->device));
  c->svc.streak = 0;
  if (c->svc.running) return svc_stop(c);
  return MPLX_OK;
}

inline int ensure(mplx_ctx *c, DevBuf &b, size_t bytes) {
  if (bytes <= b.cap) return MPLX_OK;
  if (b.p) {
    HIP_TRY(c, hipStreamSynchronize(c->stream));
    HIP_TRY(c, hipFree(b.p));
    b.p = nullptr;
    b.cap = 0;
  }
  HIP_TRY(c, hipMalloc(&b.p, bytes));
  b.cap = bytes;
  return MPLX_OK;
}

inline void release(DevBuf &b) {
  if (b.p) (void)hipFree(b.p);
  b.p = nullptr;
  b.cap = 0;
}

inline size_t align256(size_t bytes) { return (bytes + 255) & ~(size_t)255; }

struct StageLayout {
  size_t total = 0;
  char *base = nullptr;
  size_t add(size_t bytes) { const size_t at = total; total += align256(bytes); return at; }
};
inline int stage_commit(mplx_ctx *c, StageLayout *l) {
  if (int rc = ensure(c, c->s_arena, l->total)) return rc;
  l->base = (char *)c->s_arena.p;
  return MPLX_OK;
}
inline hipError_t stage_in(mplx_ctx *c, void *dev, const void *host, size_t bytes) {
  return hipMemcpyAsync(dev, host, bytes, hipMemcpyHostToDevice, c->stream);
}
inline hipError_t stage_in_rows(mplx_ctx *c, void *dev, const void *host, size_t src_stride, size_t width, size_t rows) {
  return hipMemcpy2DAsync(dev, width, host, src_stride, width, rows, hipMemcpyHostToDevice, c->stream);
}
inline hipError_t stage_out(mplx_ctx *c, void *host, const void *dev, size_t bytes) {
  return host ? hipMemcpyAsync(host, dev, bytes, hipMemcpyDeviceToHost, c->stream) : hipSuccess;
}
inline hipError_t stage_out_rows(mplx_ctx *c, void *host, size_t dst_stride, const void *dev, size_t width, size_t rows) {
  return host ? hipMemcpy2DAsync(host, dst_stride, dev, width, width, rows, hipMemcpyDeviceToHost, c->stream) : hipSuccess;
}

struct PackedLists {
  int64_t total = 0;
  const int32_t *count = nullptr;
  const int64_t *offs = nullptr;
  const double *cost = nullptr;
  const uint64_t *hash = nullptr;
  const int32_t *action = nullptr;
  const double *state = nullptr;
  const double *heur = nullptr;
};
int expand_lists_packed(mplx_ctx *c, const double *h_nodes, int64_t n_nodes, int64_t node_stride, bool want_state,
                        PackedLists *out, bool want_heur = false);

constexpr size_t kLdsBudget = 160 * 1024;
constexpr size_t kTcntOffset = 64 * 64 * 8;

inline int64_t list_stride(const mplx_ctx *c, const mplx_succ_lists *o) { return o->node_stride ? o->node_stride : c->nU; }

inline int line_pad(const mplx_ctx *c, int64_t stride) {
  return (stride % 32 == 0 && !c->tune.no_line_pad && c->nU >= mplx::kLinePadMinControls) ? 1 : 0;
}

inline int control_order(int control) {
  const int ctl = control & 0x0f;
  return ctl == MPLX_VEL ? 1 : ctl == MPLX_ACC ? 2 : ctl == MPLX_JRK ? 3 : 4;
}

int ctx_ready(mplx_ctx *c);

struct TilePlan {
  bool ok = false;
  int npb = 1, tile_pairs = 0, wl_cap = 0, n_max = 0, u_offset = 0, grid = 0;
};
TilePlan plan_tile(const mplx_ctx *c);
int ensure_tables(mplx_ctx *c);
int ensure_blocked_bits(mplx_ctx *c);
mplx::ExpandArgs expand_args(mplx_ctx *c, const double *d_nodes, int64_t n_nodes, int64_t node_stride, const mplx_succ *o);
mplx::TileArgs tile_args(mplx_ctx *c, const TilePlan &tp, const double *d_nodes, int64_t n_nodes, int64_t node_stride,
                         const mplx_succ_lists *o);
int launch_grid(mplx_ctx *c, mplx::GridArgs *a);
int lists_device(mplx_ctx *c, const double *d_nodes, int64_t n_nodes, int64_t node_stride, const mplx_succ_lists *o,
                 uint32_t *zero_rows = nullptr);

int yaw_slot(mplx_ctx *c, mplx::YawPin *y);
int resolve_pending(mplx_ctx *c, bool stream_is_idle = false);

int svc_request(mplx_ctx *c, const double *h_nodes, int64_t n_nodes, int64_t node_stride, const mplx_succ_lists *h_out,
                bool *handled, mplx_succ_lists *view);
int wait_small_launch(mplx_ctx *c);

int copy_lists_to_host(mplx_ctx *c, const mplx_succ_lists &d, const mplx_succ_lists *h_out, int64_t n_nodes);
void release_copy_buffers(mplx_ctx *c);


int table_open_args(mplx_table *t, const char *who, mplx_ctx **c, mplx::OpenArgs *a);
void table_observe(mplx_table *t);
int table_replan_args(mplx_table *t, const char *who, bool scratch, mplx_ctx **c, mplx::ReplanArgs *a, int32_t *time_keys = nullptr);
int reserve_table_args(mplx_reserve *r, const char *who, mplx_ctx **c, mplx::ReserveArgs *a);
int32_t zero_action(const mplx_ctx *c);
int table_reserve_args(mplx_table *t, const char *who, mplx_ctx **c, const int32_t **d_query, int32_t *n_queries, int64_t *cap);
int open_push(mplx_open *o, const char *who, const mplx_table_frontier *d_rows, int64_t n_max, double eps, int32_t sight, bool closed);
int open_park_args(mplx_open *o, const char *who, mplx_ctx **c, mplx_table **tab, mplx::OpenArgs *a);
void open_field_gone(mplx_open *o);

int traj_check_set(mplx_ctx *c, const char *who, const mplx_traj_set *s, const void *out);
int traj_build_table(mplx_ctx *c, const mplx_traj_set *s, mplx::TrajArgs *out);
void traj_set_rows(const mplx_ctx *c, const mplx_traj_set *s, StageLayout *l, size_t *starts, size_t *actions);
int traj_stage_set(mplx_ctx *c, const mplx_traj_set *s, const StageLayout &l, size_t starts, size_t actions, mplx_traj_set *d);

int goal_fuse_of(mplx_ctx *c, const char *who, const mplx_goal_spec *g, mplx::PostFuse *out);
int goal_sight_rows(mplx_ctx *c, const mplx_succ_lists *d_lists, int64_t n_nodes, const int32_t *d_row_query,
                    const mplx::PostFuse *d_goals, double tol, uint8_t *d_flags);

}
#endif
```

### motion_primitive_library_amd/env.py

```python
import ctypes as C

import numpy as np

from . import _abi
from .rows import (DeviceArray, DeviceArrayView, _alloc, _device_ptr, Rollouts, Rays, TrajInfo, TrajSamples,
                   TrajTraverse, SolveOut, LoadOut, PolyLimits, LambdaRows, Conflicts, ConflictResult)
from .poly import PolyTrajSet, ShortcutResult, _conflict_in, _conflict_steps, _conflict_host_out

VEL, ACC, JRK, SNP = 0x01, 0x03, 0x07, 0x0F
VELxYAW, ACCxYAW, JRKxYAW, SNPxYAW = 0x11, 0x13, 0x17, 0x1F

SLOT_SKIP_SAME, SLOT_FINITE, SLOT_BLOCKED, SLOT_SKIP_DYN = 0, 1, 2, 3
ROLLOUT_BAD_ACTION, ROLLOUT_HEADING_BAND = _abi.ROLLOUT_BAD_ACTION, _abi.ROLLOUT_HEADING_BAND
RAY_LEFT_MAP, RAY_HIT, RAY_BAD, RAY_TRUNCATED = _abi.RAY_LEFT_MAP, _abi.RAY_HIT, _abi.RAY_BAD, _abi.RAY_TRUNCATED
FLAG_GOAL_BLOCKED = _abi.FLAG_GOAL_BLOCKED
TRAJ_EMPTY, TRAJ_BAD_ACTION, TRAJ_BAD = _abi.TRAJ_EMPTY, _abi.TRAJ_BAD_ACTION, _abi.TRAJ_BAD
TRAJ_COMMAND, TRAJ_WAYPOINT = _abi.TRAJ_COMMAND, _abi.TRAJ_WAYPOINT
SOLVE_EMPTY, SOLVE_BAD_TIME, SOLVE_SINGULAR = _abi.SOLVE_EMPTY, _abi.SOLVE_BAD_TIME, _abi.SOLVE_SINGULAR
LIMITS_REFERENCE, LIMITS_ALL_ROOTS = _abi.LIMITS_REFERENCE, _abi.LIMITS_ALL_ROOTS
EXCEED_VEL, EXCEED_ACC, EXCEED_JRK = _abi.EXCEED_VEL, _abi.EXCEED_ACC, _abi.EXCEED_JRK
SHORTCUT_BAD_CHAIN = _abi.SHORTCUT_BAD_CHAIN
USE_POS, USE_VEL, USE_ACC = _abi.USE_POS, _abi.USE_VEL, _abi.USE_ACC
SCALE_REFERENCE, SCALE_ROBUST = _abi.SCALE_REFERENCE, _abi.SCALE_ROBUST
LAMBDA_BAD_POINTS, LAMBDA_NOT_POSITIVE, LAMBDA_MAX_SEGS = _abi.LAMBDA_BAD_POINTS, _abi.LAMBDA_NOT_POSITIVE, _abi.LAMBDA_MAX_SEGS
# ... 951 lines not shown
        self._flush()
        control = int(self._p.control if control is None else control)
        so = _solve_order(control)
        K = int(n_prob)
        i = _abi.SolveIn()
        i.waypoints, i.n_prob, i.w_max = _device_ptr(waypoints), K, int(w_max)
        i.wp_stride = K if wp_stride is None else int(wp_stride)
        if n_wp is not None:
            i.n_wp = _device_ptr(n_wp)
        if dts is not None:
            i.dts, i.dt_stride = _device_ptr(dts), K if dt_stride is None else int(dt_stride)
        i.v = float(v)
        if v_arr is not None:
            i.v_arr = _device_ptr(v_arr)
        if wp_flags is not None:
            i.wp_flags, i.flag_stride = _device_ptr(wp_flags), K if flag_stride is None else int(flag_stride)
        i.control, i.yaw_control = control, int(yaw_control)
        if out is not None and (out.n != K or out.w_max != int(w_max) or out.so != so):
            raise ValueError("out was allocated for another problem count, w_max or control")
        o = out.c_struct() if out is not None else _abi.SolveOut()
        _abi.check(self._ctx, _abi.lib().mplx_solve_device(poly._h, C.byref(i), C.byref(o)))
        if poly._out is not None and poly._out is not out:
            poly._out.free()
        poly.n, poly.so, poly.n_wmax, poly._host, poly._out, poly.control = K, so, int(w_max), None, out, control
        poly._lambda = None
        return poly

    def alloc_poly_limits(self, n):
        return PolyLimits(self, n)

    def alloc_lambda_rows(self, n, w_max, count=0):
        return LambdaRows(self, n, w_max, count)

    def load_traj(self, coeff, dts, n_segs=None, control=None):
        self._flush()
        control = int(self._p.control if control is None else control)
        c = np.asarray(coeff, dtype=np.float64)
        if c.ndim == 3:
            c = c[..., None]
        if c.ndim != 4 or c.shape[1] not in (self.dim, self.dim + 1) or c.shape[2] != 6 or c.shape[0] < 1:
            raise ValueError("coeff must be [S >= 1][%d or %d][6][K]" % (self.dim, self.dim + 1))
        S, K = c.shape[0], c.shape[3]
        if c.shape[1] == self.dim:
            c = np.concatenate([c, np.zeros((S, 1, 6, K))], axis=1)
        c = np.ascontiguousarray(c)
        dts = np.ascontiguousarray(np.asarray(dts, dtype=np.float64).reshape(S, K))
        poly = PolyTrajSet(self, max(K, 1), S + 1)
        try:
            i = _abi.PolyLoadIn()
            i.n_prob, i.w_max, i.control = K, S + 1, control
            if n_segs is not None:
                n_segs = np.ascontiguousarray(np.broadcast_to(np.asarray(n_segs, dtype=np.int32), (K,)))
                i.n_segs = n_segs.ctypes.data
            i.dts, i.dt_stride, i.coeff, i.coeff_stride = dts.ctypes.data, K, c.ctypes.data, K
            host, o = LoadOut.host(self, K, S + 1)
            _abi.check(self._ctx, _abi.lib().mplx_poly_load(poly._h, C.byref(i), C.byref(o)))
            seg = np.arange(S)[:, None] < host["n_segs"][None, :]
            host["dts"] = np.where(seg, dts, 0.0)
            host["segments"] = np.where(seg[:, None, None, :], c, 0.0)
            poly.n, poly.so, poly.n_wmax, poly._host, poly.control = K, None, S + 1, host, control
            poly._lambda = None
            return poly
        except Exception:
            poly.free()
            raise

    def alloc_load_out(self, n, w_max):
        return LoadOut(self, n, w_max)

    def load_traj_resident(self, poly, coeff, dts, n_prob, w_max, n_segs=None, control=None, coeff_stride=None, dt_stride=None,
                           out=None):
        self._flush()
        control = int(self._p.control if control is None else control)
        K = int(n_prob)
        i = _abi.PolyLoadIn()
        i.n_prob, i.w_max, i.control = K, int(w_max), control
        if n_segs is not None:
            i.n_segs = _device_ptr(n_segs)
        i.dts, i.dt_stride = _device_ptr(dts), K if dt_stride is None else int(dt_stride)
        i.coeff, i.coeff_stride = _device_ptr(coeff), K if coeff_stride is None else int(coeff_stride)
        if out is not None and (out.n != K or out.w_max != int(w_max)):
            raise ValueError("out was allocated for another problem count or w_max")
        o = out.c_struct() if out is not None else _abi.PolyLoadOut()
        _abi.check(self._ctx, _abi.lib().mplx_poly_load_device(poly._h, C.byref(i), C.byref(o)))
        if poly._out is not None and poly._out is not out:
            poly._out.free()
        poly.n, poly.so, poly.n_wmax, poly._host, poly._out, poly.control = K, None, int(w_max), None, out, control
        poly._lambda = None
        return poly

    def shortcut_resident(self, states, n_query, w_max, n_wp=None, control=None, max_hop=None, stride=None):
        self._flush()
        control = int(self._p.control if control is None else control)
        so = _solve_order(control)
        Q, W = int(n_query), int(w_max)
        hop = W - 1 if max_hop is None else int(max_hop)
        if Q < 1 or W < 2 or hop < 1:
            raise ValueError("shortcut: needs Q >= 1, w_max >= 2 and max_hop >= 1")
        P = Q * (W - 1) * hop
        pairs, res = PolyTrajSet(self, P, 2), PolyTrajSet(self, Q, W)
        shapes = {"status": ((Q,), np.uint8), "n_keep": ((Q,), np.int32), "keep": ((W, Q), np.int32), "cost": ((Q,), np.float64),
                  "chain_cost": ((Q,), np.float64), "edge_cost": ((Q, W - 1, hop), np.float64)}
        bufs = {}
        try:
            pair_out = SolveOut(self, P, 2, so)
            pairs._out = pair_out
            i, o = _abi.ShortcutIn(), _abi.ShortcutOut()
            i.states, i.n_query, i.w_max, i.control, i.max_hop = _device_ptr(states), Q, W, control, hop
            i.stride = Q if stride is None else int(stride)
            if n_wp is not None:
                i.n_wp = _device_ptr(n_wp)
            for key, (shape, dt) in shapes.items():
                bufs[key] = DeviceArray(self, int(np.prod(shape)) * np.dtype(dt).itemsize)
                setattr(o, key, bufs[key].ptr)
            o.keep_stride = Q
            po = pair_out.c_struct()
            o.pair_out = C.pointer(po)
            _abi.check(self._ctx, _abi.lib().mplx_shortcut_device(pairs._h, res._h, C.byref(i), C.byref(o)))
            self.synchronize()
            rows = {key: bufs[key].download(dt, shape) for key, (shape, dt) in shapes.items()}
            pairs.n, pairs.so, pairs.n_wmax, pairs.control = P, so, 2, control
            res.n, res.so, res.n_wmax, res.control = Q, None, W, control
            info = res.info(want_states=True)
            S = info["n_segs"]
            taus = np.where(np.arange(W)[:, None] <= S[None, :], info["seg_state"][self.n_fields - 1], 0.0) * (S > 0)[None, :]
            res._host = {"status": info["status"], "n_segs": S, "total_time": info["total_time"], "taus": taus}
            return ShortcutResult(res, pairs, hop, rows)
        except Exception:
            pairs.free()
            res.free()
            raise
        finally:
            for b in bufs.values():
                b.free()

    def shortcut(self, states, n_wp=None, control=None, max_hop=None):
        st = np.ascontiguousarray(np.asarray(states, dtype=np.float64))
        if st.ndim == 2:
            st = st[:, :, None]
        if st.ndim != 3 or st.shape[0] != self.n_fields:
            raise ValueError("states must be [%d][w_max][Q]" % self.n_fields)
        W, Q = st.shape[1], st.shape[2]
        d_st = DeviceArray(self, max(st.nbytes, 8))
        d_n = None
        try:
            d_st.upload(st)
            if n_wp is not None:
                n_wp = np.ascontiguousarray(np.broadcast_to(np.asarray(n_wp, dtype=np.int32), (Q,)))
                d_n = DeviceArray(self, n_wp.nbytes)
                d_n.upload(n_wp)
            return self.shortcut_resident(d_st, Q, W, n_wp=d_n, control=control, max_hop=max_hop)
        finally:
            d_st.free()
            if d_n is not None:
                d_n.free()

    def connect(self, p1_rows, p2_rows, T, control=None):
        a, b = (np.asarray(x, dtype=np.float64).reshape(self.n_fields, -1) for x in (p1_rows, p2_rows))
        K = a.shape[1]
        wp = np.ascontiguousarray(np.stack([a, b], axis=1))
        dts = np.broadcast_to(np.asarray(T, dtype=np.float64), (K,)).reshape(1, K)
        flags = np.full((2, K), USE_POS | USE_VEL | USE_ACC, np.uint8)
        return self.solve_traj(wp, dts=dts, control=control, wp_flags=flags)

    def alloc_table(self, capacity, slots_log2=0, n_queries=1):
        from .table import NodeTable
        return NodeTable(self, capacity, slots_log2, n_queries)

    def alloc_table_frontier(self, capacity):
        from .table import TableFrontier
        return TableFrontier(self, capacity)

    def cost_to_come(self, starts, g=None, g_max=float("inf"), max_rounds=None, capacity=1 << 16, lists_stride=None,
                     max_frontier=None):
        from .table import NodeTable, TableFrontier
        self._flush()
        fcap = int(capacity if max_frontier is None else max_frontier)
        tab = NodeTable(self, capacity)
        cur, nxt = TableFrontier(self, fcap), TableFrontier(self, fcap)
        lists = self.alloc_lists(fcap, want_state=True, stride=lists_stride)
        try:
            def check(where):
                status = tab.stats()[1]
                if status:
                    raise RuntimeError("cost_to_come: table status %d %s (1 nodes full, 2 probe full, 4 frontier full): "
                                       "raise capacity / max_frontier" % (status, where))
            count = tab.seed(starts, g, frontier=cur)
            check("after seeding")
            rounds = 0
            while count > 0 and (max_rounds is None or rounds < max_rounds):
                self.expand_lists_resident(cur, lists, n_nodes=count)
                count = tab.relax(lists, cur.id, cur.g, g_max, frontier=nxt, n_nodes=count)
                rounds += 1
                check("in round %d" % rounds)
                cur, nxt = nxt, cur
        except Exception:
            tab.free()
            raise
        finally:
            for b in (cur, nxt, lists):
                b.free()
        return tab, rounds

    def alloc_open(self, table):
        from .search import OpenSet
        return OpenSet(self, table)

    def alloc_field(self):
        from .search import GoalField
        return GoalField(self)

    def search(self, start, goal_row, eps=1.0, delta=None, g_max=float("inf"), max_rounds=None, max_expand=None,
               capacity=1 << 16, max_frontier=None, lists_stride=None, sight=True, tol_pos=0.5, tol_vel=-1.0, tol_acc=-1.0,
               tol_yaw=-1.0, w=None, v_max=None, start_g=0.0, prior=None, avoid=None, t0=0.0, radius=None, ignore_group=-1,
               time_keys=None, wait=False, park_goal=False, field=None, field_of_query=None, heur=None):
        from .search import run_search
        return run_search(self, start, goal_row, prior=prior, eps=eps, delta=delta, g_max=g_max, max_rounds=max_rounds,
                          max_expand=max_expand, capacity=capacity, max_frontier=max_frontier, lists_stride=lists_stride,
                          sight=sight, tol_pos=tol_pos, tol_vel=tol_vel, tol_acc=tol_acc, tol_yaw=tol_yaw, w=w, v_max=v_max,
                          start_g=start_g, avoid=avoid, t0=t0, radius=radius, ignore_group=ignore_group, time_keys=time_keys,
                          wait=wait, park_goal=park_goal, field=field, field_of_query=field_of_query, heur=heur)

    def search_many(self, starts, goal_rows, eps=1.0, delta=None, g_max=float("inf"), max_rounds=None, max_expand=None,
                    capacity=1 << 16, max_frontier=None, lists_stride=None, sight=True, tol_pos=0.5, tol_vel=-1.0,
                    tol_acc=-1.0, tol_yaw=-1.0, w=None, v_max=None, start_g=0.0, priors=None, avoid=None, t0=0.0, radius=None,
                    ignore_group=-1, time_keys=None, wait=False, park_goal=False, field=None, field_of_query=None, heur=None):
        from .search import run_search_many
        return run_search_many(self, starts, goal_rows, priors=priors, eps=eps, delta=delta, g_max=g_max, max_rounds=max_rounds,
                               max_expand=max_expand, capacity=capacity, max_frontier=max_frontier, lists_stride=lists_stride,
                               sight=sight, tol_pos=tol_pos, tol_vel=tol_vel, tol_acc=tol_acc, tol_yaw=tol_yaw, w=w,
                               v_max=v_max, start_g=start_g, avoid=avoid, t0=t0, radius=radius, ignore_group=ignore_group,
                               time_keys=time_keys, wait=wait, park_goal=park_goal, field=field, field_of_query=field_of_query,
                               heur=heur)

    def _heur_goal(self, goal_row, goal_control, w, v_max):
        goal = np.ascontiguousarray(goal_row, dtype=np.float64)
        if goal.shape != (self.n_fields,):
            raise ValueError("goal_row must have %d entries" % self.n_fields)
        g = _abi.GoalSpec()
        g.goal, g.control, g.goal_control = goal.ctypes.data, int(self._p.control), int(goal_control)
        g.w = float(self._p.w if w is None else w)
        g.v_max = float(self._p.v_max if v_max is None else v_max)
        g.tol_pos, g.tol_vel, g.tol_acc, g.tol_yaw = 0.0, -1.0, -1.0, -1.0
        return g, goal

    def heur_eval(self, states, goal_row, mode="robust", goal_control=0, w=None, v_max=None):
        self._flush()
        st = np.ascontiguousarray(np.asarray(states, dtype=np.float64).reshape(self.n_fields, -1))
        K = st.shape[1]
        g, keep = self._heur_goal(goal_row, goal_control, w, v_max)
        out = np.zeros(K)
        _abi.check(self._ctx, _abi.lib().mplx_heur_eval(self._ctx, C.byref(g), _abi.heur_mode(mode), st.ctypes.data, K, K,
                                                        out.ctypes.data))
        return out

    def heur_eval_resident(self, states, goal_row, out, n=None, stride=None, mode="robust", goal_control=0, w=None, v_max=None):
        self._flush()
        if hasattr(states, "state_stride"):
            ptr, stride, n = states.state.ptr, states.state_stride, (states.capacity if n is None else n)
        else:
            ptr = _device_ptr(states)
            if stride is None:
                raise ValueError("heur_eval_resident: a device buffer needs its stride")
            n = stride if n is None else n
        g, keep = self._heur_goal(goal_row, goal_control, w, v_max)
        _abi.check(self._ctx, _abi.lib().mplx_heur_eval_device(self._ctx, C.byref(g), _abi.heur_mode(mode), ptr, int(n),
                                                               int(stride), _device_ptr(out)))

    def alloc_reservations(self, trajs, step, n_steps=None, t0=None, radius=None, group=None, park=True):
        from .search import Reservations
        return Reservations(self, trajs, step, n_steps, t0, radius, group, park)

    def synchronize(self):
        _abi.check(self._ctx, _abi.lib().mplx_synchronize(self._ctx))

    def timer_begin(self):
        _abi.check(self._ctx, _abi.lib().mplx_timer_begin(self._ctx))

    def timer_end(self):
        ms = C.c_float()
        _abi.check(self._ctx, _abi.lib().mplx_timer_end(self._ctx, C.byref(ms)))
        return ms.value

    def set_lists_route(self, route):
        code = {"auto": _abi.ROUTE_AUTO, "dense": _abi.ROUTE_DENSE, "tile": _abi.ROUTE_TILE,
                "grid": _abi.ROUTE_GRID}[route] if isinstance(route, str) else int(route)
        _abi.check(self._ctx, _abi.lib().mplx_set_lists_route(self._ctx, code))

    def last_lists_route(self):
        code = _abi.lib().mplx_last_lists_route(self._ctx)
        return {_abi.ROUTE_AUTO: "none", _abi.ROUTE_DENSE: "dense", _abi.ROUTE_TILE: "tile",
                _abi.ROUTE_GRID: "grid"}[code]

    def debug_store_model(self, lists, n_nodes=None):
        self._flush()
        s = lists.c_struct()
        _abi.check(self._ctx, _abi.lib().mplx_debug_store_model(self._ctx, C.byref(s), lists.n_nodes if n_nodes is None else int(n_nodes)))
        if hasattr(lists, "zero_rows"):
            lists.zero_rows &= self.last_lists_zero_rows()

    def last_lists_zero_rows(self):
        return int(_abi.lib().mplx_last_lists_zero_rows(self._ctx))

    def last_grid_kernel(self):
        return {0: "none", 1: "grid", 2: "lex", 3: "pair"}[_abi.lib().mplx_last_grid_kernel(self._ctx)]

    def last_identity_form(self):
        return {0: "table", 1: "claimed", 2: "exact", 3: "claimed+exact"}[_abi.lib().mplx_last_identity_form(self._ctx)]

    def yaw_pin_stats(self):
        a, b = C.c_int64(), C.c_int64()
        _abi.check(self._ctx, _abi.lib().mplx_yaw_pin_stats(self._ctx, C.byref(a), C.byref(b)))
        return a.value, b.value

    def service(self, mode=-1):
        st = (C.c_int64 * 4)()
        _abi.check(self._ctx, _abi.lib().mplx_service(self._ctx, int(mode), st))
        return {"requests": st[0], "launches": st[1], "failures": st[2], "resident": bool(st[3])}

    def selftest_math(self, op, a, b=None):
        a = np.ascontiguousarray(a, dtype=np.float64)
        b = a if b is None else np.ascontiguousarray(b, dtype=np.float64)
        out = np.empty_like(a)
        _abi.check(self._ctx, _abi.lib().mplx_selftest_math(self._ctx, int(op), a.ctypes.data, b.ctypes.data,
                                                             out.ctypes.data, a.size))
        return out
```

Before: 109.3 billion pairs/s.

## Rebuild constant and derivable successor rows on host instead of copying them

When successor lists are copied back to host memory, rows that are known to be zero for the control order, the order-k rows (rebuilt from the action index and the control table), and the time row (parent time plus dt) are now filled on the host instead of travelling over the device-to-host link. The device launch also skips writing the constant-zero rows, and the action row is carried whenever it is cheaper than the order-k rows it replaces. This is meant to cut bytes moved per entry and device store traffic, at the cost of more host scatter work. It also adds a tunable chunk size, a copy-bytes query and optional timing instrumentation.

```diff
diff --git a/include/mplx.h b/include/mplx.h
--- a/include/mplx.h
+++ b/include/mplx.h
@@ -263,6 +263,7 @@
 int mplx_set_lists_route(mplx_ctx *ctx, int route);
 int mplx_last_lists_route(const mplx_ctx *ctx);
 int mplx_last_lists_zero_rows(const mplx_ctx *ctx);
+int64_t mplx_last_lists_copy_bytes(const mplx_ctx *ctx);
 enum { MPLX_KERNEL_NONE = 0, MPLX_KERNEL_GRID = 1, MPLX_KERNEL_LEX = 2,
        MPLX_KERNEL_PAIR = 3 };
 int mplx_last_grid_kernel(const mplx_ctx *ctx);
diff --git a/motion_primitive_library_amd/_abi.py b/motion_primitive_library_amd/_abi.py
--- a/motion_primitive_library_amd/_abi.py
+++ b/motion_primitive_library_amd/_abi.py
@@ -21,7 +21,7 @@
     "mplx_planner_create", "mplx_planner_destroy", "mplx_planner_attach_ctx", "mplx_planner_set_provider",
     "mplx_planner_set_map", "mplx_planner_edit_map", "mplx_planner_set_controls", "mplx_planner_configure", "mplx_planner_plan",
     "mplx_planner_trajectory", "mplx_planner_trajectory_end", "mplx_planner_closed_set", "mplx_planner_open_set", "mplx_planner_last_error", "mplx_planner_timing", "mplx_planner_set_prior_trajectory", "mplx_planner_set_prior_trajectory_potential", "mplx_planner_use_device_heuristic", "mplx_planner_set_lpastar", "mplx_planner_reset", "mplx_planner_linked_nodes", "mplx_planner_update_blocked_nodes", "mplx_planner_update_cleared_nodes", "mplx_planner_sub_state_space", "mplx_planner_set_edge_provider",
-    "mplx_selftest_math", "mplx_selftest_forward_state", "mplx_set_lists_route", "mplx_last_lists_route", "mplx_last_lists_zero_rows", "mplx_last_grid_kernel", "mplx_last_identity_form", "mplx_debug_store_model", "mplx_yaw_pin_stats", "mplx_service", "mplx_device_info",
+    "mplx_selftest_math", "mplx_selftest_forward_state", "mplx_set_lists_route", "mplx_last_lists_route", "mplx_last_lists_zero_rows", "mplx_last_lists_copy_bytes", "mplx_last_grid_kernel", "mplx_last_identity_form", "mplx_debug_store_model", "mplx_yaw_pin_stats", "mplx_service", "mplx_device_info",
 ]
 
 MAP_UTIL_SYMBOLS = ["mplx_map_dilate", "mplx_map_free", "mplx_map_cloud"]
@@ -420,6 +420,7 @@
         "mplx_set_lists_route": (C.c_int, [vp, C.c_int]),
         "mplx_last_lists_route": (C.c_int, [vp]),
         "mplx_last_lists_zero_rows": (C.c_int, [vp]),
+        "mplx_last_lists_copy_bytes": (C.c_int64, [vp]),
         "mplx_last_grid_kernel": (C.c_int, [vp]),
         "mplx_last_identity_form": (C.c_int, [vp]),
         "mplx_debug_store_model": (C.c_int, [vp, C.POINTER(SuccLists), i64]),
diff --git a/motion_primitive_library_amd/build.py b/motion_primitive_library_amd/build.py
--- a/motion_primitive_library_amd/build.py
+++ b/motion_primitive_library_amd/build.py
@@ -7,7 +7,7 @@
 CSRC = os.path.join(HERE, "csrc")
 LIB = os.path.join(CSRC, "libmplx.so")
 SOURCES = ["expand_kernel.hip", "expand_tile_kernel.hip", "expand_grid_kernel.hip", "expand_lex_kernel.hip", "expand_pair_kernel.hip", "map_prep_kernel.hip", "map_prep_api.cpp", "map_util_kernel.hip", "map_util_api.cpp", "rollout_kernel.hip", "rollout_api.cpp", "ray_kernel.hip", "ray_api.cpp", "traj_kernel.hip", "traj_api.cpp", "solve_kernel.hip", "solve_api.cpp", "limits_kernel.hip", "limits_api.cpp", "scale_kernel.hip", "scale_api.cpp", "conflict_kernel.hip", "conflict_api.cpp", "reserve_kernel.hip", "reserve_api.cpp", "wait_kernel.hip", "wait_api.cpp", "table_kernel.hip", "table_api.cpp", "open_kernel.hip", "open_api.cpp", "field_kernel.hip", "field_api.cpp", "heur_kernel.hip", "heur_api.cpp", "replan_kernel.hip", "replan_api.cpp", "post_kernel.hip", "identity_kernel.hip", "post_api.cpp", "edge_kernel.hip", "edge_api.cpp", "mplx_api.cpp", "lists_route.cpp", "yaw_pin.cpp", "lists_host.cpp", "planner_capi.cpp", "pack_kernel.hip", "store_model_kernel.hip", "lists_copy_api.cpp", "pack_api.cpp", "comm_api.cpp"]
-HEADERS = ["mplx_internal.h", "mplx_ctx.h", "mplx_device_common.h", "mplx_pair_device.h", "mplx_grid_common.h", "mplx_poly.h", "mplx_traj_device.h", "mplx_limits_math.h", "mplx_scale_math.h", "mplx_heur_math.h", "host_planner.hpp", "host_lpastar.hpp", os.path.join("..", "..", "include", "mplx.h"), os.path.join("..", "..", "include", "mplx_debug.h"), os.path.join("..", "..", "include", "mplx_map_util.h"), os.path.join("..", "..", "include", "mplx_rollout.h"), os.path.join("..", "..", "include", "mplx_ray.h"), os.path.join("..", "..", "include", "mplx_traj.h"), os.path.join("..", "..", "include", "mplx_table.h"), os.path.join("..", "..", "include", "mplx_open.h"), os.path.join("..", "..", "include", "mplx_multi.h"), os.path.join("..", "..", "include", "mplx_replan.h"), os.path.join("..", "..", "include", "mplx_replan_timed.h"), os.path.join("..", "..", "include", "mplx_prior.h"), os.path.join("..", "..", "include", "mplx_solve.h"), os.path.join("..", "..", "include", "mplx_limits.h"), os.path.join("..", "..", "include", "mplx_scale.h"), os.path.join("..", "..", "include", "mplx_conflict.h"), os.path.join("..", "..", "include", "mplx_reserve.h"), os.path.join("..", "..", "include", "mplx_wait.h"), os.path.join("..", "..", "include", "mplx_field.h"), os.path.join("..", "..", "include", "mplx_heur.h")]
+HEADERS = ["mplx_internal.h", "mplx_ctx.h", "lists_host_rows.h", "mplx_device_common.h", "mplx_pair_device.h", "mplx_grid_common.h", "mplx_poly.h", "mplx_traj_device.h", "mplx_limits_math.h", "mplx_scale_math.h", "mplx_heur_math.h", "host_planner.hpp", "host_lpastar.hpp", os.path.join("..", "..", "include", "mplx.h"), os.path.join("..", "..", "include", "mplx_debug.h"), os.path.join("..", "..", "include", "mplx_map_util.h"), os.path.join("..", "..", "include", "mplx_rollout.h"), os.path.join("..", "..", "include", "mplx_ray.h"), os.path.join("..", "..", "include", "mplx_traj.h"), os.path.join("..", "..", "include", "mplx_table.h"), os.path.join("..", "..", "include", "mplx_open.h"), os.path.join("..", "..", "include", "mplx_multi.h"), os.path.join("..", "..", "include", "mplx_replan.h"), os.path.join("..", "..", "include", "mplx_replan_timed.h"), os.path.join("..", "..", "include", "mplx_prior.h"), os.path.join("..", "..", "include", "mplx_solve.h"), os.path.join("..", "..", "include", "mplx_limits.h"), os.path.join("..", "..", "include", "mplx_scale.h"), os.path.join("..", "..", "include", "mplx_conflict.h"), os.path.join("..", "..", "include", "mplx_reserve.h"), os.path.join("..", "..", "include", "mplx_wait.h"), os.path.join("..", "..", "include", "mplx_field.h"), os.path.join("..", "..", "include", "mplx_heur.h")]
 ARCH = "gfx950"
 
 
diff --git a/motion_primitive_library_amd/csrc/lists_copy_api.cpp b/motion_primitive_library_amd/csrc/lists_copy_api.cpp
--- a/motion_primitive_library_amd/csrc/lists_copy_api.cpp
+++ b/motion_primitive_library_amd/csrc/lists_copy_api.cpp
@@ -1,6 +1,7 @@
 #include "mplx_ctx.h"
 
 #include <atomic>
+#include <chrono>
 #include <cstring>
 #include <thread>
 
@@ -8,14 +9,12 @@
 
 namespace {
 
-struct Row {
-  const void *dev;
-  char *host;
-  int es;
-  int64_t host_node_stride;
-};
-
 constexpr size_t kChunkBytes = 32u << 20;
+size_t chunk_bytes(const mplx_ctx *c) {
+  if (c->tune.arena_kb <= 0) return kChunkBytes;
+  const size_t tuned = (size_t)c->tune.arena_kb << 14;
+  return tuned < kChunkBytes ? tuned : kChunkBytes;
+}
 
 int ensure_pinned(mplx_ctx *c, size_t bytes) {
   if (bytes <= c->pk_pin_cap) return MPLX_OK;
@@ -32,20 +31,6 @@
 struct Chunk {
   int64_t node0, node1, off0, entries;
 };
-
-void scatter(const Row *rows, int n_rows, const int64_t *row_off, const char *pin, const int32_t *count,
-             const int64_t *offs, const Chunk &ch, int64_t a, int64_t b) {
-  for (int r = 0; r < n_rows; r++) {
-    const int es = rows[r].es;
-    const char *src = pin + row_off[r];
-    for (int64_t k = a; k < b; k++) {
-      const int cnt = count[k];
-      if (cnt > 0)
-        std::memcpy(rows[r].host + (size_t)k * rows[r].host_node_stride * es, src + (size_t)(offs[k] - ch.off0) * es,
-                    (size_t)cnt * es);
-    }
-  }
-}
 
 }
 
@@ -64,23 +49,18 @@
   c->pk_hb_cap = 0;
 }
 
-int copy_lists_to_host(mplx_ctx *c, const mplx_succ_lists &d, const mplx_succ_lists *h, int64_t n_nodes) {
-  const int F = 4 * c->dim + 2;
+int copy_lists_to_host(mplx_ctx *c, const mplx_succ_lists &d, const mplx_succ_lists *h, int64_t n_nodes,
+                       const double *h_nodes, int64_t h_node_stride) {
   const int64_t S = list_stride(c, &d);
   HIP_TRY(c, hipMemcpyAsync(h->count, d.count, (size_t)n_nodes * 4, hipMemcpyDeviceToHost, c->stream));
   HIP_TRY(c, hipStreamSynchronize(c->stream));
-  Row rows[mplx::kPackRows];
-  int n_rows = 0;
-  if (h->cost) rows[n_rows++] = {d.cost, (char *)h->cost, 8, S};
-  if (h->hash) rows[n_rows++] = {d.hash, (char *)h->hash, 8, S};
-  if (h->state)
-    for (int f = 0; f < F; f++)
-      rows[n_rows++] = {d.state + (size_t)f * d.state_stride, (char *)(h->state + (size_t)f * h->state_stride), 8, S};
-  if (h->action) rows[n_rows++] = {d.action, (char *)h->action, 4, S};
-  if (h->iters) rows[n_rows++] = {d.iters, (char *)h->iters, 4, S};
+  c->pk_last_bytes = n_nodes * 4;
+  const HostRowPlan plan = plan_host_rows(c->dim, c->prm.control, d, *h, S, c->h_U.data(), c->udim, h_nodes, h_node_stride, c->prm.dt);
+  const HostRow *rows = plan.rows;
+  const HostRowSource &src = plan.src;
+  const int n_rows = plan.n_rows, n_wire = plan.n_wire, made_bpe = plan.made_bpe;
+  const int bpe = plan.wire_bpe;
   if (n_rows == 0) return MPLX_OK;
-  int bpe = 0;
-  for (int r = 0; r < n_rows; r++) bpe += rows[r].es;
 
   std::vector<int64_t> &offs = c->pk_hoffs;
   offs.resize((size_t)n_nodes + 1);
@@ -94,7 +74,8 @@
   }
   offs[(size_t)n_nodes] = total;
   if (total == 0) return MPLX_OK;
-  size_t cap = kChunkBytes;
+  c->pk_last_bytes += total * bpe;
+  size_t cap = chunk_bytes(c);
   if ((size_t)max_cnt * bpe > cap) cap = (size_t)max_cnt * bpe;
   if ((size_t)total * bpe < cap) cap = (size_t)total * bpe;
   cap = align256(cap);
@@ -115,16 +96,16 @@
     a = b;
   }
   const int n_chunks = (int)chunks.size();
-  std::vector<int64_t> row_off((size_t)n_chunks * n_rows);
+  std::vector<int64_t> row_off((size_t)n_chunks * n_wire);
   for (int i = 0; i < n_chunks; i++) {
     int64_t o = 0;
-    for (int r = 0; r < n_rows; r++) {
-      row_off[(size_t)i * n_rows + r] = o;
-      o += chunks[(size_t)i].entries * rows[r].es;
-    }
-  }
-
-  int n_thr = (int)(((size_t)total * bpe) >> 23);
+    for (int w = 0; w < n_wire; w++) {
+      row_off[(size_t)i * n_wire + w] = o;
+      o += chunks[(size_t)i].entries * plan.wire_es[w];
+    }
+  }
+
+  int n_thr = (int)(((size_t)total * (bpe + made_bpe)) >> 23);
   const int hw = (int)std::thread::hardware_concurrency();
   if (n_thr > 15) n_thr = 15;
   if (hw > 0 && n_thr > hw - 1) n_thr = hw - 1;
@@ -138,7 +119,7 @@
     const Chunk &ch = chunks[(size_t)i];
     const int64_t n = ch.node1 - ch.node0;
     const int64_t a = ch.node0 + n * part / parts, b = ch.node0 + n * (part + 1) / parts;
-    scatter(rows, n_rows, &row_off[(size_t)i * n_rows], (const char *)c->pk_pin[i & 1], count, offs.data(), ch, a, b);
+    scatter_rows(rows, n_rows, &row_off[(size_t)i * n_wire], (const char *)c->pk_pin[i & 1], count, offs.data(), ch.off0, src, a, b);
   };
   std::vector<std::thread> helpers;
   try {
@@ -169,12 +150,12 @@
   auto issue = [&](int i) -> hipError_t {
     const Chunk &ch = chunks[(size_t)i];
     mplx::PackArgs a{};
-    for (int r = 0; r < n_rows; r++) {
-      a.src[r] = rows[r].dev;
-      a.dst_off[r] = row_off[(size_t)i * n_rows + r];
-      a.es[r] = rows[r].es;
-    }
-    a.n_rows = n_rows;
+    for (int w = 0; w < n_wire; w++) {
+      a.src[w] = plan.dev[w];
+      a.dst_off[w] = row_off[(size_t)i * n_wire + w];
+      a.es[w] = plan.wire_es[w];
+    }
+    a.n_rows = n_wire;
     a.node_stride = S;
     a.count = d.count;
     a.offs = (const int64_t *)c->pk_offs.p;
@@ -189,20 +170,31 @@
     }
     return hipEventRecord(c->pk_ev[i & 1], c->stream);
   };
+#ifdef MPLX_COPY_TIMING
+  double t_link = 0, t_host = 0;
+  auto now_ms = [] { return std::chrono::duration<double, std::milli>(std::chrono::steady_clock::now().time_since_epoch()).count(); };
+#define MPLX_COPY_TIMED(acc, stmt) { const double t0__ = now_ms(); stmt; acc += now_ms() - t0__; }
+#else
+#define MPLX_COPY_TIMED(acc, stmt) { stmt; }
+#endif
   for (int i = 0; i <= n_chunks && rc == MPLX_OK; i++) {
     hipError_t e = hipSuccess;
     if (i < n_chunks) e = issue(i);
-    if (e == hipSuccess && i >= 1) e = hipEventSynchronize(c->pk_ev[(i - 1) & 1]);
+    if (e == hipSuccess && i >= 1) MPLX_COPY_TIMED(t_link, e = hipEventSynchronize(c->pk_ev[(i - 1) & 1]))
     if (e != hipSuccess) {
       rc = fail(c, MPLX_ERR_HIP, "copy of the successor lists failed: %s", hipGetErrorString(e));
       break;
     }
     if (i >= 1) {
       ready.store(i, std::memory_order_release);
-      share(i - 1, 0);
-      while (done.load(std::memory_order_acquire) < i * n_thr) std::this_thread::yield();
-    }
-  }
+      MPLX_COPY_TIMED(t_host, share(i - 1, 0); while (done.load(std::memory_order_acquire) < i * n_thr) std::this_thread::yield())
+    }
+  }
+#ifdef MPLX_COPY_TIMING
+  fprintf(stderr, "mplx copy: %d chunks, %d + %d B per entry on the wire + made, %d helpers: waited %.2f ms for copies, %.2f ms scattering\n",
+          n_chunks, bpe, made_bpe, n_thr, t_link, t_host);
+#endif
+#undef MPLX_COPY_TIMED
   if (rc != MPLX_OK) {
     join_all();
     (void)hipStreamSynchronize(c->stream);
diff --git a/motion_primitive_library_amd/csrc/lists_host.cpp b/motion_primitive_library_amd/csrc/lists_host.cpp
--- a/motion_primitive_library_amd/csrc/lists_host.cpp
+++ b/motion_primitive_library_amd/csrc/lists_host.cpp
@@ -300,24 +300,28 @@
     return fail(c, MPLX_ERR_ARG, "mplx_expand_lists: the heur / flags rows come back through host pointers for batches of up to "
                                  "8 MiB of lists only (a search's); larger ones: mplx_expand_lists_device and a copy of the rows");
   const size_t slots = (size_t)n_slots;
+  const bool want_action = h_out->action || (h_out->state && action_worth_carrying(order_k_rows(c->dim, c->prm.control)));
   StageLayout l;
-  const size_t o_nodes = l.add((size_t)F * n_nodes * 8), o_count = l.add((size_t)n_nodes * 4), o_action = l.add(h_out->action ? slots * 4 : 0),
+  const size_t o_nodes = l.add((size_t)F * n_nodes * 8), o_count = l.add((size_t)n_nodes * 4), o_action = l.add(want_action ? slots * 4 : 0),
                o_cost = l.add(h_out->cost ? slots * 8 : 0), o_hash = l.add(h_out->hash ? slots * 8 : 0),
                o_iters = l.add(h_out->iters ? slots * 4 : 0), o_state = l.add(h_out->state ? F * slots * 8 : 0);
   if (int rc = stage_commit(c, &l)) return rc;
   HIP_TRY(c, stage_in_rows(c, l.base + o_nodes, h_nodes, (size_t)node_stride * 8, (size_t)n_nodes * 8, F));
   mplx_succ_lists d{};
   d.count = (int32_t *)(l.base + o_count);
-  if (h_out->action) d.action = (int32_t *)(l.base + o_action);
+  if (want_action) d.action = (int32_t *)(l.base + o_action);
   if (h_out->cost) d.cost = (double *)(l.base + o_cost);
   if (h_out->hash) d.hash = (uint64_t *)(l.base + o_hash);
   if (h_out->iters) d.iters = (int32_t *)(l.base + o_iters);
   if (h_out->state) { d.state = (double *)(l.base + o_state); d.state_stride = n_slots; }
   d.node_stride = h_out->node_stride;
-  if (int rc = lists_device(c, (const double *)(l.base + o_nodes), n_nodes, n_nodes, &d)) return rc;
+  uint32_t skip = const_zero_rows(c->dim, c->prm.control);
+  const int rc_launch = lists_device(c, (const double *)(l.base + o_nodes), n_nodes, n_nodes, &d, &skip);
+  c->last_zero_rows = 0;
+  if (rc_launch) return rc_launch;
   MPLX_GUARD_BEGIN
   if (int rc = resolve_pending(c)) return rc;
-  return copy_lists_to_host(c, d, h_out, n_nodes);
+  return copy_lists_to_host(c, d, h_out, n_nodes, h_nodes, node_stride);
   MPLX_GUARD_END(c)
 }
 
diff --git a/motion_primitive_library_amd/csrc/lists_host_rows.h b/motion_primitive_library_amd/csrc/lists_host_rows.h
--- /dev/null
+++ b/motion_primitive_library_amd/csrc/lists_host_rows.h
@@ -0,0 +1,162 @@
+#ifndef MPLX_LISTS_HOST_ROWS_H
+#define MPLX_LISTS_HOST_ROWS_H
+
+#include "../../include/mplx.h"
+
+#include <cstdint>
+#include <cstring>
+
+namespace mplx_detail {
+
+inline int control_order(int control) {
+  const int ctl = control & 0x0f;
+  return ctl == MPLX_VEL ? 1 : ctl == MPLX_ACC ? 2 : ctl == MPLX_JRK ? 3 : 4;
+}
+
+inline uint32_t const_zero_rows(int dim, int control) {
+  const int order = control_order(control);
+  uint32_t m = 0;
+  for (int b = order + 1; b <= 3; b++)
+    for (int i = 0; i < dim; i++) m |= 1u << (b * dim + i);
+  if (!(control & 0x10)) m |= 1u << (4 * dim);
+  return m;
+}
+
+enum HostRowKind : int {
+  kRowTravels = 0,
+  kRowZero = 1,
+  kRowOrderK = 2,
+  kRowT = 3,
+};
+
+inline void host_row_kinds(int dim, int control, int *kinds) {
+  const int F = 4 * dim + 2, order = control_order(control);
+  const uint32_t zero = const_zero_rows(dim, control);
+  for (int f = 0; f < F; f++) kinds[f] = ((zero >> f) & 1u) ? kRowZero : kRowTravels;
+#ifndef MPLX_HOST_ROWS_ZERO_ONLY
+  if (order <= 3)
+    for (int i = 0; i < dim; i++) kinds[order * dim + i] = kRowOrderK;
+  kinds[4 * dim + 1] = kRowT;
+#else
+  (void)order;
+#endif
+}
+
+inline bool action_worth_carrying(int n_order_k_rows) { return 4 < 8 * n_order_k_rows; }
+inline int order_k_rows(int dim, int control) {
+  int kinds[4 * 3 + 2], n = 0;
+  host_row_kinds(dim, control, kinds);
+  for (int f = 0; f < 4 * dim + 2; f++) n += kinds[f] == kRowOrderK;
+  return n;
+}
+
+struct HostRow {
+  char *host = nullptr;
+  int es = 0;
+  int64_t host_node_stride = 0;
+  int kind = kRowTravels;
+  int axis = 0;
+  int wire = -1;
+};
+
+struct HostRowSource {
+  const double *U = nullptr;
+  int udim = 0;
+  const double *node_t = nullptr;
+  double dt = 0;
+  int action_wire = -1;
+};
+
+constexpr int kMaxListRows = 24;
+struct HostRowPlan {
+  HostRow rows[kMaxListRows];
+  const void *dev[kMaxListRows];
+  int wire_es[kMaxListRows];
+  int n_rows = 0, n_wire = 0;
+  int wire_bpe = 0, made_bpe = 0;
+  HostRowSource src;
+};
+
+inline HostRowPlan plan_host_rows(int dim, int control, const mplx_succ_lists &d, const mplx_succ_lists &h, int64_t S,
+                                  const double *U, int udim, const double *h_nodes, int64_t h_node_stride, double dt) {
+  HostRowPlan p;
+  const int F = 4 * dim + 2;
+  int kinds[4 * 3 + 2];
+  host_row_kinds(dim, control, kinds);
+  p.src.U = U;
+  p.src.udim = udim;
+  p.src.node_t = h_nodes ? h_nodes + (size_t)(4 * dim + 1) * h_node_stride : nullptr;
+  p.src.dt = dt;
+  auto add = [&](const void *dp, void *host, int es, int kind, int axis) {
+    HostRow r;
+    r.host = (char *)host; r.es = es; r.host_node_stride = S; r.kind = kind; r.axis = axis;
+    if (kind == kRowTravels) {
+      r.wire = p.n_wire;
+      p.dev[p.n_wire] = dp;
+      p.wire_es[p.n_wire++] = es;
+      p.wire_bpe += es;
+    } else {
+      p.made_bpe += es;
+    }
+    p.rows[p.n_rows++] = r;
+  };
+  if (h.cost) add(d.cost, h.cost, 8, kRowTravels, 0);
+  if (h.hash) add(d.hash, h.hash, 8, kRowTravels, 0);
+  if (h.state)
+    for (int f = 0; f < F; f++) {
+      int kind = kinds[f];
+      if (kind == kRowOrderK && !(d.action && U)) kind = kRowTravels;
+      if (kind == kRowT && !p.src.node_t) kind = kRowTravels;
+      add(d.state + (size_t)f * d.state_stride, h.state + (size_t)f * h.state_stride, 8, kind, f % dim);
+    }
+  if (d.action && (h.action || (h.state && U && order_k_rows(dim, control) > 0))) {
+    p.src.action_wire = p.n_wire;
+    add(d.action, h.action, 4, kRowTravels, 0);
+  }
+  if (h.iters) add(d.iters, h.iters, 4, kRowTravels, 0);
+  return p;
+}
+
+inline void scatter_rows(const HostRow *rows, int n_rows, const int64_t *row_off, const char *pin, const int32_t *count,
+                         const int64_t *offs, int64_t off0, const HostRowSource &src, int64_t a, int64_t b) {
+  static const volatile double kZero = 0.0;
+  const double zero = kZero;
+  for (int r = 0; r < n_rows; r++) {
+    const HostRow &row = rows[r];
+    if (!row.host) continue;
+    const int es = row.es;
+    if (row.kind == kRowTravels) {
+      const char *from = pin + row_off[row.wire];
+      for (int64_t k = a; k < b; k++) {
+        const int cnt = count[k];
+        if (cnt > 0)
+          std::memcpy(row.host + (size_t)k * row.host_node_stride * es, from + (size_t)(offs[k] - off0) * es, (size_t)cnt * es);
+      }
+    } else if (row.kind == kRowZero) {
+      for (int64_t k = a; k < b; k++) {
+        const int cnt = count[k];
+        if (cnt > 0) std::memset(row.host + (size_t)k * row.host_node_stride * 8, 0, (size_t)cnt * 8);
+      }
+    } else if (row.kind == kRowOrderK) {
+      const int32_t *act = (const int32_t *)(pin + row_off[src.action_wire]);
+      const double *u = src.U + row.axis;
+      const size_t udim = (size_t)src.udim;
+      for (int64_t k = a; k < b; k++) {
+        const int cnt = count[k];
+        double *out = (double *)row.host + (size_t)k * row.host_node_stride;
+        const int32_t *ak = act + (offs[k] - off0);
+        for (int e = 0; e < cnt; e++) out[e] = zero + u[(size_t)ak[e] * udim];
+      }
+    } else {
+      for (int64_t k = a; k < b; k++) {
+        const int cnt = count[k];
+        double *out = (double *)row.host + (size_t)k * row.host_node_stride;
+        const double t = src.node_t[k] + src.dt;
+        for (int e = 0; e < cnt; e++) out[e] = t;
+      }
+    }
+  }
+}
+
+}
+#endif
diff --git a/motion_primitive_library_amd/csrc/lists_route.cpp b/motion_primitive_library_amd/csrc/lists_route.cpp
--- a/motion_primitive_library_amd/csrc/lists_route.cpp
+++ b/motion_primitive_library_amd/csrc/lists_route.cpp
@@ -375,15 +375,6 @@
   return MPLX_OK;
 }
 
-static uint32_t const_zero_rows(int dim, int control) {
-  const int order = control_order(control);
-  uint32_t m = 0;
-  for (int b = order + 1; b <= 3; b++)
-    for (int i = 0; i < dim; i++) m |= 1u << (b * dim + i);
-  if (!(control & 0x10)) m |= 1u << (4 * dim);
-  return m;
-}
-
 static mplx::GridArgs grid_args(mplx_ctx *c, const GridPlan &gp, const double *d_nodes, int64_t n_nodes, int64_t node_stride,
                                 const mplx_succ_lists *o, uint32_t skip) {
   mplx::GridArgs a{};
diff --git a/motion_primitive_library_amd/csrc/mplx_api.cpp b/motion_primitive_library_amd/csrc/mplx_api.cpp
--- a/motion_primitive_library_amd/csrc/mplx_api.cpp
+++ b/motion_primitive_library_amd/csrc/mplx_api.cpp
@@ -554,6 +554,7 @@
 
 int mplx_last_lists_route(const mplx_ctx *c) { return c ? c->last_route : MPLX_ERR_ARG; }
 int mplx_last_lists_zero_rows(const mplx_ctx *c) { return c ? (int)c->last_zero_rows : MPLX_ERR_ARG; }
+int64_t mplx_last_lists_copy_bytes(const mplx_ctx *c) { return c ? c->pk_last_bytes : (int64_t)MPLX_ERR_ARG; }
 int mplx_last_grid_kernel(const mplx_ctx *c) {
   if (!c) return MPLX_ERR_ARG;
   if (c->last_route != MPLX_ROUTE_GRID) return MPLX_KERNEL_NONE;
diff --git a/motion_primitive_library_amd/csrc/mplx_ctx.h b/motion_primitive_library_amd/csrc/mplx_ctx.h
--- a/motion_primitive_library_amd/csrc/mplx_ctx.h
+++ b/motion_primitive_library_amd/csrc/mplx_ctx.h
@@ -5,6 +5,7 @@
 #include "../../include/mplx_debug.h"
 #include "../../include/mplx_open.h"
 #include "../../include/mplx_traj.h"
+#include "lists_host_rows.h"
 #include "mplx_internal.h"
 
 #include <cstdarg>
@@ -127,6 +128,7 @@
   size_t pk_pin_cap = 0;
   hipEvent_t pk_ev[2] = {nullptr, nullptr};
   std::vector<int64_t> pk_hoffs;
+  int64_t pk_last_bytes = 0;
   void *pk_hb = nullptr;
   size_t pk_hb_cap = 0;
   struct YawPending {
@@ -270,11 +272,6 @@
   return (stride % 32 == 0 && !c->tune.no_line_pad && c->nU >= mplx::kLinePadMinControls) ? 1 : 0;
 }
 
-inline int control_order(int control) {
-  const int ctl = control & 0x0f;
-  return ctl == MPLX_VEL ? 1 : ctl == MPLX_ACC ? 2 : ctl == MPLX_JRK ? 3 : 4;
-}
-
 int ctx_ready(mplx_ctx *c);
 
 struct TilePlan {
@@ -298,7 +295,8 @@
                 bool *handled, mplx_succ_lists *view);
 int wait_small_launch(mplx_ctx *c);
 
-int copy_lists_to_host(mplx_ctx *c, const mplx_succ_lists &d, const mplx_succ_lists *h_out, int64_t n_nodes);
+int copy_lists_to_host(mplx_ctx *c, const mplx_succ_lists &d, const mplx_succ_lists *h_out, int64_t n_nodes,
+                       const double *h_nodes, int64_t h_node_stride);
 void release_copy_buffers(mplx_ctx *c);
 
 
diff --git a/motion_primitive_library_amd/env.py b/motion_primitive_library_amd/env.py
--- a/motion_primitive_library_amd/env.py
+++ b/motion_primitive_library_amd/env.py
@@ -1277,6 +1277,9 @@
     def last_lists_zero_rows(self):
         return int(_abi.lib().mplx_last_lists_zero_rows(self._ctx))
 
+    def last_lists_copy_bytes(self):
+        return int(_abi.lib().mplx_last_lists_copy_bytes(self._ctx))
+
     def last_grid_kernel(self):
         return {0: "none", 1: "grid", 2: "lex", 3: "pair"}[_abi.lib().mplx_last_grid_kernel(self._ctx)]
 
diff --git a/profiles/micro/host_rows_e2e.py b/profiles/micro/host_rows_e2e.py
--- /dev/null
+++ b/profiles/micro/host_rows_e2e.py
@@ -0,0 +1,33 @@
+import json
+import os
+import sys
+import time
+
+sys.path.insert(0, os.getcwd())
+
+import numpy as np
+
+import motion_primitive_library_amd as m
+
+
+def main():
+    calls = int(sys.argv[1]) if len(sys.argv) > 1 else 10
+    wl = m.workloads.make("C4")
+    env = m.EnvMap(wl.dim, 0)
+    wl.apply(env)
+    out = env.expand_lists(wl.nodes, want_state=True, want_iters=False)
+    emitted = int(out["count"].sum(dtype=np.int64))
+    times = []
+    for _ in range(calls):
+        t0 = time.perf_counter()
+        out = env.expand_lists(wl.nodes, want_state=True, want_iters=False, out=out)
+        times.append((time.perf_counter() - t0) * 1e3)
+    moved = env.last_lists_copy_bytes() if hasattr(env, "last_lists_copy_bytes") else None
+    env.close()
+    print(json.dumps({"lib": m._abi.LIB_PATH, "calls_ms": [round(t, 2) for t in times], "median_ms": round(sorted(times)[len(times) // 2], 2),
+                      "min_ms": round(min(times), 2), "max_ms": round(max(times), 2), "emitted": emitted, "d2h_bytes": moved,
+                      "caller_bytes": wl.n_nodes * 4 + emitted * 132}))
+
+
+if __name__ == "__main__":
+    main()
```

New measurement: 109.4 billion pairs/s (median of 3 runs). No clear change (+0.0%).
